# MougyTestspace/hclib

Hardware: AMD Instinct MI355X
Metric: UTS nodes/sec (tasks/sec) at 1/2/4/8 MI355X vs host-CPU HClib; forasync HBM GB/s (higher is better)
Workload: dtype u32; 1 GPU; test/uts T3L (-t 0 -b 2000 -q 0.200014 -m 5 -r 7) searched whole on 1 GPU (no split); nodes=111345631, bit_exact=True, parallelism=shard1 (hash-partitioned frontier, RCCL all-reduce of counts)

## Files before the change

hclib_amd/__init__.py:

```python
from __future__ import annotations

import ctypes as C
import os
from typing import Optional, Tuple

PKG = os.path.dirname(os.path.abspath(__file__))
LIB_PATH = os.environ.get("HCLIB_AMD_LIB") or os.path.join(PKG, "lib", "libhclib_amd.so")

HCLIB_HIP_OK = 0
FORASYNC_MODE_FLAT = 0
FORASYNC_MODE_RECURSIVE = 1
BODY_TRIAD_F32 = 1
BODY_IOTA_CHECK = 2
BODY_VISIT_COUNT = 3


class HclibError(RuntimeError):
    pass


class LoopDomain(C.Structure):

    _fields_ = [("low", C.c_int), ("high", C.c_int), ("stride", C.c_int), ("tile", C.c_int)]

# ... 48 lines not shown

class SwEdges(C.Structure):

    _fields_ = [("bottoms", C.c_void_p), ("rights", C.c_void_p), ("corners", C.c_void_p),
                ("path", C.c_int), ("form", C.c_int)]


SW_EDGE_BOTTOMS, SW_EDGE_RIGHTS, SW_EDGE_CORNERS = 1, 2, 4
SW_PATHS = {1: "queue", 2: "rows1", 3: "band-rows", 4: "dag-wave", 5: "dag-wg", 6: "dag-pk"}


class CholeskyResult(C.Structure):

    _fields_ = [("tasks", C.c_uint64), ("puts", C.c_uint64), ("releases", C.c_uint64),
                ("potrf", C.c_uint64), ("trsm", C.c_uint64), ("syrk", C.c_uint64), ("gemm", C.c_uint64),
                ("kernel_ms", C.c_double), ("gflops", C.c_double), ("fail_col", C.c_int)]


class SortResult(C.Structure):

    _fields_ = [("tasks", C.c_uint64), ("sort_leaf", C.c_uint64), ("sort_split", C.c_uint64),
                ("merge_leaf", C.c_uint64), ("merge_split", C.c_uint64), ("merge_empty", C.c_uint64),
                ("finishes", C.c_uint64), ("check_ins", C.c_uint64),
                ("kernel_ms", C.c_double), ("keys_per_s", C.c_double)]


class SparseLUResult(C.Structure):

    _fields_ = [("blocks_in", C.c_uint64), ("blocks_out", C.c_uint64),
                ("lu0", C.c_uint64), ("fwd", C.c_uint64), ("bdiv", C.c_uint64), ("bmod", C.c_uint64),
                ("tasks", C.c_uint64), ("puts", C.c_uint64), ("releases", C.c_uint64),
                ("kernel_ms", C.c_double), ("gflops", C.c_double), ("wgs_per_cu", C.c_int)]


class NQueensResult(C.Structure):

    _fields_ = [("solutions", C.c_uint64), ("tasks", C.c_uint64), ("items", C.c_uint64), ("scopes", C.c_uint64),
                ("joins", C.c_uint64), ("chunks_pushed", C.c_uint64), ("chunks_stolen", C.c_uint64),
                ("kernel_ms", C.c_double), ("busy_frac", C.c_double)]


class StrassenResult(C.Structure):

    _fields_ = [("tasks", C.c_uint64), ("splits", C.c_uint64), ("base", C.c_uint64), ("tiles", C.c_uint64),
                ("pre_bands", C.c_uint64), ("combine_bands", C.c_uint64), ("finishes", C.c_uint64),
                ("check_ins", C.c_uint64), ("workspace_bytes", C.c_uint64),
                ("kernel_ms", C.c_double), ("gflops", C.c_double)]


class FftResult(C.Structure):

    _fields_ = [("tasks", C.c_uint64), ("leaves", C.c_uint64), ("calls", C.c_uint64), ("unsh_bands", C.c_uint64),
                ("twid_bands", C.c_uint64), ("finishes", C.c_uint64), ("check_ins", C.c_uint64),
                ("bytes_moved", C.c_uint64), ("nfactors", C.c_int32), ("factors", C.c_int32 * 40),
                ("cutoff", C.c_int32), ("band", C.c_int32), ("kernel_ms", C.c_double), ("gbytes_per_s", C.c_double)]


class JacobiResult(C.Structure):

    _fields_ = [("tasks", C.c_uint64), ("puts", C.c_uint64), ("releases", C.c_uint64), ("supersteps", C.c_uint64),
                ("bytes_moved", C.c_uint64), ("block", C.c_int), ("fuse", C.c_int), ("wgs_per_cu", C.c_int),
                ("kernel_ms", C.c_double), ("gbytes_per_s", C.c_double), ("gcells_per_s", C.c_double)]


class BfsResult(C.Structure):

    _fields_ = [("levels", C.c_uint64), ("reached", C.c_uint64), ("relaxed", C.c_uint64), ("items", C.c_uint64),
                ("chunks_pushed", C.c_uint64), ("chunks_stolen", C.c_uint64),
                ("kernel_ms", C.c_double), ("busy_frac", C.c_double)]


class HealthParams(C.Structure):

    _fields_ = [(k, C.c_int) for k in ("level", "cities", "population_ratio", "sim_time", "assess_time",
                                       "convalescence_time")] + [("seed", C.c_int32)] + \
               [(k, C.c_float) for k in ("get_sick_p", "convalescence_p", "realloc_p")]


class HealthResult(C.Structure):

    _fields_ = [(k, C.c_int64) for k in ("population", "hospitals", "personnel", "hosps_visited", "in_village",
                                         "waiting", "assess", "inside", "total_time")] + \
               [(k, C.c_uint64) for k in ("tasks", "finishes", "check_ins", "leaf_calls", "inner_calls", "posts")] + \
               [("kernel_ms", C.c_double), ("rounds_per_s", C.c_double)]


class HealthState(C.Structure):

    _fields_ = [(k, C.c_void_p) for k in ("seed", "time", "time_left", "hosps_visited", "village", "lists")]


FLOORPLAN_MAX_CELLS, FLOORPLAN_MAX_SHAPES = 20, 8


class FloorplanInput(C.Structure):

    _fields_ = [("n", C.c_int32), ("solution", C.c_int32), ("shapes", C.c_int32 * (FLOORPLAN_MAX_CELLS + 1)),
                ("shape", C.c_int32 * 2 * FLOORPLAN_MAX_SHAPES * (FLOORPLAN_MAX_CELLS + 1)),
                ("left", C.c_int32 * (FLOORPLAN_MAX_CELLS + 1)), ("above", C.c_int32 * (FLOORPLAN_MAX_CELLS + 1)),
                ("next", C.c_int32 * (FLOORPLAN_MAX_CELLS + 1))]


class FloorplanPlacement(C.Structure):

    _fields_ = [("shape", C.c_int32), ("top", C.c_int32), ("lhs", C.c_int32)]


class FloorplanResult(C.Structure):

    _fields_ = [("min_area", C.c_int32), ("footprint", C.c_int32 * 2),
                ("placements", FloorplanPlacement * FLOORPLAN_MAX_CELLS)] + \
               [(k, C.c_uint64) for k in ("tasks", "items", "laid", "complete", "improvements", "chunks_pushed",
                                          "chunks_stolen")] + [("kernel_ms", C.c_double), ("busy_frac", C.c_double)]


class AlignmentInput(C.Structure):

    _fields_ = [("nseqs", C.c_int32), ("total", C.c_int32), ("length", C.POINTER(C.c_int32)),
                ("offset", C.POINTER(C.c_int32)), ("codes", C.POINTER(C.c_uint8)), ("names", C.c_void_p)]


class AlignmentMatrix(C.Structure):

    _fields_ = [("avscore", C.c_int32), ("score", C.c_int32 * 32 * 32)]


class AlignmentPair(C.Structure):

    _fields_ = [(k, C.c_int32) for k in ("si", "sj", "g", "gh", "maxscore", "se1", "se2", "sb1", "sb2", "matches",
                                         "diff_calls", "type2", "ties")]


class AlignmentResult(C.Structure):

    _fields_ = [("scores", C.c_void_p)] + \
               [(k, C.c_uint64) for k in ("pairs", "tasks", "created", "promises", "pair_tasks", "spawn_tasks",
                                          "leaf_tasks", "matches", "diff_calls", "type2", "ties", "cells")] + \
               [("cutoff", C.c_int32), ("kernel_ms", C.c_double), ("cells_per_s", C.c_double)]


class AtomicViewStruct(C.Structure):

    _fields_ = [("slots", C.c_void_p), ("nslots", C.c_uint32), ("stride", C.c_uint32),
                ("dtype", C.c_int), ("op", C.c_int)]


EXPORTS_HIP = [
    "hclib_hip_init", "hclib_hip_finalize", "hclib_hip_device_memory_live", "hclib_hip_last_error",
    "hclib_hip_num_cus",
    "hclib_hip_version", "hclib_hip_forasync", "hclib_hip_forasync_triad_f32",
    "hclib_hip_num_workers", "hclib_hip_uts_search", "hclib_hip_uts_num_children_host",
    "hclib_hip_uts_bucket_check", "hclib_hip_sha1_calibrate",
    "hclib_hip_fib", "hclib_hip_sw", "hclib_hip_last_sched_counters", "hclib_hip_last_narrow_counters",
    "hclib_hip_last_phase_counters", "hclib_hip_last_shed_counters",
    "hclib_hip_sw_band_begin", "hclib_hip_sw_band_rows", "hclib_hip_sw_band_end",
    "hclib_hip_sw_edges", "hclib_hip_sw_band_bottoms",
    "hclib_hip_atomic_create", "hclib_hip_atomic_destroy", "hclib_hip_atomic_view",
    "hclib_hip_atomic_gather", "hclib_hip_atomic_gather_async", "hclib_hip_atomic_reset",
    "hclib_hip_forasync_reduce", "hclib_hip_cholesky", "hclib_hip_sort_i64", "hclib_hip_sort_bounds",
    "hclib_hip_sparselu_genmat", "hclib_hip_sparselu_plan", "hclib_hip_sparselu", "hclib_hip_sparselu_bmod_rate",
    "hclib_hip_nqueens", "hclib_hip_nqueens_bounds",
    "hclib_hip_strassen", "hclib_hip_strassen_bounds", "hclib_hip_strassen_last_ticks",
    "hclib_hip_health", "hclib_hip_health_bounds", "hclib_hip_health_last_ticks",
    "hclib_hip_floorplan", "hclib_hip_floorplan_read_input",
    "hclib_hip_alignment", "hclib_hip_alignment_read_input", "hclib_hip_alignment_free_input",
    "hclib_hip_alignment_read_matrix", "hclib_hip_alignment_bounds", "hclib_hip_alignment_last_ticks",
    "hclib_hip_fft", "hclib_hip_fft_factors", "hclib_hip_fft_twiddles", "hclib_hip_fft_bounds", "hclib_hip_fft_last_ticks",
    "hclib_hip_jacobi", "hclib_hip_jacobi_rhs", "hclib_hip_jacobi_bounds",
    "hclib_hip_bfs", "hclib_hip_bfs_bounds", "hclib_hip_bfs_read_input",
    "hclib_atomic_create", "hclib_atomic_init", "hclib_atomic_update", "hclib_atomic_gather",
]

_lib = None


def lib():
    global _lib
    if _lib is None:
        try:
            import torch
        except ImportError:
            pass
        if not os.path.exists(LIB_PATH):
            raise HclibError(f"{LIB_PATH} is missing: run `python -m hclib_amd.build`")
        L = C.CDLL(LIB_PATH)
        L.hclib_hip_version.restype = C.c_char_p
        L.hclib_hip_last_error.restype = C.c_char_p
        L.hclib_hip_finalize.restype = None
        L.hclib_hip_device_memory_live.argtypes = [C.POINTER(C.c_uint64)]
        L.hclib_hip_device_memory_live.restype = None
        L.hclib_hip_forasync_triad_f32.argtypes = [C.c_void_p, C.c_void_p, C.c_void_p, C.c_float,
                                                   C.c_int64, C.c_void_p]
        L.hclib_hip_forasync.argtypes = [C.c_int, C.c_void_p, C.c_int, C.POINTER(LoopDomain),
                                         C.c_int, C.c_void_p]
        L.hclib_hip_uts_search.argtypes = [C.POINTER(UtsParams), C.c_int, C.c_int, C.c_int,
                                           C.POINTER(UtsResult), C.c_void_p, C.c_int]
        L.hclib_hip_uts_num_children_host.argtypes = [C.POINTER(UtsParams), C.c_int,
                                                      C.POINTER(C.c_uint32)]
        L.hclib_hip_fib.argtypes = [C.c_int, C.POINTER(C.c_int64), C.POINTER(FibResult)]
        L.hclib_hip_sw.argtypes = [C.c_char_p, C.c_size_t, C.c_char_p, C.c_size_t, C.c_int,
                                   C.c_int, C.POINTER(C.c_int), C.POINTER(SwResult)]
        L.hclib_hip_sw_band_begin.argtypes = [C.c_char_p, C.c_size_t, C.c_char_p, C.c_size_t,
                                              C.c_int, C.c_int, C.c_int, C.c_int,
                                              C.POINTER(C.c_void_p)]
        L.hclib_hip_sw_band_rows.argtypes = [C.c_void_p, C.c_int, C.c_int, C.c_void_p, C.c_void_p,
                                             C.c_void_p]
        L.hclib_hip_sw_band_end.argtypes = [C.c_void_p, C.c_void_p, C.POINTER(C.c_int),
                                            C.POINTER(C.c_uint64)]
        L.hclib_hip_sw_edges.argtypes = [C.c_char_p, C.c_size_t, C.c_char_p, C.c_size_t, C.c_int,
                                         C.c_int, C.POINTER(C.c_int), C.POINTER(SwResult),
                                         C.POINTER(SwEdges), C.POINTER(C.c_uint32)]
        L.hclib_hip_sw_band_bottoms.argtypes = [C.c_void_p, C.c_void_p, C.c_void_p]
        L.hclib_hip_atomic_calibrate.argtypes = [C.c_int, C.c_int, C.POINTER(C.c_double),
                                                 C.POINTER(C.c_double)]
        L.hclib_hip_sha1_calibrate.argtypes = [C.c_int, C.c_int, C.c_int, C.POINTER(C.c_double),
                                               C.POINTER(C.c_double)]
        L.hclib_hip_uts_last_launch.argtypes = [C.POINTER(UtsLaunch)]
        L.hclib_hip_uts_bucket_check.argtypes = [C.POINTER(UtsParams), C.c_uint64, C.POINTER(C.c_uint64)]
        L.hclib_hip_global_bytes.restype = C.c_size_t
        L.hclib_hip_global_bytes.argtypes = [C.c_uint32]
        L.hclib_hip_global_init.argtypes = [C.c_void_p, C.c_uint32, C.c_int]
        L.hclib_hip_global_alloc.argtypes = [C.c_uint32, C.c_int, C.POINTER(C.c_void_p)]
        L.hclib_hip_global_free.argtypes = [C.c_void_p]
        L.hclib_hip_global_attach.argtypes = [C.c_void_p, C.c_uint32, C.c_int]
        L.hclib_hip_global_read.argtypes = [C.c_void_p, C.POINTER(C.c_uint64)]
        L.hclib_hip_ipc_export.argtypes = [C.c_void_p, C.c_void_p]
        L.hclib_hip_ipc_import.argtypes = [C.c_void_p, C.POINTER(C.c_void_p)]
        L.hclib_hip_ipc_close.argtypes = [C.c_void_p]
        L.hclib_hip_last_timeline.argtypes = [C.c_void_p, C.c_uint64, C.POINTER(C.c_uint32)]
        L.hclib_hip_atomic_create.argtypes = [C.c_int, C.c_int, C.c_void_p, C.POINTER(C.c_void_p)]
        L.hclib_hip_atomic_destroy.argtypes = [C.c_void_p]
        L.hclib_hip_atomic_view.argtypes = [C.c_void_p, C.POINTER(AtomicViewStruct)]
        L.hclib_hip_atomic_gather.argtypes = [C.c_void_p, C.c_void_p, C.c_void_p]
        L.hclib_hip_atomic_gather_async.argtypes = [C.c_void_p, C.c_void_p, C.c_void_p]
        L.hclib_hip_atomic_reset.argtypes = [C.c_void_p, C.c_void_p]
        L.hclib_hip_forasync_reduce.argtypes = [C.c_void_p, C.c_void_p, C.c_int, C.POINTER(LoopDomain),
                                                C.c_int, C.c_void_p]
        L.hclib_hip_cholesky.argtypes = [C.c_void_p, C.c_int, C.c_int, C.c_int, C.c_void_p,
                                         C.POINTER(CholeskyResult)]
        L.hclib_hip_sort_i64.argtypes = [C.c_void_p, C.c_int64, C.c_int, C.c_int, C.POINTER(SortResult)]
        L.hclib_hip_sort_bounds.argtypes = [C.c_int64, C.c_int, C.c_int, C.POINTER(C.c_uint64)]
        L.hclib_hip_sort_last_ticks.argtypes = [C.POINTER(C.c_uint64)]
        L.hclib_hip_sort_last_ticks.restype = None
        L.hclib_hip_sparselu_genmat.argtypes = [C.c_int, C.c_int, C.c_void_p, C.c_void_p]
        L.hclib_hip_sparselu_plan.argtypes = [C.c_void_p, C.c_int, C.c_void_p, C.POINTER(C.c_uint64), C.c_void_p,
                                              C.c_void_p, C.c_void_p]
        L.hclib_hip_sparselu.argtypes = [C.c_void_p, C.c_void_p, C.c_int, C.c_int, C.c_void_p, C.c_void_p,
                                         C.POINTER(SparseLUResult)]
        L.hclib_hip_sparselu_bmod_rate.argtypes = [C.c_int, C.c_int, C.c_int, C.POINTER(C.c_double),
                                                   C.POINTER(C.c_double)]
        L.hclib_hip_nqueens.argtypes = [C.c_int, C.c_int, C.c_int, C.POINTER(NQueensResult), C.POINTER(C.c_uint64)]
        L.hclib_hip_nqueens_bounds.argtypes = [C.c_int, C.c_int, C.c_int, C.POINTER(C.c_uint64)]
        L.hclib_hip_floorplan.argtypes = [C.POINTER(FloorplanInput), C.c_int, C.POINTER(FloorplanResult), C.c_void_p,
                                          C.POINTER(C.c_uint64)]
        L.hclib_hip_floorplan_read_input.argtypes = [C.c_char_p, C.POINTER(FloorplanInput)]
        L.hclib_hip_strassen.argtypes = [C.c_void_p, C.c_void_p, C.c_void_p, C.c_int, C.c_int, C.c_int,
                                         C.POINTER(StrassenResult)]
        L.hclib_hip_strassen_bounds.argtypes = [C.c_int, C.c_int, C.c_int, C.POINTER(C.c_uint64)]
        L.hclib_hip_strassen_last_ticks.argtypes = [C.POINTER(C.c_uint64)]
        L.hclib_hip_strassen_last_ticks.restype = None
        L.hclib_hip_health.argtypes = [C.POINTER(HealthParams), C.POINTER(HealthResult), C.POINTER(HealthState)]
        L.hclib_hip_health_bounds.argtypes = [C.POINTER(HealthParams), C.POINTER(C.c_uint64)]
        L.hclib_hip_health_last_ticks.argtypes = [C.POINTER(C.c_uint64)]
        L.hclib_hip_health_last_ticks.restype = None
        L.hclib_hip_alignment.argtypes = [C.POINTER(AlignmentInput), C.POINTER(AlignmentMatrix), C.c_int,
                                          C.POINTER(AlignmentResult), C.c_void_p]
        L.hclib_hip_alignment_read_input.argtypes = [C.c_char_p, C.POINTER(AlignmentInput)]
        L.hclib_hip_alignment_free_input.argtypes = [C.POINTER(AlignmentInput)]
        L.hclib_hip_alignment_free_input.restype = None
        L.hclib_hip_alignment_read_matrix.argtypes = [C.c_char_p, C.POINTER(AlignmentMatrix)]
        L.hclib_hip_alignment_bounds.argtypes = [C.POINTER(AlignmentInput), C.c_int, C.POINTER(C.c_uint64)]
        L.hclib_hip_alignment_last_ticks.argtypes = [C.POINTER(C.c_uint64)]
        L.hclib_hip_alignment_last_ticks.restype = None
        L.hclib_hip_fft.argtypes = [C.c_void_p, C.c_void_p, C.c_int, C.c_void_p, C.c_int, C.c_int, C.POINTER(FftResult)]
        L.hclib_hip_fft_factors.argtypes = [C.c_int, C.POINTER(C.c_int)]
        L.hclib_hip_fft_twiddles.argtypes = [C.c_int, C.c_void_p]
        L.hclib_hip_fft_bounds.argtypes = [C.c_int, C.c_int, C.c_int, C.POINTER(C.c_uint64)]
        L.hclib_hip_fft_last_ticks.argtypes = [C.POINTER(C.c_uint64)]
        L.hclib_hip_fft_last_ticks.restype = None
        L.hclib_hip_jacobi.argtypes = [C.c_void_p, C.c_void_p, C.c_int, C.c_int, C.c_double, C.c_double, C.c_int, C.c_int,
                                       C.c_int, C.c_void_p, C.POINTER(JacobiResult)]
        L.hclib_hip_jacobi_rhs.argtypes = [C.c_int, C.c_int, C.c_void_p, C.c_void_p]
        L.hclib_hip_jacobi_bounds.argtypes = [C.c_int, C.c_int, C.c_int, C.c_int, C.c_int, C.POINTER(C.c_uint64)]
        L.hclib_hip_bfs.argtypes = [C.c_void_p, C.c_void_p, C.c_int, C.c_void_p, C.c_int, C.c_int, C.c_int, C.c_void_p,
                                    C.POINTER(BfsResult), C.c_void_p, C.c_void_p]
        L.hclib_hip_bfs_bounds.argtypes = [C.c_void_p, C.c_void_p, C.c_int, C.c_void_p, C.c_int, C.c_int, C.c_int,
                                           C.POINTER(C.c_uint64)]
        L.hclib_hip_bfs_read_input.argtypes = [C.c_char_p, C.c_void_p, C.c_void_p, C.c_void_p, C.POINTER(C.c_int64)]
        _lib = L
    return _lib


def _check(rc: int, what: str):
    if rc != HCLIB_HIP_OK:
        msg = lib().hclib_hip_last_error().decode(errors="replace")
        raise HclibError(f"{what} failed ({rc}): {msg}")


def version() -> str:
    return lib().hclib_hip_version().decode()


def init(device: int = 0) -> None:
    _check(lib().hclib_hip_init(device), "hclib_hip_init")


def finalize() -> None:
# ... 728 lines not shown
              inp.next[c]) for c in range(1, inp.n + 1)]
    return cells, inp.solution


def floorplan(cells_or_path, prune: bool = True, hist: bool = False) -> dict:
    cells = floorplan_read_input(cells_or_path)[0] if isinstance(cells_or_path, (str, bytes, os.PathLike)) \
        else cells_or_path
    inp = _floorplan_input(cells)
    r = FloorplanResult()
    board = (C.c_uint8 * 4096)()
    h = (C.c_uint64 * (FLOORPLAN_MAX_CELLS + 1))() if hist else None
    _check(lib().hclib_hip_floorplan(C.byref(inp), 0 if prune else FLOORPLAN_NOPRUNE, C.byref(r), board, h),
           "hclib_hip_floorplan")
    out = {k: getattr(r, k) for k, _ in FloorplanResult._fields_ if k not in ("footprint", "placements")}
    out["footprint"] = list(r.footprint)
    out["placements"] = [[p.shape, p.top, p.lhs] for p in r.placements[:inp.n]] if r.min_area < 4096 else None
    out["board"] = bytes(board)
    if hist:
        out["hist"] = list(h)[:inp.n + 1]
    return out


ALIGNMENT_CODES = "ABCDEFGHIKLMNPQRSTUVWXYZ-"
ALIGNMENT_MAX_LEN = 4999
ALIGNMENT_DEFAULT_CUTOFF = 16384
ALIGNMENT_BOUNDS = ("pairs", "tasks", "spawns", "diff_calls", "arena_bytes", "row_bytes")
ALIGNMENT_TICKS = ("root", "pair", "spawn", "leaf")


def alignment_read_input(path):
    inp = AlignmentInput()
    _check(lib().hclib_hip_alignment_read_input(os.fsencode(path), C.byref(inp)), "hclib_hip_alignment_read_input")
    try:
        names = C.string_at(inp.names, inp.nseqs * 31)
        return [(names[31 * i:31 * i + 31].split(b"\0")[0].decode("latin-1"),
                 [inp.codes[inp.offset[i] + k] for k in range(inp.length[i])]) for i in range(inp.nseqs)]
    finally:
        lib().hclib_hip_alignment_free_input(C.byref(inp))


def alignment_read_matrix(path):
    m = AlignmentMatrix()
    _check(lib().hclib_hip_alignment_read_matrix(os.fsencode(path), C.byref(m)), "hclib_hip_alignment_read_matrix")
    return m.avscore, [list(row) for row in m.score]


def _alignment_input(seqs):
    if isinstance(seqs, (str, bytes, os.PathLike)):
        seqs = alignment_read_input(seqs)
    codes = [list(q[1]) if isinstance(q, tuple) else list(q) for q in seqs]
    if any(not 0 <= c <= 255 for q in codes for c in q):
        raise ValueError("alignment: residue codes are 0..31")
    n, total = len(codes), sum(len(q) for q in codes)
    length = (C.c_int32 * max(n, 1))(*[len(q) for q in codes])
    offset = (C.c_int32 * max(n, 1))()
    flat = (C.c_uint8 * max(total, 1))()
    at = 0
    for i, q in enumerate(codes):
        offset[i] = at
        flat[at:at + len(q)] = q
        at += len(q)
    inp = AlignmentInput(nseqs=n, total=total, length=length, offset=offset, codes=flat, names=None)
    return inp, (length, offset, flat)


def _alignment_matrix(matrix) -> AlignmentMatrix:
    if isinstance(matrix, AlignmentMatrix):
        return matrix
    if isinstance(matrix, (str, bytes, os.PathLike)):
        matrix = alignment_read_matrix(matrix)
    avscore, rows = matrix
    if len(rows) != 32 or any(len(r) != 32 for r in rows):
        raise ValueError("alignment: the matrix has 32 x 32 scores")
    m = AlignmentMatrix(avscore=avscore)
    for i, row in enumerate(rows):
        for j, v in enumerate(row):
            m.score[i][j] = v
    return m


def alignment_bounds(seqs, cutoff: int = 0) -> dict:
    inp, keep = _alignment_input(seqs)
    out = (C.c_uint64 * 6)()
    _check(lib().hclib_hip_alignment_bounds(C.byref(inp), cutoff, out), "hclib_hip_alignment_bounds")
    return dict(zip(ALIGNMENT_BOUNDS, out))


def alignment(seqs, matrix, cutoff: int = 0, pairs: bool = False) -> dict:
    inp, keep = _alignment_input(seqs)
    m = _alignment_matrix(matrix)
    ns = inp.nseqs
    scores = (C.c_int32 * max(ns * ns, 1))()
    r = AlignmentResult(scores=C.addressof(scores))
    npairs = alignment_bounds([list(keep[2][keep[1][i]:keep[1][i] + keep[0][i]]) for i in range(ns)], cutoff)["pairs"] \
        if pairs else 0
    recs = (AlignmentPair * max(npairs, 1))() if pairs else None
    _check(lib().hclib_hip_alignment(C.byref(inp), C.byref(m), cutoff, C.byref(r), recs), "hclib_hip_alignment")
    out = {k: getattr(r, k) for k, _ in AlignmentResult._fields_ if k != "scores"}
    out["scores"] = [list(scores[i * ns:(i + 1) * ns]) for i in range(ns)]
    if pairs:
        out["pair_records"] = [{k: getattr(q, k) for k, _ in AlignmentPair._fields_} for q in recs[:npairs]]
    return out


def alignment_last_ticks() -> dict:
    out = (C.c_uint64 * 4)()
    lib().hclib_hip_alignment_last_ticks(out)
    return dict(zip(ALIGNMENT_TICKS, out))


ATOMIC_SCATTER_RET64 = 0
ATOMIC_HOT_WORD = 1
ATOMIC_COALESCED32 = 2


def atomic_calibrate(mode: int, iters: int = 256):
    r, ms = C.c_double(), C.c_double()
    _check(lib().hclib_hip_atomic_calibrate(mode, iters, C.byref(r), C.byref(ms)),
           "hclib_hip_atomic_calibrate")
    return r.value, ms.value


def sha1_calibrate(chains: int = 1, waves_per_cu: int = 8, iters: int = 2000):
    r, ms = C.c_double(), C.c_double()
    _check(lib().hclib_hip_sha1_calibrate(chains, waves_per_cu, iters, C.byref(r), C.byref(ms)),
           "hclib_hip_sha1_calibrate")
    return r.value, ms.value


def last_phase_counters():
    out = (C.c_uint64 * 8)()
    lib().hclib_hip_last_phase_counters(out)
    return list(out)


def last_sched_counters():
    out = (C.c_uint64 * 16)()
    lib().hclib_hip_last_sched_counters(out)
    return list(out)


def last_narrow_counters():
    out = (C.c_uint64 * 4)()
    lib().hclib_hip_last_narrow_counters(out)
    return list(out)


def last_shed_counters():
    out = (C.c_uint64 * 8)()
    lib().hclib_hip_last_shed_counters(out)
    return dict(zip(("exits", "placed", "blocks", "items", "fallbacks"), out))


TIMELINE_EVENTS = {1: "start", 2: "busy", 3: "idle", 4: "spill", 5: "term", 6: "end"}


def last_timeline():
    per = C.c_uint32()
    nw = lib().hclib_hip_last_timeline(None, 0, C.byref(per))
    if nw <= 0 or per.value == 0:
        return []
    import numpy as np
    buf = np.zeros(nw * per.value, dtype=np.uint64)
    lib().hclib_hip_last_timeline(buf.ctypes.data, buf.size, C.byref(per))
    buf = buf.reshape(nw, per.value)
    out = []
    for w in range(nw):
        row = buf[w][buf[w] != 0]
        out.append([(int(v >> 24), int((v >> 20) & 0xF), int(v & 0xFFFFF)) for v in row])
    return out
```

hclib_amd/csrc/hx_module.h:

```cpp
#pragma once

#include <hip/hip_runtime.h>
#include <stdint.h>

#include <string>
#include <vector>

#include "../../include/hclib_hip.h"
#include "../../include/hclib_hip/hx_sched.h"

namespace hx {

enum ArenaId {
    kArenaGlobals,
    kArenaWaveStats,
    kArenaWaveCtr,
    kArenaTimeline,
    kArenaDeques,
    kArenaSeed,
    kArenaDag,
    kArenaDagTrace,
    kArenaDyn,
    kArenaCholesky,
    kArenaSparselu,
    kArenaSort,
    kArenaStrassen,
    kArenaHealth,
    kArenaAlignment,
    kArenaFft,
    kArenaJacobi,
    kArenaUtsTables,
    kArenaCount
};
struct Arena {
    void *mem = nullptr;
    size_t bytes = 0;
};

struct Module {
    bool inited = false;
    int device = -1;
    int num_cus = 0;
    std::string arch;
    hipStream_t stream = nullptr;
    hipEvent_t ev0 = nullptr, ev1 = nullptr;
    Arena arenas[kArenaCount];
    bool uts_tables_cached = false;
    SchedGlobals *globals = nullptr;
    unsigned long long last_counters[16] = {};
    unsigned long long last_narrow[4] = {};
    unsigned long long last_shed[8] = {};
    unsigned long long last_phase[8] = {};
    WaveStat *wave_stats = nullptr;
    uint32_t wave_stats_cap = 0;
    std::vector<WaveStat> last_waves;
    unsigned long long *wave_ctr = nullptr;
    uint32_t rec_workers = 0;
    GlobalView gview = {nullptr, nullptr, nullptr, 0, 0};
    unsigned long long *timeline = nullptr;
    uint32_t timeline_cap = 0;
    std::vector<unsigned long long> last_timeline;
};

Module &mod();
void set_error(const char *fmt, ...);
int ensure_device();
int hip_check(hipError_t e, const char *what);
int check_resident(const void *kern, int blocks, int threads, size_t lds, const char *what);
int upload_async(void *dst, const void *src, size_t bytes, hipStream_t stream);

int arena_reserve(ArenaId id, size_t bytes, const char *who, void **ptr);

class DevBuf {
  public:
    DevBuf() = default;
    DevBuf(const DevBuf &) = delete;
    DevBuf &operator=(const DevBuf &) = delete;
    ~DevBuf();
    int alloc(size_t bytes, const char *who);
    char *p = nullptr;

  private:
    size_t bytes_ = 0;
};

int make_pool(uint32_t nq, uint32_t cap, uint32_t chunk, uint32_t words, PoolView *out);
struct SeedCfg {
    uint32_t target, max_levels, words, min_levels;
    uint32_t solo_cap = 0;
};
int reset_sched(const PoolView &pool, uint32_t outstanding_init, bool global = false, uint32_t workers = 0,
                const SeedCfg *seed = nullptr);
int finish_sched(SchedGlobals *host_copy, const char *who);

int env_int(const char *name, int dflt);

}

#define HX_TRY(expr)                         \
    do {                                     \
        int _rc = (expr);                    \
        if (_rc != HCLIB_HIP_OK) return _rc; \
    } while (0)
#define HX_HIP(call) HX_TRY(::hx::hip_check((call), #call))
```

hclib_amd/csrc/hx_uts_plan.h:

```cpp
#pragma once

#include <stdarg.h>
#include <stdio.h>

#include "hx_uts_host.h"

namespace hx {

enum UtsMode : int {
    kUtsRulesGlobal = 0,
    kUtsRulesLds = 1,
    kUtsBin = 2,
    kUtsGeoFixed = 3,
};

constexpr int kUtsSeedMaxLevels = 24;

struct UtsKnobs {
    static constexpr int kUnset = -0x7fffffff;
    int grid = 0;
    int waves_per_cu = kUnset;
    int wpg = 4;
    int uts_ring = kUnset;
    int uts_geo_fixed = 1;
    int uts_seed = 1;
    int uts_trace = 0;
    int uts_dual = 1;
    int deques = 128, deque_cap = 4096, chunk = 64;
    int spill_hi = 512;
    int spill_lo = kUnset;
    int seed_per_wave = kUnset;
    bool seed_per_wave_set = false;
    int seed_levels = 20, seed_solo = 128;
    int hunger = kUnset;
    int spin_limit_ms = 20000, stamps = 0, carry = 2, backoff = 16, defer = 1, spills_per_batch = 0;
    int narrow_shed = 1, narrow_shed_sibs = 3;
};

struct UtsPlan {
    int status = HCLIB_HIP_OK;
    bool bin = false, geo_fixed = false;
    int geo_depth = 0;
    int lds_tables = 0;
    uint32_t bin_thr = 0;
    int mode = 0;
    int feat = 0;
    bool global = false;
    int ring = 512, wpg = 1, grid = 0, waves_per_cu = 0;
    uint32_t nq = 0, deque_cap = 0, chunk = 0;
    uint32_t spill_hi = 0, spill_lo = 0, spin_limit = 0, nwaves = 0, stamps = 0, hunger = 0, backoff = 0, carry = 0,
             defer = 0, dual = 0, spills = 0, hunger_init_full = 0, narrow_shed = 0;
    uint32_t seed_target = 0, seed_max_levels = 0, seed_min_levels = 0, seed_solo_cap = 0;
    hclib_hip_uts_launch_t launch = {-1, 0, 0, 0, 0, 0, 0, 0, 0};
};

namespace uts_detail {
__attribute__((format(printf, 2, 3))) inline int refuse(std::string &err, const char *fmt, ...) {
    char buf[512];
    va_list ap;
    va_start(ap, fmt);
    vsnprintf(buf, sizeof(buf), fmt, ap);
    va_end(ap);
    err = buf;
    return HCLIB_HIP_EINVAL;
}
}

inline UtsPlan uts_plan(const hclib_hip_uts_params_t &p, const UtsTables &T, int num_cus, int shard, int nshards,
                        int split_depth, int max_levels, bool global_attached, const UtsKnobs &kn, std::string &err) {
    using uts_detail::refuse;
    constexpr int U = UtsKnobs::kUnset;
    (void)shard;
    UtsPlan P;
    const int trace_kind = max_levels > 0 ? kn.uts_trace : 0;
    const bool trace = trace_kind != 0;

    P.lds_tables = (T.rules.size() <= kUtsLdsRules && T.thr.size() <= kUtsLdsThr) ? 1 : 0;
    {
        const int nr = (int)T.rules.size();
        int d = 1;
        while (d < nr && T.rules[d].x == 2 && T.rules[d].z == 0) ++d;
        bool rest_zero = d > 1 && T.stationary;
        for (int e = d; e < nr && rest_zero; ++e) rest_zero = T.rules[e].x == 0 && T.rules[e].y == 0;
        if (rest_zero && T.thr.size() >= 128) P.geo_depth = d;
    }
    const bool bin = p.type == 0 && T.rules.size() == 2 && T.rules[1].x == 1 && T.stationary;
    const bool geo_fixed = !bin && P.geo_depth > 0 && kn.uts_geo_fixed;
    P.bin = bin;
    P.geo_fixed = geo_fixed;
    if (bin) P.bin_thr = (uint32_t)T.rules[1].y;
    const int mode = bin ? kUtsBin : geo_fixed ? kUtsGeoFixed : (P.lds_tables ? kUtsRulesLds : kUtsRulesGlobal);
    P.mode = mode;
    const double est = uts_expected_nodes(p);

    const bool trace_refused = trace && (mode != kUtsBin || nshards > 1);

    P.nq = (uint32_t)kn.deques;
    P.deque_cap = (uint32_t)kn.deque_cap;
    P.chunk = (uint32_t)kn.chunk;

    const bool global = nshards > 1 && global_attached && max_levels == 0;
    P.global = global;
    const bool seed_on = geo_fixed && !global && kn.uts_seed;
    bool bin_seed = bin && nshards > 1 && !global && max_levels == 0 && split_depth >= 1 &&
                    split_depth + 1 < kUtsSeedMaxLevels && kn.uts_seed;
    int wpc_default = bin && !global ? 4 : 2, ring_default = 512;
    if (!bin) {
        if (seed_on) {
            wpc_default = 8;
            ring_default = 512;
        } else {
            wpc_default = est >= 3e7 ? 8 : (geo_fixed ? 2 : 4);
            ring_default = est >= 3e7 ? 512 : 256;
        }
    }
    const int grid = kn.grid > 0 ? kn.grid : num_cus * (kn.waves_per_cu != U ? kn.waves_per_cu : wpc_default);
    P.grid = grid;
    P.waves_per_cu = grid / (num_cus > 0 ? num_cus : 1);
    if (bin_seed) {
        const double cap = 8.0 * 1 + 65536.0;
        const double qm = p.non_leaf_prob * bin_rule_m(p) > 0 ? p.non_leaf_prob * bin_rule_m(p) : 0.0;
        double n = T.root_nc > 0 ? (double)T.root_nc : 0.0, widest = n;
        for (int d = 2; d <= split_depth; ++d) {
            n *= qm;
            if (n > widest) widest = n;
        }
        const double n_mine = n * qm / nshards;
        if (!(widest <= 0.5 * cap && n_mine <= 0.5 * cap && n_mine <= (double)grid * (1024 / 4))) bin_seed = false;
    }
    P.spill_hi = (uint32_t)kn.spill_hi;
    const int ring_used = geo_fixed && !(nshards > 1 || max_levels > 0) ? (kn.uts_ring != U ? kn.uts_ring : ring_default)
                                                                       : 512;
    if (ring_used != 256 && ring_used != 512 && ring_used != 1024) {
        P.status = refuse(err,
                          "hclib_hip_uts_search: HCLIB_HIP_UTS_RING=%d is not a ring the search is built for (256, 512 "
                          "or 1024 items per wave)", ring_used);
        return P;
    }
    int spill_lo_default = bin ? 66 : (geo_fixed && ring_used < 512) ? 128 : 224;
    const int per_wave = kn.seed_per_wave != U ? kn.seed_per_wave : (est >= 3e7 ? 32 : 16);
    bool seed_fits = seed_on && ring_used >= 512;
    if (seed_fits) {
        if (kn.seed_per_wave_set) {
            const double b = geo_bi(p, 1) > kUtsMaxChildren ? (double)kUtsMaxChildren : geo_bi(p, 1);
            if (per_wave < 1) {
                P.status = refuse(err,
                                  "hclib_hip_uts_search: HCLIB_HIP_SEED_PER_WAVE=%d is not a slot count (1 or more; "
                                  "HCLIB_HIP_UTS_SEED=0 turns the seeding off)", per_wave);
                return P;
            }
            if (b * per_wave > ring_used / 2) {
                P.status = refuse(err,
                                  "hclib_hip_uts_search: HCLIB_HIP_SEED_PER_WAVE=%d cannot fit the ring: a wave's share "
                                  "of the seeded level reaches %.0f x %d items, the seeding hands over at most %d of a "
                                  "%d-item ring", per_wave, b, per_wave, ring_used / 2, ring_used);
                return P;
            }
        }
        const double target = (double)grid * per_wave, cap = 8.0 * target + 65536.0;
        double n = T.root_nc > 0 ? (double)T.root_nc : 0.0;
        for (int d = 1; d < 64 && n > 0.0 && n < target; ++d) {
            const double b = geo_bi(p, d) > kUtsMaxChildren ? (double)kUtsMaxChildren : geo_bi(p, d);
            n *= b > 0.0 ? b : 0.0;
        }
        seed_fits = n <= 0.5 * cap && n <= (double)grid * (ring_used / 4);
    }
    const bool seeded = seed_fits;
    if (seeded) spill_lo_default = est >= 3e7 ? 448 : 336;
    {
        const int ring_launch = bin ? 1024 : ring_used, lo = kn.spill_lo != U ? kn.spill_lo : spill_lo_default;
        if (lo < 1 || lo > ring_launch) {
            P.status = refuse(err,
                              "hclib_hip_uts_search: HCLIB_HIP_SPILL_LO=%d does not fit the %d-item ring of this launch "
                              "(1..%d)", lo, ring_launch, ring_launch);
            return P;
        }
        P.spill_lo = (uint32_t)lo;
    }
    P.spin_limit = (uint32_t)kn.spin_limit_ms;
    P.nwaves = (uint32_t)grid;
    P.stamps = (uint32_t)kn.stamps;
    const bool small_fixed = geo_fixed && est < 3e7;
    const bool large_fixed = geo_fixed && ring_used >= 512 && !small_fixed;
    P.hunger = (uint32_t)(kn.hunger != U ? kn.hunger : large_fixed ? 128 : bin ? 64 : 32);
    P.carry = (uint32_t)kn.carry;
    P.backoff = (uint32_t)kn.backoff;
    P.defer = (uint32_t)kn.defer;
    P.dual = (uint32_t)kn.uts_dual;
    P.spills = (uint32_t)kn.spills_per_batch;
    {
        const int rule = kn.narrow_shed, sibs = kn.narrow_shed_sibs;
        if (rule < 0 || rule > 3 || sibs < 0 || sibs > 3) {
            P.status = refuse(err,
                              "hclib_hip_uts_search: HCLIB_HIP_NARROW_SHED=%d / HCLIB_HIP_NARROW_SHED_SIBS=%d: the keep "
                              "rule is 0 (off), 1, 2 or 3, the sibling inboxes per exit 0..3", rule, sibs);
            return P;
        }
        P.narrow_shed = (uint32_t)rule | (uint32_t)sibs << 8;
    }
    if (trace_refused) {
        P.status = refuse(err, "hclib_hip_uts_search: the depth trace is for unsharded BIN trees");
        return P;
    }
    if (seeded) {
        P.seed_target = (uint32_t)(grid * per_wave);
        P.seed_max_levels = (uint32_t)kn.seed_levels;
        P.seed_solo_cap = (uint32_t)kn.seed_solo;
        if (nshards > 1) {
            double n_split = 1.0, n_next = 1.0;
            for (int d = 0; d <= split_depth && d < 64; ++d) {
                if (d < split_depth) n_split *= geo_bi(p, d) > 0 ? geo_bi(p, d) : 0.0;
                n_next *= geo_bi(p, d) > 0 ? geo_bi(p, d) : 0.0;
            }
            const double cap = 8.0 * P.seed_target + 65536.0;
            const bool fits = split_depth + 1 < kUtsSeedMaxLevels && split_depth < (int)P.seed_max_levels &&
                              n_split <= 0.5 * cap && n_next / nshards <= (double)grid * (512 / 8);
            P.seed_min_levels = fits ? (uint32_t)split_depth : 0u;
        }
    } else if (bin_seed) {
        P.seed_target = 1;
        P.seed_max_levels = (uint32_t)split_depth;
        P.seed_min_levels = (uint32_t)split_depth;
    }

    const bool seed_past_split = P.seed_target && nshards > 1 && P.seed_min_levels == (uint32_t)split_depth;
    const bool filter = max_levels > 0 || (nshards > 1 && (global || !seed_past_split));
    P.feat = trace ? (trace_kind == 2 ? 3 : 2) : (filter ? 1 : 0);
    P.ring = mode == kUtsBin ? 1024 : 512;
    if (mode == kUtsGeoFixed && !filter && !global) P.ring = ring_used;
    if (mode == kUtsBin && !global && (!trace || trace_kind == 2)) {
        P.wpg = kn.wpg;
        if (P.wpg != 2 && P.wpg != 4) P.wpg = 1;
        if (grid % P.wpg) P.wpg = 1;
    }
    P.launch = hclib_hip_uts_launch_t{mode, trace ? 1 + trace_kind : P.feat, P.wpg, grid, P.ring, P.seed_target ? 1 : 0, (int)P.seed_target,
                                      (int)P.spill_lo, P.waves_per_cu};
    return P;
}

}
```

hclib_amd/csrc/module.hip:

```cpp
#include <stdarg.h>
#include <stdio.h>
#include <stdlib.h>
#include <string.h>

#include "hx_client.h"

namespace hx {

static Module g_mod;
static thread_local char g_err[512] = "";

Module &mod() { return g_mod; }

void set_error(const char *fmt, ...) {
    va_list ap;
    va_start(ap, fmt);
    vsnprintf(g_err, sizeof(g_err), fmt, ap);
    va_end(ap);
}

static uint64_t g_live[2] = {0, 0};
static bool dev_acquire(void **p, size_t bytes) {
    if (hipMalloc(p, bytes) != hipSuccess) {
        (void)hipGetLastError();
// ... 82 lines not shown
int make_pool(uint32_t nq, uint32_t cap, uint32_t chunk, uint32_t words, PoolView *out) {
    if (nq < 8 || nq % 8 || cap < 2 || (cap & (cap - 1)) || chunk < 1 || chunk > 64) {
        set_error("chunk deques: need 8k deques, power-of-two capacity, 1..64 items per chunk");
        return HCLIB_HIP_EINVAL;
    }
    for (uint32_t c = chunk; c * 2 <= 64; c *= 2) cap *= 2;
    const size_t hdr = sizeof(QueueHdr) * nq;
    const size_t slots = (size_t)nq * cap;
    const size_t need = hdr + slots * 4 * 2 + slots * chunk * words * 4 + 4096;
    char *p = nullptr;
    HX_TRY(arena_reserve(kArenaDeques, need, "chunk deques", (void **)&p));
    out->hdr = (QueueHdr *)p;
    p += hdr;
    out->seq = (uint32_t *)p;
    out->cnt = out->seq + 1;
    p += slots * 8;
    p = (char *)(((uintptr_t)p + 255) & ~(uintptr_t)255);
    out->data = (uint32_t *)p;
    out->nq = nq;
    out->cap = cap;
    out->chunk = chunk;
    return HCLIB_HIP_OK;
}

struct Staged {
    void *host;
    hipEvent_t done;
};
std::vector<Staged> &staged() {
    static std::vector<Staged> v;
    return v;
}
void reap_staged() {
    std::vector<Staged> &v = staged();
    for (size_t i = 0; i < v.size();) {
        if (hipEventQuery(v[i].done) == hipSuccess) {
            (void)hipHostFree(v[i].host);
            (void)hipEventDestroy(v[i].done);
            v[i] = v.back();
            v.pop_back();
        } else {
            ++i;
        }
    }
}
int upload_async(void *dst, const void *src, size_t bytes, hipStream_t st) {
    reap_staged();
    void *pin = nullptr;
    HX_HIP(hipHostMalloc(&pin, bytes, hipHostMallocDefault));
    memcpy(pin, src, bytes);
    hipEvent_t ev;
    if (hipEventCreateWithFlags(&ev, hipEventDisableTiming) != hipSuccess) {
        (void)hipHostFree(pin);
        set_error("upload: hipEventCreate failed");
        return HCLIB_HIP_EHIP;
    }
    if (hipMemcpyAsync(dst, pin, bytes, hipMemcpyHostToDevice, st) != hipSuccess ||
        hipEventRecord(ev, st) != hipSuccess) {
        (void)hipStreamSynchronize(st);
        (void)hipHostFree(pin);
        (void)hipEventDestroy(ev);
        set_error("upload: host-to-device copy failed");
        return HCLIB_HIP_EHIP;
    }
    staged().push_back(Staged{pin, ev});
    return HCLIB_HIP_OK;
}

int reset_sched(const PoolView &pool, uint32_t outstanding_init, bool global, uint32_t workers,
                const SeedCfg *seed) {
    Module &m = g_mod;
    HX_HIP(hipMemsetAsync(pool.hdr, 0, sizeof(QueueHdr) * pool.nq, m.stream));
    const uint32_t total = pool.nq * pool.cap;
    hipLaunchKernelGGL(k_reset_pool, dim3((total + 255) / 256), dim3(256), 0, m.stream, pool.seq,
                       pool.cap, total);
    HX_HIP(hipGetLastError());
    SchedGlobals init;
    memset(&init, 0, sizeof(init));
    init.outstanding = outstanding_init;
    init.wave_stats = m.wave_stats;
    init.wave_stats_cap = m.wave_stats_cap;
    m.rec_workers = workers < m.wave_stats_cap ? workers : m.wave_stats_cap;
    init.wave_ctr = m.rec_workers ? m.wave_ctr : nullptr;
    init.wave_ctr_cap = m.rec_workers;
    if (seed && seed->target && workers) {
        const uint32_t cap = 8u * seed->target + 65536u;
        const size_t ctl = (size_t)kSeedCtlLines * 256;
        const size_t need = ctl + 2ull * cap * seed->words * 4;
        char *seed_mem = nullptr;
        HX_TRY(arena_reserve(kArenaSeed, need, "seeding", (void **)&seed_mem));
        HX_HIP(hipMemsetAsync(seed_mem, 0, ctl, m.stream));
        init.seed.ctl = (uint32_t *)seed_mem;
        init.seed.buf = (uint32_t *)(seed_mem + ctl);
        init.seed.cap = cap;
        init.seed.target = seed->target;
        init.seed.max_levels = seed->max_levels;
        init.seed.min_levels = seed->min_levels;
        init.seed.solo_cap = seed->solo_cap;
        init.outstanding = workers;
    }
    if (global) init.gview = m.gview;
    const int tl_cap = env_int("HCLIB_HIP_TIMELINE", 0);
    if (tl_cap > 0) {
        HX_TRY(arena_reserve(kArenaTimeline, (size_t)m.wave_stats_cap * tl_cap * 8, "worker timelines",
                             (void **)&m.timeline));
        m.timeline_cap = (uint32_t)tl_cap;
        HX_HIP(hipMemsetAsync(m.timeline, 0, (size_t)m.wave_stats_cap * tl_cap * 8, m.stream));
        init.timeline = m.timeline;
        init.timeline_cap = m.timeline_cap;
    }
    static SchedGlobals *stage = nullptr;
    if (!stage && hipHostMalloc((void **)&stage, sizeof(SchedGlobals), hipHostMallocDefault) != hipSuccess)
        return upload_async(m.globals, &init, sizeof(init), m.stream);
    *stage = init;
    HX_HIP(hipMemcpyAsync(m.globals, stage, sizeof(init), hipMemcpyHostToDevice, m.stream));
    return HCLIB_HIP_OK;
}

static const char *err_name(uint32_t e) {
    switch (e) {
    case kErrQueueFull: return "chunk deque full and LDS ring near capacity";
    case kErrStackOverflow: return "LDS ring overflow";
    case kErrSpinTimeout: return "idle spin timed out (no termination)";
    case kErrDepthTable: return "tree deeper than the device depth-rule table";
    case kErrArena: return "device arena exhausted";
    case kErrBadTask: return "malformed task";
    default: return "unknown device error";
    }
}

int finish_sched(SchedGlobals *host_copy, const char *who) {
    Module &m = g_mod;
    HX_HIP(hipMemcpyAsync(host_copy, m.globals, sizeof(SchedGlobals), hipMemcpyDeviceToHost,
                          m.stream));
    const uint32_t nw_cap = m.wave_stats_cap;
    static std::vector<unsigned long long> rec;
    const uint32_t nrec = m.rec_workers;
    for (int i = 0; i < 8; ++i) m.last_phase[i] = 0;
    m.rec_workers = 0;
    if (nrec) {
        rec.resize((size_t)nrec * kWaveCtrWords);
        HX_HIP(hipMemcpyAsync(rec.data(), m.wave_ctr, rec.size() * 8, hipMemcpyDeviceToHost, m.stream));
    }
    HX_HIP(hipStreamSynchronize(m.stream));
    for (uint32_t w = 0; w < nrec; ++w) {
        const unsigned long long *r = &rec[(size_t)w * kWaveCtrWords];
        for (int i = 0; i < 16; ++i)
            if (i >= 8 || i < 4) host_copy->counters[i] += r[i];
        for (int i = 4; i < 8; ++i) host_copy->counters[i] += r[24 + i - 4];
        for (int i = 0; i < 4; ++i)
            if (r[16 + i] > host_copy->maxes[i]) host_copy->maxes[i] = r[16 + i];
        for (int i = 0; i < 3; ++i) host_copy->narrow[i] += r[20 + i];
        for (int i = 0; i < kShedCounts; ++i) host_copy->shed[i] += r[32 + i];
        m.last_phase[0] += r[23];
        for (int i = 0; i < 4; ++i) m.last_phase[1 + i] += r[28 + i];
        m.last_phase[5] += r[24];
        m.last_phase[6] += r[27];
    }
    memcpy(m.last_counters, host_copy->counters, sizeof(m.last_counters));
    memcpy(m.last_narrow, host_copy->narrow, sizeof(m.last_narrow));
    memcpy(m.last_shed, host_copy->shed, sizeof(m.last_shed));
    uint64_t nw = host_copy->counters[kCtrWaves];
    if (nw > nw_cap) nw = nw_cap;
    m.last_waves.resize(nw);
    if (nw) HX_HIP(hipMemcpy(m.last_waves.data(), m.wave_stats, nw * sizeof(WaveStat), hipMemcpyDeviceToHost));
    if (host_copy->timeline) {
        m.last_timeline.resize((size_t)nw * m.timeline_cap);
        if (nw)
            HX_HIP(hipMemcpy(m.last_timeline.data(), m.timeline, (size_t)nw * m.timeline_cap * 8,
                             hipMemcpyDeviceToHost));
    } else {
        m.last_timeline.clear();
    }
    if (host_copy->err) {
        set_error("%s: device error %u (%s)", who, host_copy->err, err_name(host_copy->err));
        return HCLIB_HIP_EDEVICE;
    }
    return HCLIB_HIP_OK;
}

}

using namespace hx;

extern "C" {

const char *hclib_hip_version(void) { return "hclib-mi355x 0.1 (gfx950 megakernel scheduler)"; }

const char *hclib_hip_last_error(void) { return g_err; }

int hclib_hip_init(int device) {
    Module &m = g_mod;
    if (m.inited) return HCLIB_HIP_OK;
    int n = 0;
    if (hipGetDeviceCount(&n) != hipSuccess || n <= 0) {
        set_error("hclib_hip_init: no HIP device visible");
        return HCLIB_HIP_ENODEV;
    }
    if (device < 0 || device >= n) {
        set_error("hclib_hip_init: device %d out of range (%d devices)", device, n);
        return HCLIB_HIP_EINVAL;
    }
    HX_HIP(hipSetDevice(device));
    hipDeviceProp_t prop;
    HX_HIP(hipGetDeviceProperties(&prop, device));
    m.arch = prop.gcnArchName;
    if (m.arch.rfind("gfx950", 0) != 0) {
        set_error("hclib_hip_init: device %d is %s, this module is built for gfx950 only", device,
                  prop.gcnArchName);
        return HCLIB_HIP_ENODEV;
    }
    m.device = device;
    m.num_cus = prop.multiProcessorCount;
    HX_HIP(hipStreamCreateWithFlags(&m.stream, hipStreamNonBlocking));
    HX_HIP(hipEventCreate(&m.ev0));
    HX_HIP(hipEventCreate(&m.ev1));
    const char *who = "hclib_hip_init";
    HX_TRY(arena_reserve(kArenaGlobals, sizeof(SchedGlobals), who, (void **)&m.globals));
    m.wave_stats_cap = (uint32_t)m.num_cus * 32;
    HX_TRY(arena_reserve(kArenaWaveStats, sizeof(WaveStat) * m.wave_stats_cap, who, (void **)&m.wave_stats));
    HX_TRY(arena_reserve(kArenaWaveCtr, 8ull * kWaveCtrWords * m.wave_stats_cap, who, (void **)&m.wave_ctr));
    m.inited = true;
    return HCLIB_HIP_OK;
}

void hclib_hip_finalize(void) {
    Module &m = g_mod;
    if (!m.inited) return;
    (void)hipStreamSynchronize(m.stream);
    for (Arena &a : m.arenas) dev_release(a.mem, a.bytes);
    (void)hipEventDestroy(m.ev0);
    (void)hipEventDestroy(m.ev1);
    (void)hipStreamDestroy(m.stream);
    m = Module();
}

void hclib_hip_device_memory_live(uint64_t out[2]) {
    out[0] = g_live[0];
    out[1] = g_live[1];
}

int hclib_hip_num_cus(void) { return g_mod.inited ? g_mod.num_cus : 0; }

int hclib_hip_device(void) { return g_mod.inited ? g_mod.device : -1; }

void *hclib_hip_stream(void) { return g_mod.inited ? (void *)g_mod.stream : nullptr; }

void hclib_hip_last_sched_counters(uint64_t out[16]) {
    for (int i = 0; i < 16; ++i) out[i] = g_mod.last_counters[i];
}

extern "C" void hclib_hip_last_phase_counters(uint64_t out[8]) {
    for (int i = 0; i < 8; ++i) out[i] = g_mod.last_phase[i];
}

void hclib_hip_last_narrow_counters(uint64_t out[4]) {
    for (int i = 0; i < 4; ++i) out[i] = g_mod.last_narrow[i];
}

void hclib_hip_last_shed_counters(uint64_t out[8]) {
    for (int i = 0; i < 8; ++i) out[i] = g_mod.last_shed[i];
}

int hclib_hip_last_wave_stats(hclib_hip_wave_stats_t *out, int max) {
    static_assert(sizeof(hclib_hip_wave_stats_t) == sizeof(WaveStat), "layout");
    const int n = (int)g_mod.last_waves.size();
    for (int i = 0; out && i < n && i < max; ++i) memcpy(&out[i], &g_mod.last_waves[(size_t)i], sizeof(WaveStat));
    return n;
}

int hclib_hip_last_timeline(uint64_t *out, uint64_t max_words, uint32_t *events_per_worker) {
    Module &m = g_mod;
    if (events_per_worker) *events_per_worker = m.last_timeline.empty() ? 0u : m.timeline_cap;
    const uint64_t n = m.last_timeline.size();
    for (uint64_t i = 0; out && i < n && i < max_words; ++i) out[i] = m.last_timeline[i];
    return m.timeline_cap ? (int)(n / m.timeline_cap) : 0;
}

int hclib_hip_sched_begin(uint32_t entry_words, uint32_t chunk, int waves_per_cu,
                          hclib_hip_sched_launch_t *out) {
    if (!out || entry_words < 4 || entry_words > 64 || waves_per_cu < 1 || waves_per_cu > 8) {
        set_error("hclib_hip_sched_begin: invalid arguments");
        return HCLIB_HIP_EINVAL;
    }
    HX_TRY(ensure_device());
    Module &m = g_mod;
    PoolView pool;
    HX_TRY(sched_pool(64, chunk, entry_words, &pool));
    HX_TRY(reset_sched(pool, 1, false, (uint32_t)(m.num_cus * waves_per_cu)));
    HX_HIP(hipEventRecord(m.ev0, m.stream));
    out->hdr = pool.hdr;
    out->seq = pool.seq;
    out->cnt = pool.cnt;
    out->data = pool.data;
    out->nq = pool.nq;
    out->cap = pool.cap;
    out->chunk = pool.chunk;
    out->globals = m.globals;
    out->stream = m.stream;
    out->grid = m.num_cus * waves_per_cu;
    out->num_cus = m.num_cus;
    return HCLIB_HIP_OK;
}

int hclib_hip_sched_end(const char *who, uint64_t counters[16], uint64_t maxes[4], double *kernel_ms) {
    Module &m = g_mod;
    if (!m.inited) {
        set_error("hclib_hip_sched_end: no device");
        return HCLIB_HIP_ENODEV;
    }
    SchedGlobals gl;
    memset(&gl, 0, sizeof(gl));
    float ms = 0;
    const int rc = end_sched(who ? who : "hclib_hip_sched_end", &gl, &ms);
    if (kernel_ms) *kernel_ms = ms;
    for (int i = 0; counters && i < 16; ++i) counters[i] = gl.counters[i];
    for (int i = 0; maxes && i < 4; ++i) maxes[i] = gl.maxes[i];
    return rc;
}

int hclib_hip_num_workers(void) {
    if (!g_mod.inited) return 0;
    return g_mod.num_cus * env_int("HCLIB_HIP_WAVES_PER_CU", 4);
}

}

static size_t global_layout(uint32_t cap, size_t *ctl_off, size_t *data_off) {
    const size_t words = 64 * 8;
    const size_t hdr = (sizeof(GlobalHdr) + 255) & ~(size_t)255;
    const size_t ctl = ((size_t)cap * 8 + 255) & ~(size_t)255;
    *ctl_off = hdr;
    *data_off = hdr + ctl;
    return hdr + ctl + (size_t)cap * words * 4;
}

extern "C" size_t hclib_hip_global_bytes(uint32_t cap) {
    size_t a, b;
    if (cap < 2 || (cap & (cap - 1))) return 0;
    return global_layout(cap, &a, &b);
}

__global__ void k_reset_global(uint32_t *ctl, uint32_t cap) {
    const uint32_t i = blockIdx.x * blockDim.x + threadIdx.x;
    if (i < cap) {
        ctl[2 * i] = i;
        ctl[2 * i + 1] = 0;
    }
}

extern "C" int hclib_hip_global_init(void *region, uint32_t cap, int nranks) {
    if (!region || cap < 2 || (cap & (cap - 1)) || nranks < 1 || nranks > kGlobalMaxRanks) {
        set_error("hclib_hip_global_init: invalid arguments");
        return HCLIB_HIP_EINVAL;
    }
    HX_TRY(ensure_device());
    Module &m = g_mod;
    size_t co, dof;
    global_layout(cap, &co, &dof);
    HX_HIP(hipMemsetAsync(region, 0, co, m.stream));
    hipLaunchKernelGGL(k_reset_global, dim3((cap + 255) / 256), dim3(256), 0, m.stream,
                       (uint32_t *)((char *)region + co), cap);
    HX_HIP(hipGetLastError());
    const uint32_t active = (uint32_t)nranks;
    uint32_t held[kGlobalMaxRanks];
    for (int r = 0; r < kGlobalMaxRanks; ++r) held[r] = r < nranks ? 1u : 0u;
    HX_HIP(hipMemcpyAsync(region, &active, 4, hipMemcpyHostToDevice, m.stream));
    HX_HIP(hipMemcpyAsync((char *)region + offsetof(GlobalHdr, held), held, sizeof(held), hipMemcpyHostToDevice,
                          m.stream));
    HX_HIP(hipStreamSynchronize(m.stream));
    return HCLIB_HIP_OK;
}

extern "C" int hclib_hip_global_attach(void *region, uint32_t cap, int rank) {
    HX_TRY(ensure_device());
    Module &m = g_mod;
    if (!region) {
        m.gview = GlobalView{nullptr, nullptr, nullptr, 0, 0};
        return HCLIB_HIP_OK;
    }
    if (cap < 2 || (cap & (cap - 1)) || rank < 0 || rank >= kGlobalMaxRanks) {
        set_error("hclib_hip_global_attach: invalid arguments");
        return HCLIB_HIP_EINVAL;
    }
    size_t co, dof;
    global_layout(cap, &co, &dof);
    m.gview.hdr = (GlobalHdr *)region;
    m.gview.ctl = (uint32_t *)((char *)region + co);
    m.gview.data = (uint32_t *)((char *)region + dof);
    m.gview.cap = cap;
    m.gview.rank = (uint32_t)rank;
    return HCLIB_HIP_OK;
}

extern "C" int hclib_hip_global_read(const void *region, uint64_t out[3 + 2 * kGlobalMaxRanks]) {
    if (!region || !out) {
        set_error("hclib_hip_global_read: invalid arguments");
        return HCLIB_HIP_EINVAL;
    }
    HX_TRY(ensure_device());
    GlobalHdr h;
    HX_HIP(hipMemcpy(&h, region, sizeof(h), hipMemcpyDeviceToHost));
    out[0] = h.active;
    out[1] = h.idle;
    out[2] = h.tail - h.head;
    for (int i = 0; i < 2 * kGlobalMaxRanks; ++i) out[3 + i] = h.moved[i];
    return HCLIB_HIP_OK;
}

extern "C" int hclib_hip_global_alloc(uint32_t cap, int kind, void **region_out) {
    size_t co, dof;
    if (!region_out || cap < 2 || (cap & (cap - 1)) || kind < 0 || kind > 2) {
        set_error("hclib_hip_global_alloc: invalid arguments");
        return HCLIB_HIP_EINVAL;
// ... 50 lines not shown
```

hclib_amd/csrc/uts.hip:

```cpp
#include <string.h>

#include <type_traits>
#include <vector>

#include "hx_client.h"
#include "uts_sha1.h"
#include "hx_uts_plan.h"

namespace hx {


static_assert(sizeof(UtsRule) == sizeof(int4) && offsetof(UtsRule, x) == offsetof(int4, x) &&
                  offsetof(UtsRule, y) == offsetof(int4, y) && offsetof(UtsRule, z) == offsetof(int4, z) &&
                  offsetof(UtsRule, w) == offsetof(int4, w),
              "UtsRule is uploaded as int4");
static_assert(kUtsSeedMaxLevels == kSeedMaxLevels, "the plan's level bound is the seeding's");
struct UtsCtx {
    uint32_t root[5];
    int root_nc;
    int nrules;
    int stationary;
    int gran;
    int m;
    int shard, nshards, split;
// ... 74 lines not shown
    using Ctx = UtsCtx;
    static constexpr bool kFixedChildren = MODE == kUtsBin;
    __device__ static uint32_t fixed_children(const Ctx &c) { return c.m > 0 ? (uint32_t)c.m : 0u; }
    struct Acc {
        uint32_t nodes = 0, leaves = 0;
        uint32_t maxd = 0;
        uint32_t trace_seen = 0;
        uint32_t mode = 0;
        uint32_t wid = 0;
        __device__ void totals(unsigned long long (&c)[8], unsigned long long (&m)[4]) {
            c[0] = wave_sum((unsigned long long)nodes);
            c[1] = wave_sum((unsigned long long)leaves);
            m[0] = (unsigned long long)wave_max(maxd);
        }
    };

    __device__ static bool movable(const Ctx &c, const uint32_t *tmpl) {
        return c.nshards <= 1 || (int)tmpl[5] >= c.split;
    }

    __device__ static int roots(const Ctx &c, Acc &acc, uint32_t *tmpl) {
        if (lane_id() == 0 && c.shard == 0) {
            acc.nodes += 1;
            if (c.root_nc <= 0) acc.leaves += 1;
            if (c.hist && c.hist_levels > 0) atomicAdd(&c.hist[0], 1ull);
        }
        for (int k = 0; k < 5; ++k) tmpl[k] = c.root[k];
        tmpl[5] = FEAT == 3 ? 0x80000000u : 0u;
        return c.root_nc;
    }

    template <int F = FEAT>
    __device__ static __forceinline__ int finish(const Ctx &c, Acc &acc, const uint32_t *t, const uint32_t *ch,
                                                 uint32_t *child, uint32_t *err, bool valid) {
        const int h1 = (int)(F == 3 ? t[5] & 0x7fffffffu : t[5]) + 1;
        bool counted = valid;
        if (F && c.nshards > 1) {
            if (h1 == c.split && (ch[0] % (uint32_t)c.nshards) != (uint32_t)c.shard) return 0;
            if (h1 < c.split && c.shard != 0) counted = false;
        }
        int nc = uts_nc<MODE>(c, valid ? h1 : 1, ch[4] & 0x7fffffffu, err);
        acc.nodes += counted ? 1u : 0u;
        acc.leaves += (counted && nc <= 0) ? 1u : 0u;
        acc.maxd = (counted && (uint32_t)h1 > acc.maxd) ? (uint32_t)h1 : acc.maxd;
        if (F == 1 && counted && c.hist && h1 < c.hist_levels) atomicAdd(&c.hist[h1], 1ull);
        if (F == 2 && c.hist) {
            const uint32_t dm = wave_max(counted ? (uint32_t)h1 : 0u);
            if (dm > acc.trace_seen) {
                acc.trace_seen = dm;
                if (lane_id() == 0 && (int)dm < c.hist_levels)
                    __hip_atomic_fetch_min(&c.hist[dm],
                                           ((__builtin_amdgcn_s_memrealtime() & 0x3fffffffffffull) << 17) |
                                               ((unsigned long long)(acc.wid & 0xffffu) << 1) | acc.mode,
                                           __ATOMIC_RELAXED, HX_AGENT);
            }
        }
        if (!valid) nc = 0;
        child[0] = ch[0];
        child[1] = ch[1];
        child[2] = ch[2];
        child[3] = ch[3];
        child[4] = ch[4];
        child[5] = (uint32_t)h1;
        return nc;
    }

    __device__ static __forceinline__ uint32_t chain_next(const Ctx &c, const uint32_t *t, bool valid) {
        uint32_t kc = 0xffffffffu;
        if (FEAT == 3 && valid && (t[5] >> 31)) kc = c.chain[(t[5] & 0x7fffffffu) + 1u];
        return kc;
    }
    __device__ static __forceinline__ void chain_stamp(const Ctx &c, const Acc &acc, uint32_t *child, bool on,
                                                       bool valid, uint32_t dual) {
        if constexpr (FEAT == 3) {
            const uint32_t fill = (uint32_t)__builtin_popcountll(__ballot(valid));
            if (on) {
                const uint32_t d = child[5];
                child[5] = d | 0x80000000u;
                c.hist[4 * d] = __builtin_amdgcn_s_memrealtime();
                c.hist[4 * d + 1] = (unsigned long long)((acc.wid & 0xffffu) | (acc.mode << 16) | (dual << 17) |
                                                         (fill << 20));
            }
        }
    }

    __device__ static void trace_item(const Ctx &c, const uint32_t *w, bool valid, uint32_t ev, bool via_inbox) {
        if constexpr (FEAT == 3) {
            if (valid && (w[5] >> 31)) {
                const uint32_t d = (w[5] & 0x7fffffffu) + 1u;
                const uint32_t kc = c.chain[d];
                if (kc >= w[kWords - 2] && kc < w[kWords - 1])
                    c.hist[4 * d + ev] = __builtin_amdgcn_s_memrealtime() | (via_inbox ? 1ull << 63 : 0ull);
            }
        }
    }

    __device__ static int process(const Ctx &c, Acc &acc, const uint32_t *t, uint32_t k,
                                  uint32_t *child, uint32_t *err, bool valid) {
        uint32_t ch[5];
        const uint32_t kc = chain_next(c, t, valid);
        rng_spawn_dev(t, k, ch);
        for (int g = 1; g < c.gran; ++g) rng_spawn_dev(t, k, ch);
        const int nc = finish(c, acc, t, ch, child, err, valid);
        chain_stamp(c, acc, child, k == kc, valid, 0u);
        return nc;
    }

    static constexpr bool kBulkCount = FEAT == 0;
    __device__ static __forceinline__ bool process_bulk(const Ctx &c, Acc &acc, const uint32_t *t, uint32_t k,
                                                        uint32_t *child, uint32_t *err, bool valid) {
        static_assert(MODE == kUtsBin, "the fixed-size narrow loop runs BIN trees");
        uint32_t ch[5];
        rng_spawn_dev(t, k, ch);
        for (int g = 1; g < c.gran; ++g) rng_spawn_dev(t, k, ch);
        const int h1 = (int)t[5] + 1;
        acc.maxd = (valid && (uint32_t)h1 > acc.maxd) ? (uint32_t)h1 : acc.maxd;
        for (int i = 0; i < 5; ++i) child[i] = ch[i];
        child[5] = (uint32_t)h1;
        return valid && (ch[4] & 0x7fffffffu) < c.bin_thr;
    }
    __device__ static void count_bulk(Acc &acc, uint32_t nodes, uint32_t leaves) {
        if (lane_id() == 0) {
            acc.nodes += nodes;
            acc.leaves += leaves;
        }
    }

    __device__ static int seed_process(const Ctx &c, Acc &acc, const uint32_t *t, uint32_t k, uint32_t *child,
                                       uint32_t *err, bool valid) {
        uint32_t ch[5];
        rng_spawn_dev(t, k, ch);
        for (int g = 1; g < c.gran; ++g) rng_spawn_dev(t, k, ch);
        return finish<FEAT == 0 ? 1 : FEAT>(c, acc, t, ch, child, err, valid);
    }

    __device__ static void process2(const Ctx &c, Acc &acc, const uint32_t *tA, uint32_t kA, uint32_t *childA,
                                    int &ncA, const uint32_t *tB, uint32_t kB, uint32_t *childB, int &ncB,
                                    uint32_t *err, bool validB) {
        uint32_t chA[5], chB[5];
        const uint32_t kcA = chain_next(c, tA, true), kcB = chain_next(c, tB, validB);
        const uint32_t *pp[2] = {tA, tB};
        const uint32_t ii[2] = {kA, kB};
        uint32_t *oo[2] = {chA, chB};
        rng_spawn_n<2>(pp, ii, oo);
        for (int g = 1; g < c.gran; ++g) rng_spawn_n<2>(pp, ii, oo);
        ncA = finish(c, acc, tA, chA, childA, err, true);
        ncB = finish(c, acc, tB, chB, childB, err, validB);
        chain_stamp(c, acc, childA, kA == kcA, true, 1u);
        chain_stamp(c, acc, childB, kB == kcB, validB, 1u);
    }
};

template <int MODE, int FEAT, int CAP = (MODE == kUtsBin ? 1024 : 512), bool GLOBAL = false, int WPG = 1>
__global__ __launch_bounds__(64 * WPG) void k_uts_search(UtsCtx ctx, PoolView pool, SchedGlobals *g,
                                                         SchedConfig cfg) {
    constexpr int kUtsCap = CAP;
    using K = UtsKind<MODE, FEAT, CAP>;
    __shared__ WaveStack<K, kUtsCap> st[WPG];
    __shared__ Inbox<K> ib[WPG];
    const uint32_t wave = WPG > 1 ? threadIdx.x / 64 : 0;
    const uint32_t worker = blockIdx.x * WPG + wave;
    if (WPG > 1) {
        if (threadIdx.x < WPG) {
            ib[threadIdx.x].state = 0;
            ib[threadIdx.x].idle = 0;
        }
    }
    if (MODE == kUtsGeoFixed) {
        for (int i = threadIdx.x; i < 128; i += 64 * WPG) s_thr[i] = ctx.thr[i];
        for (int i = threadIdx.x; i < kUtsBuckets / 4; i += 64 * WPG) s_thr[128 + i] = ctx.nb[i];
    }
    if (MODE == kUtsRulesLds) {
        for (int i = threadIdx.x; i < ctx.nrules; i += 64 * WPG) s_rules[i] = ctx.rules[i];
        for (int i = threadIdx.x; i < ctx.nthr; i += 64 * WPG) s_thr[i] = ctx.thr[i];
    }
    __syncthreads();
    run_worker<K, kUtsCap, GLOBAL, WPG>(ctx, pool, g, cfg, st[wave], worker == 0, ib, wave, worker);
}

static int uts_tables(const hclib_hip_uts_params_t &p, UtsTables &T) {
    std::string err;
    const int rc = build_tables(p, T, err);
    if (rc != HCLIB_HIP_OK) set_error("%s", err.c_str());
    return rc;
}

}

using namespace hx;

extern "C" int hclib_hip_uts_num_children_host(const hclib_hip_uts_params_t *params, int height,
                                               const uint32_t st[5]) {
    static hclib_hip_uts_params_t last_p;
    static UtsTables T;
    static bool have = false;
    if (!have || memcmp(&last_p, params, sizeof(last_p)) != 0) {
        have = false;
        if (uts_tables(*params, T) != HCLIB_HIP_OK) return -1;
        last_p = *params;
        have = true;
    }
    if (height == 0) return T.root_nc;
    return host_nc(*params, T, height, st[4] & 0x7fffffffu);
}

extern "C" int hclib_hip_uts_bucket_check(const hclib_hip_uts_params_t *params, uint64_t nrandom,
                                          uint64_t *checked) {
    if (!params) {
        set_error("hclib_hip_uts_bucket_check: NULL params");
        return HCLIB_HIP_EINVAL;
    }
    UtsTables T;
    if (uts_tables(*params, T) != HCLIB_HIP_OK) return HCLIB_HIP_EINVAL;
    if (T.thr.size() < 128) {
        if (checked) *checked = 0;
        return 0;
    }
    const uint32_t *t0 = T.thr.data();
    uint8_t nb[kUtsBuckets];
    build_buckets(t0, nb);
    uint64_t n = 0;
    int bad = 0;
    auto one = [&](int64_t v) {
        if (v < 0 || v > 0x7fffffffll) return;
        const uint32_t r = (uint32_t)v;
        int exact = 0;
        for (int k = 1; k <= 100; ++k) exact += t0[k] <= r;
        bad += bucket_nc(t0, nb, r) != exact;
        ++n;
    };
    for (int k = 1; k <= 100; ++k)
        if (t0[k] != 0x80000000u)
            for (int d = -3; d <= 3; ++d) one((int64_t)t0[k] + d);
    for (int b = 0; b <= kUtsBuckets; ++b)
        for (int d = -1; d <= 1; ++d) one(((int64_t)b << kUtsBucketShift) + d);
    uint64_t x = 0x9e3779b97f4a7c15ull;
    for (uint64_t i = 0; i < nrandom; ++i) {
        x += 0x9e3779b97f4a7c15ull;
        uint64_t z = x;
        z = (z ^ (z >> 30)) * 0xbf58476d1ce4e5b9ull;
        z = (z ^ (z >> 27)) * 0x94d049bb133111ebull;
        one((int64_t)((z ^ (z >> 31)) & 0x7fffffffull));
    }
    if (checked) *checked = n;
    return bad;
}

static thread_local hclib_hip_uts_launch_t g_last_launch{-1, 0, 0, 0, 0, 0, 0, 0, 0};

extern "C" int hclib_hip_uts_last_launch(hclib_hip_uts_launch_t *out) {
    if (!out) {
        set_error("hclib_hip_uts_last_launch: null output");
        return HCLIB_HIP_EINVAL;
    }
    *out = g_last_launch;
    return g_last_launch.mode < 0 ? HCLIB_HIP_EINVAL : HCLIB_HIP_OK;
}

static UtsKnobs uts_knobs() {
    UtsKnobs k;
    k.grid = env_int("HCLIB_HIP_GRID", k.grid);
    k.waves_per_cu = env_int("HCLIB_HIP_WAVES_PER_CU", k.waves_per_cu);
    k.wpg = env_int("HCLIB_HIP_WPG", k.wpg);
    k.uts_ring = env_int("HCLIB_HIP_UTS_RING", k.uts_ring);
    k.uts_geo_fixed = env_int("HCLIB_HIP_UTS_GEO_FIXED", k.uts_geo_fixed);
    k.uts_seed = env_int("HCLIB_HIP_UTS_SEED", k.uts_seed);
    k.uts_trace = env_int("HCLIB_HIP_UTS_TRACE", k.uts_trace);
    k.uts_dual = env_int("HCLIB_HIP_UTS_DUAL", k.uts_dual);
    k.deques = env_int("HCLIB_HIP_DEQUES", k.deques);
    k.deque_cap = env_int("HCLIB_HIP_DEQUE_CAP", k.deque_cap);
    k.chunk = env_int("HCLIB_HIP_CHUNK", k.chunk);
    k.spill_hi = env_int("HCLIB_HIP_SPILL_HI", k.spill_hi);
    k.spill_lo = env_int("HCLIB_HIP_SPILL_LO", k.spill_lo);
    k.seed_per_wave = env_int("HCLIB_HIP_SEED_PER_WAVE", k.seed_per_wave);
    k.seed_per_wave_set = getenv("HCLIB_HIP_SEED_PER_WAVE") != nullptr;
    k.seed_levels = env_int("HCLIB_HIP_SEED_LEVELS", k.seed_levels);
    k.seed_solo = env_int("HCLIB_HIP_SEED_SOLO", k.seed_solo);
    k.hunger = env_int("HCLIB_HIP_HUNGER", k.hunger);
    k.spin_limit_ms = env_int("HCLIB_HIP_SPIN_LIMIT_MS", k.spin_limit_ms);
    k.stamps = env_int("HCLIB_HIP_STAMPS", k.stamps);
    k.carry = env_int("HCLIB_HIP_CARRY", k.carry);
    k.backoff = env_int("HCLIB_HIP_BACKOFF", k.backoff);
    k.defer = env_int("HCLIB_HIP_DEFER", k.defer);
    k.spills_per_batch = env_int("HCLIB_HIP_SPILLS_PER_BATCH", k.spills_per_batch);
    k.narrow_shed = env_int("HCLIB_HIP_NARROW_SHED", k.narrow_shed);
    k.narrow_shed_sibs = env_int("HCLIB_HIP_NARROW_SHED_SIBS", k.narrow_shed_sibs);
    return k;
}

typedef void (*uts_kernel_t)(UtsCtx, PoolView, SchedGlobals *, SchedConfig);
static uts_kernel_t uts_kernel(int mode, int feat, int cap, bool global, int wpg) {
#define HX_UTS_KERNEL(MODE, FEAT, CAP, GLOBAL, WPG) {MODE, FEAT, CAP, GLOBAL, WPG, k_uts_search<MODE, FEAT, CAP, GLOBAL, WPG>}
    static const struct {
        int mode, feat, cap;
        bool global;
        int wpg;
        uts_kernel_t kern;
    } kernels[] = {
        HX_UTS_KERNEL(kUtsRulesGlobal, 0, 512, false, 1), HX_UTS_KERNEL(kUtsRulesGlobal, 1, 512, false, 1),
        HX_UTS_KERNEL(kUtsRulesLds, 0, 512, false, 1), HX_UTS_KERNEL(kUtsRulesLds, 1, 512, false, 1),
        HX_UTS_KERNEL(kUtsBin, 0, 1024, false, 1), HX_UTS_KERNEL(kUtsBin, 1, 1024, false, 1),
        HX_UTS_KERNEL(kUtsGeoFixed, 0, 512, false, 1), HX_UTS_KERNEL(kUtsGeoFixed, 1, 512, false, 1),
        HX_UTS_KERNEL(kUtsBin, 3, 1024, false, 1), HX_UTS_KERNEL(kUtsBin, 2, 1024, false, 1),
        HX_UTS_KERNEL(kUtsRulesGlobal, 1, 512, true, 1), HX_UTS_KERNEL(kUtsRulesLds, 1, 512, true, 1),
        HX_UTS_KERNEL(kUtsBin, 1, 1024, true, 1), HX_UTS_KERNEL(kUtsGeoFixed, 1, 512, true, 1),
        HX_UTS_KERNEL(kUtsGeoFixed, 0, 256, false, 1), HX_UTS_KERNEL(kUtsGeoFixed, 0, 1024, false, 1),
        HX_UTS_KERNEL(kUtsBin, 3, 1024, false, 2), HX_UTS_KERNEL(kUtsBin, 3, 1024, false, 4),
        HX_UTS_KERNEL(kUtsBin, 1, 1024, false, 2), HX_UTS_KERNEL(kUtsBin, 0, 1024, false, 2),
        HX_UTS_KERNEL(kUtsBin, 1, 1024, false, 4), HX_UTS_KERNEL(kUtsBin, 0, 1024, false, 4),
    };
#undef HX_UTS_KERNEL
    for (const auto &k : kernels)
        if (k.mode == mode && k.feat == feat && k.cap == cap && k.global == global && k.wpg == wpg) return k.kern;
    return nullptr;
}

extern "C" int hclib_hip_uts_search(const hclib_hip_uts_params_t *params, int shard, int nshards,
                                    int split_depth, hclib_hip_uts_result_t *result,
                                    uint64_t *level_hist, int max_levels) {
    const char *who = "hclib_hip_uts_search";
    const UtsKnobs knobs = uts_knobs();
    if (!params || !result || nshards < 1 || shard < 0 || shard >= nshards || max_levels < 0 ||
        max_levels > (knobs.uts_trace == 2 ? 4 * 65536 : 65536) || (nshards > 1 && split_depth < 1)) {
        set_error("hclib_hip_uts_search: invalid arguments");
        return HCLIB_HIP_EINVAL;
    }
    HX_TRY(ensure_device());
    Module &m = mod();
    static struct {
        hclib_hip_uts_params_t p;
        UtsTables T;
    } tab;
    const auto pad = [](size_t b) { return (b + 255) & ~(size_t)255; };
    if (!m.uts_tables_cached || memcmp(&tab.p, params, sizeof(tab.p)) != 0) {
        m.uts_tables_cached = false;
        HX_TRY(uts_tables(*params, tab.T));
        const size_t rb = tab.T.rules.size() * sizeof(int4), tb = tab.T.thr.size() * 4;
        char *dp = nullptr;
        HX_TRY(arena_reserve(kArenaUtsTables, pad(rb) + pad(tb) + kUtsBuckets + 256, who, (void **)&dp));
        HX_HIP(hipMemcpy(dp, tab.T.rules.data(), rb, hipMemcpyHostToDevice));
        HX_HIP(hipMemcpy(dp + pad(rb), tab.T.thr.data(), tb, hipMemcpyHostToDevice));
        uint8_t nb[kUtsBuckets] = {0};
        if (tab.T.thr.size() >= 128) build_buckets(tab.T.thr.data(), nb);
        HX_HIP(hipMemcpy(dp + pad(rb) + pad(tb), nb, kUtsBuckets, hipMemcpyHostToDevice));
        tab.p = *params;
        m.uts_tables_cached = true;
    }
    const UtsTables &T = tab.T;
    char *d_tab = (char *)m.arenas[kArenaUtsTables].mem;

    std::string why;
    const UtsPlan plan = uts_plan(*params, T, m.num_cus, shard, nshards, split_depth, max_levels,
                                  m.gview.hdr != nullptr, knobs, why);
    if (plan.status != HCLIB_HIP_OK) {
        set_error("%s", why.c_str());
        return plan.status;
    }
    const uts_kernel_t kern = uts_kernel(plan.mode, plan.feat, plan.ring, plan.global, plan.wpg);
    if (!kern) {
        set_error("%s: no kernel for mode %d, feat %d, ring %d, global %d, %d waves per workgroup", who, plan.mode,
                  plan.feat, plan.ring, (int)plan.global, plan.wpg);
        return HCLIB_HIP_EINVAL;
    }

    const size_t hb = (size_t)max_levels * 8;
    DevBuf hist_buf, chain_buf;
    if (max_levels) HX_TRY(hist_buf.alloc(hb, who));
    unsigned long long *d_hist = (unsigned long long *)hist_buf.p;
    if (max_levels) HX_HIP(hipMemsetAsync(d_hist, plan.feat >= 2 ? 0xff : 0, hb, m.stream));
    uint32_t *d_chain = nullptr;
    if (plan.feat == 3) {
        std::vector<uint32_t> chain;
        const char *path = getenv("HCLIB_HIP_UTS_CHAIN");
        if (FILE *f = path ? fopen(path, "rb") : nullptr) {
            uint32_t w;
            while (fread(&w, 4, 1, f) == 1) chain.push_back(w);
            fclose(f);
        }
        if (chain.empty() || chain[0] + 1 != chain.size() || (size_t)max_levels < 4 * chain.size()) {
            set_error("hclib_hip_uts_search: chain trace needs HCLIB_HIP_UTS_CHAIN and max_levels >= 4 (D + 1)");
            return HCLIB_HIP_EINVAL;
        }
        HX_TRY(chain_buf.alloc(chain.size() * 4, who));
        d_chain = (uint32_t *)chain_buf.p;
        HX_HIP(hipMemcpy(d_chain, chain.data(), chain.size() * 4, hipMemcpyHostToDevice));
    }

    UtsCtx ctx;
    memcpy(ctx.root, T.root, sizeof(ctx.root));
    ctx.root_nc = T.root_nc;
    ctx.nrules = (int)T.rules.size();
    ctx.stationary = T.stationary;
    ctx.gran = params->compute_gran < 1 ? 1 : params->compute_gran;
    ctx.m = bin_rule_m(*params);
    ctx.shard = shard;
    ctx.nshards = nshards;
    ctx.split = split_depth;
    ctx.hist_levels = max_levels;
    ctx.lds_tables = plan.lds_tables;
    ctx.bin_thr = plan.bin_thr;
    ctx.nthr = (int)T.thr.size();
    ctx.geo_depth = plan.geo_depth;
    ctx.rules = (const int4 *)d_tab;
    ctx.thr = (const uint32_t *)(d_tab + pad(T.rules.size() * sizeof(int4)));
    ctx.nb = (const uint32_t *)((const char *)ctx.thr + pad(T.thr.size() * 4));
    ctx.hist = max_levels ? d_hist : nullptr;
    ctx.chain = d_chain;

    PoolView pool;
    HX_TRY(make_pool(plan.nq, plan.deque_cap, plan.chunk, UtsKind<kUtsBin, 0>::kWords, &pool));
    SchedConfig cfg;
    cfg.spill_hi = plan.spill_hi;
    cfg.spill_lo = plan.spill_lo;
    cfg.spin_limit = plan.spin_limit;
    cfg.nwaves = plan.nwaves;
    cfg.stamps = plan.stamps;
    cfg.hunger = plan.hunger;
    cfg.backoff = plan.backoff;
    cfg.carry = plan.carry;
    cfg.defer = plan.defer;
    cfg.dual = plan.dual;
    cfg.spills = plan.spills;
    cfg.hunger_init_full = plan.hunger_init_full;
    cfg.narrow_shed = plan.narrow_shed;
    SeedCfg seed{plan.seed_target, plan.seed_max_levels, (uint32_t)UtsKind<kUtsBin, 0>::kWords, plan.seed_min_levels};
    seed.solo_cap = plan.seed_solo_cap;
    HX_TRY(reset_sched(pool, 1, plan.global, (uint32_t)plan.grid, seed.target ? &seed : nullptr));
    g_last_launch = plan.launch;
    SchedGlobals gl;
    float ms = 0;
    const int rc = launch_sched((const void *)kern, plan.grid / plan.wpg, 64 * plan.wpg, who, [&] {
        hipLaunchKernelGGL(kern, dim3(plan.grid / plan.wpg), dim3(64 * plan.wpg), 0, m.stream, ctx, pool, m.globals, cfg);
    }, &gl, &ms);
    if (rc != HCLIB_HIP_OK) return rc;
    if (max_levels) {
        std::vector<unsigned long long> h(max_levels);
        HX_HIP(hipMemcpy(h.data(), d_hist, hb, hipMemcpyDeviceToHost));
        for (int i = 0; i < max_levels; ++i) level_hist[i] = h[i];
    }
    result->nodes = gl.counters[0];
    result->leaves = gl.counters[1];
    result->max_depth = gl.maxes[0];
    result->batches = gl.counters[kCtrBatches];
    result->chunks_pushed = gl.counters[kCtrPushed];
    result->chunks_stolen = gl.counters[kCtrStolen];
    result->kernel_ms = ms;
    result->busy_frac = busy_frac(gl);
    const double busy = (double)gl.counters[kCtrBusyCycles];
    const double mhz = gl.counters[kCtrRealTicks]
                           ? 100.0 * (double)gl.counters[kCtrClockTicks] / (double)gl.counters[kCtrRealTicks]
                           : 2400.0;
    result->us_per_batch = gl.counters[kCtrBatches] ? busy / gl.counters[kCtrBatches] / mhz : 0.0;
    return HCLIB_HIP_OK;
}
```

include/hclib_hip.h:

```cpp
#ifndef HCLIB_HIP_H_
#define HCLIB_HIP_H_

#include <stddef.h>
#include <stdint.h>

#ifdef __cplusplus
extern "C" {
#endif

#define HCLIB_HIP_OK 0
#define HCLIB_HIP_ENODEV (-1)
#define HCLIB_HIP_EINVAL (-2)
#define HCLIB_HIP_ENOMEM (-3)
#define HCLIB_HIP_EDEVICE (-4)
#define HCLIB_HIP_EHIP (-5)

int hclib_hip_init(int device);
void hclib_hip_finalize(void);
void hclib_hip_device_memory_live(uint64_t out[2]);
const char *hclib_hip_last_error(void);
int hclib_hip_num_cus(void);
int hclib_hip_device(void);
void *hclib_hip_stream(void);
const char *hclib_hip_version(void);
void hclib_hip_last_sched_counters(uint64_t out[16]);

typedef struct {
    uint64_t executed;
    uint64_t spawned;
    uint64_t batches;
    uint64_t chunks_pushed;
    uint64_t chunks_stolen;
    uint64_t items_stolen;
    uint64_t xcd;
    uint64_t reserved;
    uint64_t stolen_from[8];
} hclib_hip_wave_stats_t;
int hclib_hip_last_wave_stats(hclib_hip_wave_stats_t *out, int max);
void hclib_hip_last_narrow_counters(uint64_t out[4]);
void hclib_hip_last_shed_counters(uint64_t out[8]);
void hclib_hip_last_phase_counters(uint64_t out[8]);
int hclib_hip_last_timeline(uint64_t *out, uint64_t max_words, uint32_t *events_per_worker);

#define HCLIB_HIP_ATOMIC_SCATTER_RET64 0
#define HCLIB_HIP_ATOMIC_HOT_WORD 1
#define HCLIB_HIP_ATOMIC_COALESCED32 2
int hclib_hip_atomic_calibrate(int mode, int iters, double *mops_per_s, double *kernel_ms);
int hclib_hip_sparselu_bmod_rate(int B, int wgs_per_cu, int reps, double *ms, double *gflops);
int hclib_hip_sha1_calibrate(int chains, int waves_per_cu, int iters, double *sha1_per_s, double *kernel_ms);

typedef struct {
    void *hdr;
    uint32_t *seq;
    uint32_t *cnt;
    uint32_t *data;
    uint32_t nq, cap, chunk;
    void *globals;
    void *stream;
    int grid;
    int num_cus;
} hclib_hip_sched_launch_t;

int hclib_hip_sched_begin(uint32_t entry_words, uint32_t chunk, int waves_per_cu,
                          hclib_hip_sched_launch_t *out);
int hclib_hip_sched_end(const char *who, uint64_t counters[16], uint64_t maxes[4],
                        double *kernel_ms);

typedef struct {
    int low;
    int high;
    int stride;
    int tile;
} hclib_hip_loop_domain_t;

#define HCLIB_HIP_FORASYNC_FLAT 0
#define HCLIB_HIP_FORASYNC_RECURSIVE 1

#define HCLIB_HIP_BODY_TRIAD_F32 1
#define HCLIB_HIP_BODY_IOTA_CHECK 2
#define HCLIB_HIP_BODY_VISIT_COUNT 3

typedef struct {
    float *a;
    const float *b;
    const float *c;
    float s;
} hclib_hip_triad_args_t;

typedef struct {
    int *ran;
    int *errors;
} hclib_hip_iota_args_t;

typedef struct {
    int *counts;
    int base[3];
    int extent[3];
} hclib_hip_visit_args_t;

int hclib_hip_forasync(int body, const void *args, int dim, hclib_hip_loop_domain_t *domain,
                       int mode, void *stream);

int hclib_hip_forasync_triad_f32(float *a, const float *b, const float *c, float s, int64_t n,
                                 void *stream);

int hclib_hip_num_workers(void);

typedef struct {
    int first, count, stride, pad;
} hclib_hip_run_t;
typedef struct {
    const hclib_hip_run_t *runs[3];
    const int64_t *prefix[3];
    int nruns[3];
    int ndim;
    int64_t total;
    void *mem;
} hclib_hip_sweep_plan_t;
int hclib_hip_forasync_plan(int dim, hclib_hip_loop_domain_t *domain, int mode, void *stream,
                            hclib_hip_sweep_plan_t *plan);
int hclib_hip_forasync_plan_release(hclib_hip_sweep_plan_t *plan, void *stream);

#define HCLIB_HIP_ATOMIC_I32 0
#define HCLIB_HIP_ATOMIC_U32 1
#define HCLIB_HIP_ATOMIC_I64 2
#define HCLIB_HIP_ATOMIC_U64 3
#define HCLIB_HIP_ATOMIC_F32 4
#define HCLIB_HIP_ATOMIC_F64 5
#define HCLIB_HIP_ATOMIC_SUM 0
#define HCLIB_HIP_ATOMIC_MAX 1
#define HCLIB_HIP_ATOMIC_OR 2
#define HCLIB_HIP_ATOMIC_STRIDE 128

typedef struct hclib_hip_atomic hclib_hip_atomic_t;
typedef struct {
    void *slots;
    uint32_t nslots;
    uint32_t stride;
    int dtype, op;
} hclib_hip_atomic_view_t;

int hclib_hip_atomic_create(int dtype, int op, const void *default_value, hclib_hip_atomic_t **out);
int hclib_hip_atomic_destroy(hclib_hip_atomic_t *atomic);
int hclib_hip_atomic_view(const hclib_hip_atomic_t *atomic, hclib_hip_atomic_view_t *view);
int hclib_hip_atomic_gather(hclib_hip_atomic_t *atomic, void *stream, void *host_out);
int hclib_hip_atomic_gather_async(hclib_hip_atomic_t *atomic, void *stream, void *device_out);
int hclib_hip_atomic_reset(hclib_hip_atomic_t *atomic, void *stream);

int hclib_hip_forasync_reduce(hclib_hip_atomic_t *atomic, const void *x, int dim, hclib_hip_loop_domain_t *domain,
                              int mode, void *stream);

typedef struct {
    int type;
    int shape_fn;
    int gen_mx;
    int root_id;
    int non_leaf_bf;
    int compute_gran;
    double b_0;
    double non_leaf_prob;
    double shift_depth;
} hclib_hip_uts_params_t;

typedef struct {
    uint64_t nodes;
    uint64_t leaves;
    uint64_t max_depth;
    uint64_t chunks_pushed;
    uint64_t chunks_stolen;
    uint64_t batches;
    double kernel_ms;
    double busy_frac;
    double us_per_batch;
} hclib_hip_uts_result_t;

int hclib_hip_uts_search(const hclib_hip_uts_params_t *params, int shard, int nshards,
                         int split_depth, hclib_hip_uts_result_t *result, uint64_t *level_hist,
                         int max_levels);

typedef struct {
    int mode, feat, workers_per_group, grid, ring, seeded, seed_target, spill_lo, waves_per_cu;
} hclib_hip_uts_launch_t;
int hclib_hip_uts_last_launch(hclib_hip_uts_launch_t *out);

size_t hclib_hip_global_bytes(uint32_t cap);
int hclib_hip_global_alloc(uint32_t cap, int kind, void **region_out);
int hclib_hip_global_free(void *region);
int hclib_hip_global_init(void *region, uint32_t cap, int nranks);
int hclib_hip_global_attach(void *region, uint32_t cap, int rank);
int hclib_hip_global_read(const void *region, uint64_t out[35]);
int hclib_hip_ipc_export(void *dev_ptr, void *handle_out);
int hclib_hip_ipc_import(const void *handle, void **dev_ptr_out);
int hclib_hip_ipc_close(void *dev_ptr);
// ... 282 lines not shown
```

include/hclib_hip/hx_sched.h:

```cpp
#pragma once

#include <type_traits>

#include "hx_common.h"

namespace hx {

constexpr int kWaveSize = 64;

struct alignas(256) QueueHdr {
    uint32_t head;
    uint32_t done;
    uint32_t pad0[30];
    uint32_t tail;
    uint32_t pad1[31];
};

struct WaveStat {
    unsigned long long executed, spawned, batches, chunks_pushed, chunks_stolen, items_stolen;
    unsigned long long xcd;
    unsigned long long reserved;
    unsigned long long stolen_from[8];
};
static_assert(sizeof(WaveStat) == 128, "WaveStat is 16 words");

struct alignas(256) GlobalHdr {
    uint32_t active;
    uint32_t pad0[63];
    uint32_t idle;
    uint32_t pad1[63];
    uint32_t head;
    uint32_t pad2[63];
    uint32_t tail;
    uint32_t pad3[63];
    uint32_t err;
    uint32_t pad4[63];
    unsigned long long moved[32];
    uint32_t held[16];
};
constexpr int kGlobalMaxRanks = 16;

struct GlobalView {
    GlobalHdr *hdr;
    uint32_t *ctl;
    uint32_t *data;
    uint32_t cap;
    uint32_t rank;
};

struct alignas(256) SchedGlobals {
    uint32_t outstanding;
    uint32_t pad0[63];
    uint32_t hint;
    uint32_t pad1[63];
    uint32_t hints[8 * 64];
    uint32_t err;
    uint32_t pad2[63];
    unsigned long long counters[16];
    unsigned long long maxes[4];
    WaveStat *wave_stats;
    uint32_t wave_stats_cap;
    unsigned long long narrow[4];
    GlobalView gview;
    unsigned long long *timeline;
    uint32_t timeline_cap;
    unsigned long long *wave_ctr;
    uint32_t wave_ctr_cap;
    struct Seed {
        uint32_t *buf;
        uint32_t *ctl;
        uint32_t cap;
        uint32_t target;
        uint32_t max_levels;
        uint32_t min_levels;
        uint32_t solo_cap;
    } seed;
    unsigned long long shed[8];
};
constexpr int kSeedMaxLevels = 24;
constexpr int kSeedGoLines = 64;
constexpr int kSeedCtlLines = 2 * kSeedMaxLevels + 2 + kSeedGoLines;
constexpr int kWaveCtrWords = 40;
enum : int {
    kShedExits = 0,
    kShedPlaced = 1,
    kShedBlocks = 2,
    kShedItems = 3,
    kShedFallbacks = 4,
    kShedCounts = 5,
};

#ifndef HX_TIMELINE
#define HX_TIMELINE 0
#endif
enum : uint32_t {
    kTlStart = 1,
    kTlBusy = 2,
    kTlIdle = 3,
    kTlSpill = 4,
    kTlTerm = 5,
    kTlEnd = 6,
    kTlProbe = 7,
    kTlSeed = 8,
};
struct Timeline {
    unsigned long long *p;
    uint32_t n, cap;
    __device__ __forceinline__ void init(SchedGlobals *g, uint32_t worker) {
#if HX_TIMELINE
        cap = g->timeline_cap;
        p = g->timeline ? g->timeline + (size_t)worker * cap : nullptr;
        n = 0;
#endif
    }
    __device__ __forceinline__ void log(uint32_t type, uint32_t value) {
#if HX_TIMELINE
        if (p && n < cap && lane_id() == 0)
            p[n] = ((unsigned long long)__builtin_amdgcn_s_memrealtime() << 24) | ((unsigned long long)type << 20) |
                   (value & 0xfffffu);
        ++n;
#endif
    }
};

#ifndef HX_STAMPS
#define HX_STAMPS 0
#endif

enum : int {
    kCtrPushCycles = 4,
    kCtrClockTicks = 5,
    kCtrRealTicks = 6,
    kCtrFormCycles = 7,
    kCtrProcCycles = 8,
    kCtrBusyCycles = 9,
    kCtrIdleCycles = 10,
    kCtrSpillCycles = 11,
    kCtrWaves = 12,
    kCtrBatches = 13,
    kCtrPushed = 14,
    kCtrStolen = 15,
};

struct PoolView {
    QueueHdr *hdr;
    uint32_t *seq;
    uint32_t *cnt;
    uint32_t *data;
    uint32_t nq;
    uint32_t cap;
    uint32_t chunk;
};

struct SchedConfig {
    uint32_t spill_hi;
    uint32_t spill_lo;
    uint32_t spin_limit;
    uint32_t nwaves;
    uint32_t stamps;
    uint32_t hunger;
    uint32_t backoff = 16;
    uint32_t carry = 2;
    uint32_t defer = 1;
    uint32_t dual = 1;
    uint32_t spills = 0;
    uint32_t hunger_init_full = 0;
    uint32_t narrow_shed = 0;
};


constexpr uint32_t kResidualSplitMin = 2;

template <class K, class = void>
struct KindHasSeedProcess {
    static constexpr bool value = false;
};
template <class K>
struct KindHasSeedProcess<K, decltype((void)&K::seed_process)> {
    static constexpr bool value = true;
};
template <class K>
__device__ __forceinline__ int kind_seed_process(const typename K::Ctx &c, typename K::Acc &acc, const uint32_t *t,
                                                 uint32_t k, uint32_t *child, uint32_t *err, bool valid) {
    if constexpr (KindHasSeedProcess<K>::value) return K::seed_process(c, acc, t, k, child, err, valid);
    else return K::process(c, acc, t, k, child, err, valid);
}

template <class K, class = void>
struct KindPieces {
    static constexpr int value = 8;
};
template <class K>
struct KindPieces<K, decltype((void)K::kPieces)> {
    static constexpr int value = K::kPieces;
};
template <class K>
constexpr int pieces_of() { return KindPieces<K>::value; }
template <class K, class = void>
struct KindHasDual {
    static constexpr bool value = false;
};
template <class K>
struct KindHasDual<K, decltype((void)&K::process2)> {
    static constexpr bool value = K::kPure;
};
template <class K>
constexpr int group_max_of() { return KindPieces<K>::value + 2; }
template <class K, class = void>
struct KindFixedChildren {
    static constexpr bool value = false;
};
template <class K, class = void>
struct KindBulkCount {
    static constexpr bool value = false;
};
template <class K>
struct KindBulkCount<K, decltype((void)K::kBulkCount)> {
    static constexpr bool value = K::kBulkCount;
};
template <class K>
struct KindFixedChildren<K, decltype((void)K::kFixedChildren)> {
    static constexpr bool value = K::kFixedChildren;
};
constexpr uint32_t kMaxChildren = 1u << 24;

template <bool ON>
struct ShedSlots {};
template <>
struct ShedSlots<true> {
    unsigned long long shed_g;
    uint32_t shed_ib;
    uint32_t shed_wave;
    uint32_t shed_cfg;
    uint32_t shed_cnt[kShedCounts];
};

template <class Kind, int CAP>
struct WaveStack : ShedSlots<(CAP >= 1024)> {
    static constexpr int TW = Kind::kTmplWords;
    static_assert(TW == 2 || TW == 6, "templates are 2 or 6 words");
    static_assert((CAP & (CAP - 1)) == 0, "CAP must be a power of two");
    uint2 d[CAP];
    uint4 t0[TW == 6 ? CAP : 1];
    uint2 t1[CAP];
    uint32_t mark[64];
    uint32_t stolen_from[8];
    unsigned long long cyc[6];
    static constexpr bool kCarryLds = CAP >= 1024;
    uint4 cscr[kCarryLds ? 128 : 1];
};

template <class WS>
__device__ __forceinline__ void lds_sum(WS &st, int i, unsigned long long v) {
    if (lane_id() == 0) __hip_atomic_fetch_add(&st.cyc[i], v, __ATOMIC_RELAXED, __HIP_MEMORY_SCOPE_WAVEFRONT);
}

template <class Kind, int CAP>
__device__ __forceinline__ void load_tmpl(const WaveStack<Kind, CAP> &st, uint32_t slot, uint32_t *t) {
    if constexpr (Kind::kTmplWords == 6) {
        const uint4 a = st.t0[slot];
        const uint2 b = st.t1[slot];
        t[0] = a.x;
        t[1] = a.y;
        t[2] = a.z;
        t[3] = a.w;
        t[4] = b.x;
        t[5] = b.y;
    } else {
        const uint2 b = st.t1[slot];
        t[0] = b.x;
        t[1] = b.y;
    }
}
template <class Kind, int CAP>
__device__ __forceinline__ void store_tmpl(WaveStack<Kind, CAP> &st, uint32_t slot, const uint32_t *t) {
    if constexpr (Kind::kTmplWords == 6) {
        st.t0[slot] = make_uint4(t[0], t[1], t[2], t[3]);
        st.t1[slot] = make_uint2(t[4], t[5]);
    } else {
        st.t1[slot] = make_uint2(t[0], t[1]);
    }
}

__device__ __forceinline__ int wave_scan_add(int x) {
    x += __builtin_amdgcn_update_dpp(0, x, 0x111, 0xf, 0xf, false);
    x += __builtin_amdgcn_update_dpp(0, x, 0x112, 0xf, 0xf, false);
    x += __builtin_amdgcn_update_dpp(0, x, 0x114, 0xf, 0xf, false);
    x += __builtin_amdgcn_update_dpp(0, x, 0x118, 0xf, 0xf, false);
    x += __builtin_amdgcn_update_dpp(0, x, 0x142, 0xa, 0xf, false);
    x += __builtin_amdgcn_update_dpp(0, x, 0x143, 0xc, 0xf, false);
    return x;
}
__device__ __forceinline__ int imax(int a, int b) { return a > b ? a : b; }
__device__ __forceinline__ int wave_scan_max(int x) {
    x = imax(x, __builtin_amdgcn_update_dpp(-1, x, 0x111, 0xf, 0xf, false));
    x = imax(x, __builtin_amdgcn_update_dpp(-1, x, 0x112, 0xf, 0xf, false));
    x = imax(x, __builtin_amdgcn_update_dpp(-1, x, 0x114, 0xf, 0xf, false));
    x = imax(x, __builtin_amdgcn_update_dpp(-1, x, 0x118, 0xf, 0xf, false));
    x = imax(x, __builtin_amdgcn_update_dpp(-1, x, 0x142, 0xa, 0xf, false));
    x = imax(x, __builtin_amdgcn_update_dpp(-1, x, 0x143, 0xc, 0xf, false));
    return x;
}
__device__ __forceinline__ int lane63(int x) { return __builtin_amdgcn_readlane(x, 63); }

#ifndef HX_STRICT_HANDOFF
#define HX_STRICT_HANDOFF 0
#endif
__device__ __forceinline__ void handoff_publish() {
#if HX_STRICT_HANDOFF
    release_agent();
#else
    vm_drain();
#endif
}
__device__ __forceinline__ void handoff_consume() {
#if HX_STRICT_HANDOFF
    acquire_agent();
#else
    __builtin_amdgcn_fence(__ATOMIC_ACQUIRE, "wavefront");
#endif
}
__device__ __forceinline__ uint32_t lane0(uint32_t x) { return __builtin_amdgcn_readfirstlane(x); }

__device__ __forceinline__ uint32_t *slot_ctl(const PoolView &pool, uint32_t slot) { return pool.seq + 2u * slot; }

struct PendingChunk {
    uint32_t slot, pos, q;
    bool live;
};

template <int TW>
__device__ __forceinline__ void after_body(const uint32_t *child) {
    (void)child;
}

template <class Kind, int CAP>
__device__ __forceinline__ void publish_pending(const PoolView &pool, SchedGlobals *g, PendingChunk &pc) {
    if (!pc.live) return;
    handoff_publish();
    if (lane_id() == 0) {
        st_sc1_u32(slot_ctl(pool, pc.slot), pc.pos + 1);
        st_sc1_u32(&g->hints[64u * ((pc.q / (pool.nq / 8u)) & 7u)], pc.q);
    }
    pc.live = false;
}

template <class K, class = void>
struct kind_has_export : std::false_type {};
template <class K>
struct kind_has_export<K, decltype((void)&K::export_item)> : std::true_type {};
template <class Kind>
__device__ __forceinline__ void kind_export(const typename Kind::Ctx &ctx, uint32_t *w, bool valid, uint32_t *err) {
    if constexpr (kind_has_export<Kind>::value) Kind::export_item(ctx, w, valid, err);
}

template <class K, class = void>
struct kind_has_trace_item : std::false_type {};
template <class K>
struct kind_has_trace_item<K, decltype((void)&K::trace_item)> : std::true_type {};
template <class Kind>
__device__ __forceinline__ void kind_trace_item(const typename Kind::Ctx &ctx, const uint32_t *w, bool valid,
                                                uint32_t ev, bool via_inbox) {
    if constexpr (kind_has_trace_item<Kind>::value) Kind::trace_item(ctx, w, valid, ev, via_inbox);
}

template <class K, class = void>
struct kind_has_seed : std::false_type {};
template <class K>
struct kind_has_seed<K, decltype((void)&K::seeding)> : std::true_type {};

template <class K, class = void>
struct kind_has_drain : std::false_type {};
template <class K>
struct kind_has_drain<K, decltype((void)&K::drain)> : std::true_type {};
template <class K, class = void>
struct kind_has_renew : std::false_type {};
template <class K>
struct kind_has_renew<K, decltype((void)&K::renew)> : std::true_type {};
template <class Kind>
__device__ __forceinline__ void kind_drain(const typename Kind::Ctx &ctx, typename Kind::Acc &acc, uint32_t *err) {
    if constexpr (kind_has_drain<Kind>::value) Kind::drain(ctx, acc, err);
}

template <class Kind, int CAP>
__device__ bool enqueue_chunk(const typename Kind::Ctx &ctx, const PoolView &pool, SchedGlobals *g, uint32_t q,
                              WaveStack<Kind, CAP> &st, uint32_t bot, uint32_t n, uint32_t &occ, PendingChunk &pc,
                              bool defer, bool relief = false) {
    constexpr int W = Kind::kWords;
    const int lane = lane_id();
    QueueHdr *h = &pool.hdr[q];
    const bool valid = (uint32_t)lane < n;
    uint32_t w[W];
    {
        const uint32_t p = bot + (valid ? (uint32_t)lane : 0u);
        const uint2 dd = st.d[p & (CAP - 1)];
        load_tmpl<Kind, CAP>(st, (p - (dd.y >> 24)) & (CAP - 1), w);
        w[W - 2] = dd.x;
        w[W - 1] = dd.y & (kMaxChildren - 1);
    }
    uint32_t pos = 0, seen = 0;
    int ok = 0;
    const bool fast = occ < pool.cap / 4;
    if (lane == 0) {
        if (fast) {
            add_agent(&g->outstanding, 1u);
            pos = add_agent(&h->tail, 1u);
            seen = pos - ld_agent(&h->head);
            ok = 1;
        } else {
            const uint32_t hd = ld_agent(&h->head), tl = ld_agent(&h->tail);
            seen = tl - hd;
            if ((int)(tl - hd) < (int)(relief ? pool.cap - 1 : pool.cap / 2) && cas_agent(&h->tail, tl, tl + 1u)) {
                add_agent(&g->outstanding, 1u);
                pos = tl;
                ok = 1;
            }
        }
    }
    occ = lane0(seen);
    if (!lane0((uint32_t)ok)) return false;
    pos = lane0(pos);
    const uint32_t slot = q * pool.cap + (pos & (pool.cap - 1));
    if (lane == 0) {
        const unsigned long long t0 = __builtin_amdgcn_s_memrealtime();
        while (ld_agent(slot_ctl(pool, slot)) != pos) {
            if (__builtin_amdgcn_s_memrealtime() - t0 > 100000000ull) {
                dev_error(&g->err, kErrQueueFull);
                break;
            }
            __builtin_amdgcn_s_sleep(1);
        }
    }
    uint32_t *dst = pool.data + (size_t)slot * pool.chunk * W;
    {
        kind_export<Kind>(ctx, w, valid, &g->err);
        kind_trace_item<Kind>(ctx, w, valid, 2u, false);
        if (valid) {
            if constexpr (W % 4 == 0) {
#pragma unroll
                for (int i = 0; i < W; i += 4)
                    st_sc1_x4(&dst[(uint32_t)lane * W + i], make_uint4(w[i], w[i + 1], w[i + 2], w[i + 3]));
            } else {
#pragma unroll
                for (int i = 0; i < W; ++i) st_agent(&dst[(uint32_t)lane * W + i], w[i]);
            }
        }
    }
    if (lane == 0) st_sc1_u32(slot_ctl(pool, slot) + 1, n);
    if (defer) {
        pc.slot = slot;
        pc.pos = pos;
        pc.q = q;
        pc.live = true;
        return true;
    }
    handoff_publish();
    if (lane == 0) {
        st_sc1_u32(slot_ctl(pool, slot), pos + 1);
        st_sc1_u32(&g->hints[64u * ((q / (pool.nq / 8u)) & 7u)], q);
    }
    vm_drain();
    return true;
}

struct ProbeStats {
    uint32_t probes = 0, empty = 0, lost = 0, wait_us = 0;
};

template <class Kind, int CAP>
__device__ uint32_t dequeue_chunk(const typename Kind::Ctx &ctx, const PoolView &pool, uint32_t q, WaveStack<Kind, CAP> &st,
                                  SchedGlobals *g, uint32_t &done, ProbeStats &ps) {
    constexpr int W = Kind::kWords;
    const int lane = lane_id();
    QueueHdr *h = &pool.hdr[q];
    uint32_t pos = 0, fin = 0;
    int ok = 0, nonempty = 0;
    unsigned long long sc0 = 0;
    if (lane == 0) {
        const unsigned long long hd2 = ld_agent((const unsigned long long *)&h->head);
        const uint32_t hd = (uint32_t)hd2, tl = ld_agent(&h->tail);
        fin = (uint32_t)(hd2 >> 32);
        nonempty = (int)(tl - hd) > 0;
        if (nonempty) {
            sc0 = ld_agent((const unsigned long long *)slot_ctl(pool, q * pool.cap + (hd & (pool.cap - 1))));
            if (cas_agent(&h->head, hd, hd + 1)) {
                pos = hd;
                ok = 1;
            }
        }
    }
    done = lane0(fin);
    if (HX_TIMELINE) {
        ps.probes++;
        if (!lane0((uint32_t)nonempty)) ps.empty++;
        else if (!lane0((uint32_t)ok)) ps.lost++;
    }
    if (!lane0((uint32_t)ok)) return 0;
    pos = lane0(pos);
    const uint32_t slot = q * pool.cap + (pos & (pool.cap - 1));
    uint32_t cnt = 0;
    uint32_t waited = 0;
    if (lane == 0) {
        const unsigned long long t0 = __builtin_amdgcn_s_memrealtime();
        for (bool first = true;; first = false) {
            const unsigned long long sc = first ? sc0 : ld_agent((const unsigned long long *)slot_ctl(pool, slot));
            if ((uint32_t)sc == pos + 1) {
                cnt = (uint32_t)(sc >> 32);
                break;
            }
            if (__builtin_amdgcn_s_memrealtime() - t0 > 100000000ull) {
                dev_error(&g->err, kErrSpinTimeout);
                break;
            }
            __builtin_amdgcn_s_sleep(1);
        }
        if (HX_TIMELINE) waited = (uint32_t)((__builtin_amdgcn_s_memrealtime() - t0) / 100u);
    }
    if (HX_TIMELINE) ps.wait_us += lane0(waited);
    handoff_consume();
    const uint32_t n = lane0(cnt);
    const uint32_t *src = pool.data + (size_t)slot * pool.chunk * W;
    if ((uint32_t)lane < n) {
        uint32_t w[W];
        if constexpr (W == 8) {
            uint4 a, b;
            ld_sc1_x4x2(&src[(uint32_t)lane * W], a, b);
            w[0] = a.x, w[1] = a.y, w[2] = a.z, w[3] = a.w, w[4] = b.x, w[5] = b.y, w[6] = b.z, w[7] = b.w;
        } else {
#pragma unroll
            for (int i = 0; i < W; ++i) w[i] = ld_agent(&src[(uint32_t)lane * W + i]);
        }
        store_tmpl<Kind, CAP>(st, (uint32_t)lane, w);
        st.d[lane] = make_uint2(w[W - 2], w[W - 1]);
        kind_trace_item<Kind>(ctx, w, true, 3u, false);
    }
    vm_drain();
    if (lane == 0) st_sc1_u32(slot_ctl(pool, slot), pos + pool.cap);
    return n;
}

template <class Kind, int CAP>
__device__ bool global_enqueue(const typename Kind::Ctx &ctx, const GlobalView &gv, uint32_t words_per_chunk,
                               WaveStack<Kind, CAP> &st, uint32_t bot, uint32_t n, uint32_t *err) {
    constexpr int W = Kind::kWords;
    const int lane = lane_id();
    GlobalHdr *h = gv.hdr;
    uint32_t w[W];
    bool mv = true;
    if ((uint32_t)lane < n) {
        const uint32_t p = bot + (uint32_t)lane;
        const uint2 dd = st.d[p & (CAP - 1)];
        load_tmpl<Kind, CAP>(st, (p - (dd.y >> 24)) & (CAP - 1), w);
        w[W - 2] = dd.x;
        w[W - 1] = dd.y & (kMaxChildren - 1);
        mv = Kind::movable(ctx, w);
    }
    if (__ballot(!mv) != 0) return false;
    uint32_t pos = 0;
    int ok = 0;
    if (lane == 0) {
        const uint32_t hd = ld_sys(&h->head), tl = ld_sys(&h->tail);
        if ((int)(tl - hd) < (int)(gv.cap / 2)) {
            add_sys(&h->active, 1u);
            pos = add_sys(&h->tail, 1u);
            ok = 1;
        }
    }
    if (!lane0((uint32_t)ok)) return false;
    kind_export<Kind>(ctx, w, (uint32_t)lane < n, err);
    pos = lane0(pos);
    const uint32_t slot = pos & (gv.cap - 1);
    uint32_t *ctl = gv.ctl + 2u * slot;
    uint32_t timed_out = 0;
    if (lane == 0) {
        const unsigned long long t0 = __builtin_amdgcn_s_memrealtime();
        while (ld_sys(ctl) != pos) {
            if (__builtin_amdgcn_s_memrealtime() - t0 > 100000000ull) {
                dev_error(err, kErrQueueFull);
                dev_error_sys(&h->err, kErrQueueFull);
                timed_out = 1;
                break;
            }
            __builtin_amdgcn_s_sleep(2);
        }
    }
    if (lane0(timed_out)) return false;
    uint32_t *dst = gv.data + (size_t)slot * words_per_chunk;
    if ((uint32_t)lane < n) {
#pragma unroll
// ... 266 lines not shown
    NarrowState<Kind::kTmplWords> ns, uint32_t mu, uint32_t r_fix, uint32_t ck_fix) {
    constexpr int TW = Kind::kTmplWords;
    const typename Kind::Ctx ctx = ctx_ref;
    typename Kind::Acc acc = acc_ref;
    acc_set_mode(acc, 1u);
    const uint32_t lane = (uint32_t)lane_id();
    constexpr bool kBulk = KindBulkCount<Kind>::value;
    uint32_t carry = lane0(ns.carry), batches = 0, s_exec = 0, s_nsp = 0, t2;
    const uint32_t k = ck_fix;
    uint32_t ch2[TW];
    bool sp;
    unsigned long long sp2;
    while (true) {
    do {
        const bool h = lane < carry;
        if constexpr (kBulk) sp = Kind::process_bulk(ctx, acc, ns.ctmpl, k, ch2, err, h);
        else sp = Kind::process(ctx, acc, ns.ctmpl, k, ch2, err, h) > 0;
        ++batches;
        s_exec += carry;
        sp2 = __builtin_amdgcn_ballot_w64(sp);
        const uint32_t nsp = (uint32_t)__builtin_popcountll(sp2);
        s_nsp += nsp;
        t2 = mu * nsp;
        carry_lds_slot<TW>(st.cscr, sp2, sp, ch2, ns.ctmpl, r_fix);
        carry = t2;
    } while (t2 - 1u < (uint32_t)kWaveSize);
    if (t2 == 0) break;
    const uint32_t nsp = (uint32_t)__builtin_popcountll(sp2);
    uint32_t kept = 0, to_ring = 0;
    if constexpr (WPG > 1) kept = narrow_shed<Kind, CAP, WPG>(ctx, st, mu, nsp, r_fix, ck_fix, to_ring);
    carry = mu * kept;
    if (kept != 0 && to_ring == nsp) continue;
    const uint32_t rk2 = (uint32_t)__builtin_amdgcn_mbcnt_hi(
        (uint32_t)(sp2 >> 32), __builtin_amdgcn_mbcnt_lo((uint32_t)sp2, 0u));
    push_uniform<Kind, CAP>(st, ns.top, mu * (rk2 - to_ring), mu * (nsp - to_ring), mu, sp && rk2 >= to_ring, ch2);
    ns.top += mu * (nsp - to_ring);
    break;
    }
    ns.ck = ck_fix;
    if constexpr (kBulk) Kind::count_bulk(acc, s_exec, s_exec - s_nsp);
    if (lane == 0) {
        ns.n_exec += s_exec;
        ns.n_spawn += mu * s_nsp;
    }
    ns.carry = carry;
    ns.batches = batches;
    acc_set_mode(acc, 0u);
    acc_ref = acc;
    return ns;
}

template <class Kind, int CAP, int WPG = 1>
__device__ __forceinline__ NarrowState<Kind::kTmplWords> narrow_loop(
    const typename Kind::Ctx &ctx_ref, typename Kind::Acc &acc_ref, uint32_t *err, WaveStack<Kind, CAP> &st,
    NarrowState<Kind::kTmplWords> ns) {
    constexpr int TW = Kind::kTmplWords;
    constexpr int kPieces = pieces_of<Kind>();
    const typename Kind::Ctx ctx = ctx_ref;
    typename Kind::Acc acc = acc_ref;
    acc_set_mode(acc, 1u);
    const uint32_t lane = (uint32_t)lane_id();
    uint32_t carry = lane0(ns.carry), batches = 0;
    uint32_t mu_fix = 0, rcp_fix = 0;
    if constexpr (KindFixedChildren<Kind>::value) {
        mu_fix = lane0(Kind::fixed_children(ctx));
        if (mu_fix > (uint32_t)kPieces) mu_fix = 0;
        rcp_fix = mu_fix ? rcp16(mu_fix) : 0u;
    }
    const bool hoist = mu_fix != 0;
    const uint32_t r_fix = hoist ? __umul24(lane, rcp_fix) >> 16 : 0u;
    const uint32_t ck_fix = hoist ? lane - __umul24(r_fix, mu_fix) : 0u;
    if constexpr (KindFixedChildren<Kind>::value && Kind::kPure && Kind::kBoundedChildren &&
                  WaveStack<Kind, CAP>::kCarryLds) {
        if (hoist) return narrow_loop_fixed<Kind, CAP, WPG>(ctx_ref, acc_ref, err, st, ns, mu_fix, r_fix, ck_fix);
    }
    while (true) {
        const bool h = lane < carry;
        uint32_t ch2[TW];
        int c2 = 0;
        if constexpr (Kind::kPure) {
            c2 = Kind::process(ctx, acc, ns.ctmpl, ns.ck, ch2, err, h);
        } else {
            if (h) c2 = Kind::process(ctx, acc, ns.ctmpl, ns.ck, ch2, err, true);
        }
        ++batches;
        uint32_t u2 = c2 > 0 ? (uint32_t)c2 : 0u;
        if (!Kind::kBoundedChildren && u2 >= kMaxChildren) {
            dev_error(err, kErrBadTask);
            u2 = 0;
        }
        ns.n_exec += h ? 1u : 0u;
        ns.n_spawn += h ? u2 : 0u;
        const uint32_t n2 = u2 > (uint32_t)kPieces ? (uint32_t)kPieces : u2;
        const unsigned long long sp2 = __ballot(n2 != 0);
        if (!sp2) {
            carry = 0;
            break;
        }
        uint32_t mu2;
        bool uni2;
        if (KindFixedChildren<Kind>::value && mu_fix) {
            mu2 = mu_fix;
            uni2 = true;
        } else {
            mu2 = (uint32_t)__builtin_amdgcn_readlane((int)n2, __builtin_ctzll(sp2));
            uni2 = __ballot(u2 > (uint32_t)kPieces || (n2 != 0 && n2 != mu2)) == 0;
        }
        if (uni2) {
            const uint32_t t2 = mu2 * (uint32_t)__builtin_popcountll(sp2);
            if (t2 <= (uint32_t)kWaveSize) {
                if constexpr (WaveStack<Kind, CAP>::kCarryLds) {
                    if (hoist) {
                        carry_lds_slot<TW>(st.cscr, sp2, ((sp2 >> lane) & 1ull) != 0, ch2, ns.ctmpl, r_fix);
                        ns.ck = ck_fix;
                    } else {
                        carry_lds<TW>(st.cscr, sp2, mu2, ch2, ns.ctmpl, ns.ck, rcp_fix);
                    }
                }
                else carry_permute<TW>(sp2, mu2, n2, ch2, ns.ctmpl, ns.ck, rcp_fix);
                carry = t2;
                continue;
            }
            const uint32_t rk2 = (uint32_t)__builtin_amdgcn_mbcnt_hi(
                (uint32_t)(sp2 >> 32), __builtin_amdgcn_mbcnt_lo((uint32_t)sp2, 0u));
            push_uniform<Kind, CAP>(st, ns.top, mu2 * rk2, t2, mu2, n2 != 0, ch2);
            ns.top += t2;
        } else {
            const int P2 = wave_scan_add((int)n2);
            const uint32_t t2 = (uint32_t)lane63(P2);
            push_outputs<Kind, CAP>(st, ns.top, (uint32_t)(P2 - (int)n2), t2, 0u, u2, n2, ns.ctmpl, ch2, ns.ck,
                                    ns.ck + 1, ns.tag);
            ns.tag += 16;
            ns.top += t2;
        }
        carry = 0;
        break;
    }
    ns.carry = carry;
    ns.batches = batches;
    acc_set_mode(acc, 0u);
    acc_ref = acc;
    return ns;
}

template <class Kind>
struct Inbox {
    uint32_t state;
    uint32_t n;
    uint32_t idle;
    uint32_t pad;
    uint32_t w[64 * Kind::kWords];
};

template <class Kind>
__device__ __forceinline__ uint32_t inbox_claim(Inbox<Kind> &ib) {
    uint32_t ok = 0;
    if (lane_id() == 0) ok = lds_cas(&ib.state, 0u, 2u) ? 1u : 0u;
    return ok;
}

template <class Kind>
__device__ __forceinline__ void inbox_fill(const typename Kind::Ctx &ctx, Inbox<Kind> &ib, uint32_t *w, bool valid,
                                           uint32_t n, SchedGlobals *g) {
    constexpr int W = Kind::kWords;
    kind_export<Kind>(ctx, w, valid, &g->err);
    kind_trace_item<Kind>(ctx, w, valid, 2u, true);
    if (valid) {
        hx_lds_u32 *dst = (hx_lds_u32 *)&ib.w[(uint32_t)lane_id() * W];
#pragma unroll
        for (int i = 0; i < W; ++i) dst[i] = w[i];
    }
    asm volatile("" ::: "memory");
    if (lane_id() == 0) {
        add_agent(&g->outstanding, 1u);
        lds_store(&ib.n, n);
        lds_store(&ib.idle, 0u);
        lds_store(&ib.state, 1u);
    }
}

template <class Kind, int CAP>
__device__ bool inbox_put(const typename Kind::Ctx &ctx, Inbox<Kind> &ib, WaveStack<Kind, CAP> &st, uint32_t bot,
                          uint32_t n, SchedGlobals *g) {
    constexpr int W = Kind::kWords;
    const int lane = lane_id();
    const bool valid = (uint32_t)lane < n;
    const uint32_t p = bot + (valid ? (uint32_t)lane : 0u);
    const uint2 dd = st.d[p & (CAP - 1)];
    const uint32_t ok = inbox_claim<Kind>(ib);
    uint32_t w[W];
    load_tmpl<Kind, CAP>(st, (p - (dd.y >> 24)) & (CAP - 1), w);
    if (!lane0(ok)) return false;
    w[W - 2] = dd.x;
    w[W - 1] = dd.y & (kMaxChildren - 1);
    inbox_fill<Kind>(ctx, ib, w, valid, n, g);
    return true;
}

template <class Kind, int CAP, int WPG>
__device__ __forceinline__ uint32_t narrow_shed(const typename Kind::Ctx &ctx, WaveStack<Kind, CAP> &st, uint32_t mu,
                                                uint32_t nsp, uint32_t r_fix, uint32_t ck_fix, uint32_t &to_ring) {
    constexpr int TW = Kind::kTmplWords, W = Kind::kWords;
    const uint32_t lane = (uint32_t)lane_id();
    to_ring = 0;
    const uint32_t cfg = lane0(lds_load(&st.shed_cfg));
    const uint32_t rule = cfg & 0xffu, max_blocks = (cfg >> 8) & 0xffu;
    if (rule == 0) return 0;
    const uint32_t fit = (64u * rcp16(mu)) >> 16;
    uint32_t keep = rule == 2 ? fit : (rule == 3 ? nsp / 4 : nsp / 2);
    keep = keep > fit ? fit : (keep == 0 ? 1u : keep);
    const uint32_t wave = lane0(lds_load(&st.shed_wave));
    typedef __attribute__((address_space(3))) Inbox<Kind> lds_inbox;
    Inbox<Kind> *ib = (Inbox<Kind> *)(lds_inbox *)(uintptr_t)lane0(lds_load(&st.shed_ib));
    const unsigned long long gp = st.shed_g;
    SchedGlobals *g = (SchedGlobals *)(((unsigned long long)lane0((uint32_t)(gp >> 32)) << 32) | lane0((uint32_t)gp));
    uint32_t sid[WPG], sst[WPG];
#pragma unroll
    for (uint32_t a = 1; a < (uint32_t)WPG; ++a) {
        sid[a] = lds_load(&ib[(wave + a) % (uint32_t)WPG].idle);
        sst[a] = lds_load(&ib[(wave + a) % (uint32_t)WPG].state);
    }
    const uint32_t nshed = nsp - keep;
    uint32_t placed = 0, blocks = 0;
#pragma unroll
    for (uint32_t a = 1; a < (uint32_t)WPG; ++a) {
        if (placed < nshed && blocks < max_blocks && lane0(sid[a]) == 1u && lane0(sst[a]) == 0u) {
            Inbox<Kind> &to = ib[(wave + a) % (uint32_t)WPG];
            const uint32_t bs = nshed - placed < fit ? nshed - placed : fit, n = bs * mu;
            const bool valid = lane < n;
            const uint32_t ok = inbox_claim<Kind>(to);
            uint32_t w[W];
            carry_lds_read<TW>(st.cscr, keep + placed + (valid ? r_fix : 0u), w);
            if (lane0(ok)) {
                w[W - 2] = ck_fix;
                w[W - 1] = ck_fix + 1u;
                inbox_fill<Kind>(ctx, to, w, valid, n, g);
                placed += bs;
                ++blocks;
            }
        }
    }
    to_ring = keep + placed;
    if (lane == 0) {
        st.shed_cnt[kShedExits] += 1u;
        st.shed_cnt[placed == nshed ? kShedPlaced : kShedFallbacks] += 1u;
        st.shed_cnt[kShedBlocks] += blocks;
        st.shed_cnt[kShedItems] += placed * mu;
    }
    return keep;
}

template <class Kind, int CAP>
__device__ uint32_t inbox_take(const typename Kind::Ctx &ctx, Inbox<Kind> &ib, WaveStack<Kind, CAP> &st) {
    constexpr int W = Kind::kWords;
    const int lane = lane_id();
    if (lane0(lds_load(&ib.state)) != 1u) return 0;
    const uint32_t n = lane0(lds_load(&ib.n));
    if ((uint32_t)lane < n) {
        uint32_t w[W];
#pragma unroll
        for (int i = 0; i < W; ++i) w[i] = ib.w[(uint32_t)lane * W + i];
        store_tmpl<Kind, CAP>(st, (uint32_t)lane, w);
        st.d[lane] = make_uint2(w[W - 2], w[W - 1]);
        kind_trace_item<Kind>(ctx, w, true, 3u, true);
    }
    if (lane == 0) lds_store(&ib.state, 0u);
    return n;
}

template <bool GLOBAL>
__device__ __forceinline__ void wave_goes_idle(SchedGlobals *g, const GlobalView &gv, const PoolView &pool) {
    if (lane_id() != 0) return;
    if constexpr (GLOBAL) {
        const uint32_t prev = __hip_atomic_fetch_add(&g->outstanding, (uint32_t)-1, __ATOMIC_RELEASE, HX_AGENT);
        if (prev == 1u) {
            add_sys(&gv.hdr->idle, 1u);
            __hip_atomic_store(&gv.hdr->held[gv.rank], 0u, __ATOMIC_RELEASE, __HIP_MEMORY_SCOPE_SYSTEM);
            add_sys(&gv.hdr->active, (uint32_t)-1);
        }
    } else {
        const uint32_t prev = __hip_atomic_fetch_add(&g->outstanding, (uint32_t)-1, __ATOMIC_RELEASE, HX_AGENT);
        if (prev == 1u) {
            for (uint32_t q = 0; q < pool.nq; ++q) st_agent(&pool.hdr[q].done, 1u);
        }
    }
}

#ifndef HX_SEED_FENCES
#define HX_SEED_FENCES 0
#endif
template <class Kind, int CAP>
__device__ uint32_t seed_levels(const typename Kind::Ctx &ctx, typename Kind::Acc &acc, SchedGlobals *g,
                                WaveStack<Kind, CAP> &st, uint32_t gid, uint32_t nw, uint32_t spin_limit_ms,
                                uint32_t &n_exec, uint32_t &n_spawn, uint32_t &nbatch, Timeline &tl) {
    static_assert(Kind::kPure, "breadth-first seeding runs slots branch-free");
    constexpr int TW = Kind::kTmplWords, W = Kind::kWords;
    static_assert(TW == 6 && W == 8, "seeding moves 32-byte slots {6-word template, k, k + 1}");
    const int lane = lane_id();
    const auto &sd = g->seed;
    uint32_t *ctl = sd.ctl;
    auto line = [&](int i) { return ctl + 64 * i; };
    uint32_t *go = line(2 * kSeedMaxLevels + 2 + (int)(gid % kSeedGoLines));
    uint32_t *err = &g->err;
    const unsigned long long t0 = __builtin_amdgcn_s_memrealtime();
    auto wait_ge = [&](uint32_t *p, uint32_t want) -> bool {
        uint32_t v = 0;
        for (uint32_t n = 0;; ++n) {
            if (lane == 0) v = ld_agent(p);
            if (lane0(v) >= want) return true;
            if ((n & 63) == 63) {
                if (__builtin_amdgcn_s_memrealtime() - t0 > 100000ull * spin_limit_ms) {
                    if (lane == 0) dev_error(err, kErrSpinTimeout);
                    return false;
                }
                uint32_t e = 0;
                if (lane == 0) e = ld_agent(err);
                if (lane0(e)) return false;
            }
            __builtin_amdgcn_s_sleep(1);
        }
    };
    constexpr uint32_t kSoloCap = (uint32_t)(CAP - 64) / 2;
    constexpr uint32_t kScr = 2 * kSoloCap;
    static_assert(kSoloCap >= 64, "the solo levels need ring room");
    uint32_t mtag = 1u << 20;
    auto run_slots = [&](const uint32_t (&tmpl)[TW], uint32_t k, bool valid, uint32_t *dst, uint32_t lds_out,
                         auto &&alloc) -> bool {
        uint32_t child[TW];
        const int nc = kind_seed_process<Kind>(ctx, acc, tmpl, k, child, err, valid);
        ++nbatch;
        const uint32_t u = valid && nc > 0 ? (uint32_t)nc : 0u;
        n_exec += valid ? 1u : 0u;
        n_spawn += u;
        const int S = wave_scan_add((int)u);
        const uint32_t tot = (uint32_t)lane63(S), excl = (uint32_t)S - u;
        const uint32_t base = alloc(tot);
        st.t0[kScr + lane] = make_uint4(child[0], child[1], child[2], child[3]);
        st.t1[kScr + lane] = make_uint2(child[4], child[5]);
        st.d[kScr + lane] = make_uint2(excl, u);
        asm volatile("" ::: "memory");
        if (base + tot > sd.cap) {
            if (lane == 0) dev_error(err, kErrStackOverflow);
            return false;
        }
        int owner = 0;
        for (uint32_t r0 = 0; r0 < tot; r0 += 64) {
            ++mtag;
            if (u && excl >= r0 && excl < r0 + 64u) st.mark[excl - r0] = (mtag << 6) | (uint32_t)lane;
            const uint32_t mk = st.mark[lane];
            const int sc = wave_scan_max((mk >> 6) == mtag ? (int)(mk & 63u) : -1);
            const int prev = owner;
            owner = (int)lane63(sc >= 0 ? sc : prev);
            const uint32_t o = r0 + (uint32_t)lane;
            if (o < tot) {
                const int lo = sc >= 0 ? sc : prev;
                const uint32_t j = o - st.d[kScr + lo].x;
                const uint4 t0 = st.t0[kScr + lo];
                const uint2 t1 = st.t1[kScr + lo];
                uint32_t *q = dst + (size_t)(base + o) * W;
                st_sc1_x4(q, t0);
                st_sc1_x4(q + 4, make_uint4(t1.x, t1.y, j, j + 1));
                if (lds_out != ~0u && base + o < kSoloCap) {
                    st.t0[lds_out + base + o] = t0;
                    st.t1[lds_out + base + o] = t1;
                    st.d[lds_out + base + o] = make_uint2(j, j + 1);
                }
            }
        }
        asm volatile("" ::: "memory");
        return true;
    };
    auto buf = [&](int d) { return sd.buf + (size_t)(d & 1) * sd.cap * W; };
    auto stop = [&](uint32_t E, int d) {
        return E == 0 || d >= (int)sd.max_levels || d + 1 >= kSeedMaxLevels ||
               (E >= sd.target && d >= (int)sd.min_levels);
    };
    uint32_t E = 0;
    int d = 0;
    if (gid == 0) {
        uint32_t tmpl[TW];
        const int rn = Kind::roots(ctx, acc, tmpl);
        E = rn > 0 ? ((uint32_t)rn < sd.cap ? (uint32_t)rn : sd.cap) : 0u;
        for (uint32_t e = (uint32_t)lane; e < E; e += 64) {
            uint32_t *q = buf(0) + (size_t)e * W;
            st_sc1_x4(q, make_uint4(tmpl[0], tmpl[1], tmpl[2], tmpl[3]));
            st_sc1_x4(q + 4, make_uint4(tmpl[4], tmpl[5], e, e + 1));
            if (e < kSoloCap) {
                st.t0[e] = make_uint4(tmpl[0], tmpl[1], tmpl[2], tmpl[3]);
                st.t1[e] = make_uint2(tmpl[4], tmpl[5]);
                st.d[e] = make_uint2(e, e + 1);
            }
        }
        asm volatile("" ::: "memory");
        uint32_t in = 0, out = kSoloCap;
        bool ok = true;
        const uint32_t solo = sd.solo_cap && sd.solo_cap < kSoloCap ? sd.solo_cap : kSoloCap;
        while (ok && !stop(E, d) && E <= solo) {
            uint32_t cnt = 0;
            auto alloc = [&](uint32_t tot) {
                const uint32_t b0 = cnt;
                cnt += tot;
                return b0;
            };
            for (uint32_t b = 0; b * 64 < E && ok; ++b) {
                const uint32_t e = b * 64 + (uint32_t)lane;
                const bool valid = e < E;
                const uint32_t src = in + (valid ? e : 0u);
                const uint4 a = st.t0[src];
                const uint2 c = st.t1[src];
                const uint32_t t[TW] = {a.x, a.y, a.z, a.w, c.x, c.y};
                ok = run_slots(t, st.d[src].x, valid, buf(d + 1), out, alloc);
            }
            E = cnt;
            ++d;
            const uint32_t x = in;
            in = out;
            out = x;
            tl.log(kTlSeed, (uint32_t)d);
        }
        vm_drain();
        if (HX_SEED_FENCES) release_agent();
        for (uint32_t i = (uint32_t)lane; i < (uint32_t)kSeedGoLines; i += 64) {
            unsigned long long *gl = (unsigned long long *)(line(2 * kSeedMaxLevels + 2 + (int)i) + kSeedMaxLevels);
            st_agent(gl, (unsigned long long)(E + 1) | ((unsigned long long)(uint32_t)d << 32));
        }
        vm_drain();
        if (!ok) return 0;
    }
    if (!wait_ge(go + kSeedMaxLevels, 1u)) return 0;
    if (HX_SEED_FENCES) acquire_agent();
    if (lane == 0) {
        const unsigned long long r = ld_agent((const unsigned long long *)(go + kSeedMaxLevels));
        E = (uint32_t)r - 1u;
        d = (int)(r >> 32);
    }
    E = lane0(E);
    d = (int)lane0((uint32_t)d);
    for (; !stop(E, d); ++d) {
        const uint32_t nblk = (E + 63) / 64;
        unsigned long long *word = (unsigned long long *)line(2 * d + 1);
        auto alloc = [&](uint32_t tot) {
            unsigned long long b0 = 0;
            if (lane == 0 && tot) b0 = add_agent(word, (unsigned long long)tot);
            return (uint32_t)lane0((uint32_t)b0);
        };
        bool ok = true;
        for (uint32_t b = gid; b < nblk && ok; b += nw) {
            const uint32_t e = b * 64 + (uint32_t)lane;
            const bool valid = e < E;
            uint4 s0, s1;
            ld_sc1_x4x2(buf(d) + (size_t)(valid ? e : 0u) * W, s0, s1);
            const uint32_t t[TW] = {s0.x, s0.y, s0.z, s0.w, s1.x, s1.y};
            ok = run_slots(t, s1.z, valid, buf(d + 1), ~0u, alloc);
        }
        if (!ok) return 0;
        const uint32_t P = nblk < nw ? nblk : nw;
        if (gid < P) {
            vm_drain();
            unsigned long long prev = 0;
            if (lane == 0) prev = __hip_atomic_fetch_add(word, 1ull << 32, __ATOMIC_ACQ_REL, HX_AGENT);
            const uint32_t done = lane0((uint32_t)(prev >> 32)) + 1u;
            const uint32_t e1 = lane0((uint32_t)prev) + 1u;
            if (done == P) {
                if (HX_SEED_FENCES) release_agent();
                for (uint32_t i = (uint32_t)lane; i < (uint32_t)kSeedGoLines; i += 64)
                    st_agent(line(2 * kSeedMaxLevels + 2 + (int)i) + d, e1);
            }
        }
        if (!wait_ge(go + d, 1u)) return 0;
        if (HX_SEED_FENCES) acquire_agent();
        uint32_t e2 = 0;
        if (lane == 0) e2 = ld_agent(go + d);
        E = lane0(e2) - 1u;
        tl.log(kTlSeed, (uint32_t)d + 1u);
    }
    if (E > sd.cap) E = sd.cap;
    const uint32_t lo = (uint32_t)(((unsigned long long)E * gid) / nw),
                   hi = (uint32_t)(((unsigned long long)E * (gid + 1)) / nw);
    const uint32_t n = hi - lo;
    constexpr uint32_t kMax = CAP / 2;
    if (n > kMax) {
        if (lane == 0) dev_error(err, kErrStackOverflow);
        return 0;
    }
    const uint32_t *src = buf(d);
    for (uint32_t i0 = 0; i0 < n; i0 += 64) {
        const uint32_t i = i0 + (uint32_t)lane;
        uint4 a, c;
        ld_sc1_x4x2(src + (size_t)(lo + (i < n ? i : 0u)) * W, a, c);
        if (i < n) {
            const uint32_t w[W] = {a.x, a.y, a.z, a.w, c.x, c.y, c.z, c.w};
            store_tmpl<Kind, CAP>(st, i, w);
            st.d[i] = make_uint2(w[W - 2], w[W - 1]);
        }
    }
    return n;
}

template <class Kind, int CAP>
__device__ __forceinline__ uint32_t push_root(WaveStack<Kind, CAP> &st, uint32_t *err, const uint32_t *tmpl, int n,
                                              int lane, uint32_t tag) {
    constexpr int kPieces = pieces_of<Kind>();
    uint32_t ucnt = lane == 0 && n > 0 ? (uint32_t)n : 0u;
    if (ucnt >= kMaxChildren) {
        dev_error(err, kErrBadTask);
        ucnt = 0;
    }
    const uint32_t nch = ucnt > (uint32_t)kPieces ? (uint32_t)kPieces : ucnt;
    const uint32_t tout = lane0(nch);
    push_outputs<Kind, CAP>(st, 0, 0, tout, 0, ucnt, nch, tmpl, tmpl, 0, 0, tag);
    return tout;
}

template <class Kind, int CAP, bool GLOBAL = false, int WPG = 1>
__device__ void run_worker(const typename Kind::Ctx &ctx, const PoolView &pool, SchedGlobals *g,
                           const SchedConfig &cfg, WaveStack<Kind, CAP> &st, bool seed_roots,
                           Inbox<Kind> *ib = nullptr, uint32_t wave = 0, uint32_t worker = 0xffffffffu) {
    constexpr int TW = Kind::kTmplWords;
    constexpr uint32_t M = CAP - 1;
    constexpr int kPieces = pieces_of<Kind>();
    constexpr int kGroupMax = group_max_of<Kind>();
    constexpr uint32_t kRoom = CAP - kGroupMax;
    static_assert(CAP >= kWaveSize * kGroupMax + kGroupMax, "ring must hold one batch's pushes");
    const int lane = lane_id();
    const uint32_t gid = worker != 0xffffffffu ? worker : blockIdx.x;
    GlobalView gv;
    if constexpr (GLOBAL) gv = g->gview;
    uint32_t gidle_pf = 0, gidle = 0;
    const uint32_t qpx = pool.nq / 8;
    const uint32_t xcc = xcc_id() & 7u;
    const uint32_t home = xcc * qpx + (gid / 8) % qpx;
    uint32_t rng = 0x9e3779b9u ^ (gid * 0x85ebca6bu + 1u);

    typename Kind::Acc acc;
    acc_set_wid(acc, gid);
    Timeline tl;
    tl.init(g, gid);
    tl.log(kTlStart, 0);
    ProbeStats pstat;
    uint32_t bot = 0, top = 0;
    bool active = false;
    uint32_t spins = 0;
    unsigned long long idle_since = 0;
    uint32_t nbatch = 0, npush = 0, nsteal = 0;
    unsigned long long cyc_form = 0, cyc_proc = 0, cyc_push = 0;
    unsigned long long ph_sum[6] = {0, 0, 0, 0, 0, 0}, ph_n = 0, ph_a = 0, ph_b = 0, ph_c = 0, ph_d = 0, ph_m = 0,
                       ph_p = 0;
    bool ph_single = false;
    uint32_t tag = 1;
    for (int i = lane; i < kWaveSize; i += kWaveSize) st.mark[i] = 0;
    if (lane < 8) st.stolen_from[lane] = 0;
    constexpr bool kShed = WPG > 1 && WaveStack<Kind, CAP>::kCarryLds;
    if constexpr (kShed) {
        if (lane == 0) {
            st.shed_g = (unsigned long long)(uintptr_t)g;
            st.shed_ib = (uint32_t)(uintptr_t)(__attribute__((address_space(3))) Inbox<Kind> *)ib;
            st.shed_wave = wave;
            st.shed_cfg = cfg.narrow_shed;
        }
        if (lane < kShedCounts) st.shed_cnt[lane] = 0;
    }
    uint32_t n_exec = 0, n_spawn = 0;
    uint32_t items_stolen = 0;
    uint32_t n_narrow = 0, n_narrow_in = 0;
    uint32_t carry = 0, ck = 0;
    uint32_t ctmpl[TW];
    PendingChunk pend;
    pend.live = false;
    uint32_t occ = 0;
#pragma unroll
    for (int i = 0; i < TW; ++i) ctmpl[i] = 0;

    bool seeded = false;
    if constexpr (Kind::kPure && Kind::kTmplWords == 6 && Kind::kWords == 8 && CAP >= 128) {
        if (g->seed.buf) {
            seeded = true;
            top = seed_levels<Kind, CAP>(ctx, acc, g, st, gid, cfg.nwaves, cfg.spin_limit, n_exec, n_spawn, nbatch, tl);
            st.mark[lane] = 0;
            active = true;
            tl.log(kTlBusy, top);
            if (top == 0) {
                active = false;
                wave_goes_idle<GLOBAL>(g, gv, pool);
            }
        }
    }
    if constexpr (kind_has_seed<Kind>::value) {
        if (!seeded && Kind::seeding(ctx)) {
            seeded = true;
            top = lane0(Kind::seed(ctx, acc, st, gid, cfg.nwaves, cfg.spin_limit, &g->err));
            active = true;
            tl.log(kTlBusy, top);
            if (top == 0) {
                active = false;
                wave_goes_idle<GLOBAL>(g, gv, pool);
            }
        }
    }
    if (seed_roots && !seeded) {
        uint32_t tmpl[TW];
        const int n = Kind::roots(ctx, acc, tmpl);
        const uint32_t tout = push_root<Kind, CAP>(st, &g->err, tmpl, n, lane, tag);
        tag += 16;
        top = tout;
        active = true;
        tl.log(kTlBusy, tout);
        if (top == 0) {
            active = false;
            wave_goes_idle<GLOBAL>(g, gv, pool);
        }
    }

    unsigned long long t_mark = __builtin_amdgcn_s_memtime();
    if (lane < 6) st.cyc[lane] = 0;
    if (lane == 0) {
        st.cyc[4] = t_mark;
        st.cyc[5] = __builtin_amdgcn_s_memrealtime();
    }
    unsigned long long t_batch = t_mark;
    bool busy_phase = true;
    uint32_t outst_pf = seeded && cfg.hunger_init_full ? cfg.nwaves : 0u;
    uint32_t outst_cur = 0, hunger_in = 0;
    vm_drain();
    while (true) {
        top = lane0(top);
        bot = lane0(bot);
        carry = lane0(carry);
        const uint32_t size = top - bot;
        if (size == 0 && carry == 0) {
            publish_pending<Kind, CAP>(pool, g, pend);
            if (busy_phase) {
                const unsigned long long now = __builtin_amdgcn_s_memtime();
                lds_sum(st, 0, now - t_mark);
                t_mark = now;
                busy_phase = false;
            }
            if (active) {
                kind_drain<Kind>(ctx, acc, &g->err);
                if constexpr (kind_has_renew<Kind>::value) {
                    uint32_t tmpl[TW];
                    const int rn = Kind::renew(ctx, acc, tmpl);
                    if (rn > 0) {
                        bot = 0;
                        top = push_root<Kind, CAP>(st, &g->err, tmpl, rn, lane, tag);
                        tag += 16;
                        if (top) {
                            tl.log(kTlBusy, top);
                            const unsigned long long now = __builtin_amdgcn_s_memtime();
                            lds_sum(st, 1, now - t_mark);
                            t_mark = now;
                            t_batch = now;
                            busy_phase = true;
                            continue;
                        }
                    }
                }
                active = false;
                wave_goes_idle<GLOBAL>(g, gv, pool);
                tl.log(kTlIdle, 0);
                if constexpr (WPG > 1) {
                    if (lane == 0) lds_store(&ib[wave].idle, 1u);
                }
            }
            uint32_t n = 0, src = 0;
            uint32_t q = home;
            if constexpr (WPG > 1) {
                n = inbox_take<Kind, CAP>(ctx, ib[wave], st);
                if (n) src = 3;
            }
            uint32_t fin = 0;
            if (n == 0) {
                const uint32_t phase = spins % 3;
                if (phase == 1) {
                    uint32_t hq = 0;
                    if (lane == 0) hq = ld_agent(&g->hints[64u * ((xcc + spins / 3u) & 7u)]);
                    q = lane0(hq) % pool.nq;
                } else if (phase == 2) {
                    uint32_t r = lane0(xorshift(rng));
                    q = ((r & 3) != 0) ? xcc * qpx + (r >> 2) % qpx : (r >> 2) % pool.nq;
                }
                n = dequeue_chunk<Kind, CAP>(ctx, pool, q, st, g, fin, pstat);
                src = q == home ? 1 : 2;
            }
            if constexpr (!GLOBAL) {
                if (fin) {
                    tl.log(kTlTerm, 0);
                    break;
                }
            }
            if constexpr (WPG > 1) {
                if (n && lane == 0) lds_store(&ib[wave].idle, 0u);
            }
            if constexpr (GLOBAL) {
                if (n == 0 && (spins & 3) == 3) {
                    n = global_dequeue<Kind, CAP>(gv, pool.chunk * (uint32_t)Kind::kWords, st, &g->err);
                    if (n && lane == 0) {
                        const uint32_t prev = add_agent(&g->outstanding, 1u);
                        if (prev == 0u) {
                            const unsigned long long t0 = __builtin_amdgcn_s_memrealtime();
                            while (true) {
                                uint32_t z = 0u;
                                if (__hip_atomic_compare_exchange_strong(&gv.hdr->held[gv.rank], &z, 1u,
                                                                         __ATOMIC_ACQUIRE, __ATOMIC_RELAXED,
                                                                         __HIP_MEMORY_SCOPE_SYSTEM))
                                    break;
                                if (__builtin_amdgcn_s_memrealtime() - t0 > 100000000ull) {
                                    dev_error(&g->err, kErrSpinTimeout);
                                    dev_error_sys(&gv.hdr->err, kErrSpinTimeout);
                                    break;
                                }
                                __builtin_amdgcn_s_sleep(1);
// ... 162 lines not shown
                const int P = wave_scan_add(nout);
                tout = (uint32_t)lane63(P);
                const uint32_t excl = (uint32_t)(P - nout);
                if (!make_room(tout)) break;
                push_group<Kind, CAP>(st, top + excl, nresA, uA, nchA, tA, cA, kA, kendA);
                push_group<Kind, CAP>(st, top + excl + nresA + nchA, nresB, uB, nchB, tB, cB, kB, kendB);
                top += tout;
            }
        }
        if (!dual) {
        const uint32_t room = (uint32_t)kWaveSize - carry;
        const uint32_t take_ring = size < room ? size : room;
        const uint32_t take = carry + take_ring;
        const bool has = (uint32_t)lane < take;
        uint32_t tmpl[TW], child[TW];
        uint32_t k = 0, kend = 0;
        int cnt = 0;
        unsigned long long ts0 = 0;
        if (HX_STAMPS && cfg.stamps) ts0 = __builtin_amdgcn_s_memtime();
        if (HX_PHASES) {
            ph_b = __builtin_amdgcn_s_memtime();
            ph_single = true;
        }
        if ((uint32_t)lane < carry || take_ring == 0) {
#pragma unroll
            for (int i = 0; i < TW; ++i) tmpl[i] = ctmpl[i];
            k = ck;
            kend = ck + 1;
        } else if (Kind::kPure || has) {
            const uint32_t p = top - 1 - ((uint32_t)lane - carry);
            const uint2 dd = st.d[p & M];
            k = dd.x;
            kend = has ? dd.y & (kMaxChildren - 1) : k + 1;
            load_tmpl<Kind, CAP>(st, (p - (dd.y >> 24)) & M, tmpl);
        }
        carry = 0;
        if (HX_PHASES) {
            asm volatile("s_waitcnt lgkmcnt(0)" ::: "memory");
            ph_c = __builtin_amdgcn_s_memtime();
        }
        unsigned long long tsl = 0;
        if (HX_STAMPS && cfg.stamps) {
            asm volatile("s_waitcnt lgkmcnt(0)" ::: "memory");
            tsl = __builtin_amdgcn_s_memtime();
            cyc_form += tsl - t_batch;
            ts0 = tsl;
        }
        if constexpr (Kind::kPure) {
            cnt = Kind::process(ctx, acc, tmpl, k, child, &g->err, has);
        } else {
            if (has) cnt = Kind::process(ctx, acc, tmpl, k, child, &g->err, true);
        }
        after_body<TW>(child);
        if (HX_PHASES) {
#pragma unroll
            for (int i = 0; i < TW; ++i) asm volatile("" ::"v"(child[i]));
            ph_d = __builtin_amdgcn_s_memtime();
        }
        publish_pending<Kind, CAP>(pool, g, pend);
        if (HX_STAMPS && cfg.stamps) {
            const unsigned long long ts1 = __builtin_amdgcn_s_memtime();
            cyc_proc += ts1 - tsl;
        }
        top -= take_ring;
        const uint32_t rlen = has ? kend - k - 1u : 0u;
        const uint32_t nres = rlen == 0 ? 0u : (rlen < kResidualSplitMin ? 1u : 2u);
        uint32_t ucnt = cnt > 0 ? (uint32_t)cnt : 0u;
        n_exec += has ? 1u : 0u;
        n_spawn += has ? ucnt : 0u;
        if (!Kind::kBoundedChildren && ucnt >= kMaxChildren) {
            dev_error(&g->err, kErrBadTask);
            ucnt = 0;
        }
        const uint32_t nch = ucnt > (uint32_t)kPieces ? (uint32_t)kPieces : ucnt;
        const unsigned long long spawn = __ballot(nch != 0);
        const uint32_t mu = spawn ? (uint32_t)__builtin_amdgcn_readlane((int)nch, __builtin_ctzll(spawn)) : 0u;
        const bool uniform = __ballot(nres != 0 || ucnt > (uint32_t)kPieces || (nch != 0 && nch != mu)) == 0;
        uint32_t excl;
        int nout = 0;
        if (uniform) {
            excl = mu * (uint32_t)__builtin_amdgcn_mbcnt_hi((uint32_t)(spawn >> 32),
                                                            __builtin_amdgcn_mbcnt_lo((uint32_t)spawn, 0u));
            tout = mu * (uint32_t)__builtin_popcountll(spawn);
        } else {
            nout = (int)(nres + nch);
            const int P = wave_scan_add(nout);
            tout = (uint32_t)lane63(P);
            excl = (uint32_t)(P - nout);
        }
        {
            const uint32_t hungry0 = cfg.nwaves > outst ? cfg.nwaves - outst : 0;
            if (cfg.carry && uniform && tout > 0 && tout <= (uint32_t)kWaveSize &&
                !(hungry0 > 0 && (top - bot) + tout >= cfg.spill_lo)) {
                if constexpr (WaveStack<Kind, CAP>::kCarryLds) carry_lds<TW>(st.cscr, spawn, mu, child, ctmpl, ck);
                else carry_permute<TW>(spawn, mu, nch, child, ctmpl, ck);
                carry = tout;
                if (HX_STAMPS && cfg.stamps) cyc_push += __builtin_amdgcn_s_memtime() - ts0;
                if (HX_STAMPS && cfg.stamps) t_batch = __builtin_amdgcn_s_memtime();
                if (cfg.carry > 1 && top == bot && cfg.spill_lo > (uint32_t)kWaveSize && !(HX_STAMPS && cfg.stamps)) {
                    const unsigned long long tn0 = __builtin_amdgcn_s_memtime();
                    NarrowState<TW> ns;
#pragma unroll
                    for (int i = 0; i < TW; ++i) ns.ctmpl[i] = ctmpl[i];
                    ns.ck = ck;
                    ns.carry = carry;
                    ns.top = top;
                    ns.tag = tag;
                    ns.n_exec = n_exec;
                    ns.n_spawn = n_spawn;
                    ns.batches = 0;
                    ns = narrow_loop<Kind, CAP, WPG>(ctx, acc, &g->err, st, ns);
#pragma unroll
                    for (int i = 0; i < TW; ++i) ctmpl[i] = ns.ctmpl[i];
                    ck = ns.ck;
                    carry = lane0(ns.carry);
                    top = lane0(ns.top);
                    tag = lane0(ns.tag);
                    n_exec = ns.n_exec;
                    n_spawn = ns.n_spawn;
                    nbatch += lane0(ns.batches);
                    n_narrow += lane0(ns.batches);
                    lds_sum(st, 3, __builtin_amdgcn_s_memtime() - tn0);
                    ++n_narrow_in;
                }
                continue;
            }
        }
        if (HX_PHASES) ph_m = __builtin_amdgcn_s_memtime();
        if (!make_room(tout)) break;
        if (uniform) {
            push_uniform<Kind, CAP>(st, top, excl, tout, mu, nch != 0, child);
        } else {
            push_outputs<Kind, CAP>(st, top, excl, tout, nres, ucnt, nch, tmpl, child, k, kend, tag);
            tag += 16;
        }
        top += tout;
        if (HX_STAMPS && cfg.stamps) cyc_push += __builtin_amdgcn_s_memtime() - ts0;
        }
        if (HX_PHASES) ph_p = __builtin_amdgcn_s_memtime();
        uint32_t sz = top - bot;
        uint32_t hungry = cfg.nwaves > outst ? cfg.nwaves - outst : 0;
        const uint32_t lo = cfg.spill_lo;
        if (sz > cfg.spill_hi || (hungry > 0 && sz >= lo)) {
            const unsigned long long ts = __builtin_amdgcn_s_memtime();
            const uint32_t cmax = pool.chunk;
            uint32_t nsp = 0;
            while (sz > cfg.spill_hi || (hungry > 0 && sz >= lo)) {
                uint32_t n = (sz + 1) / 2;
                if (n > cmax) n = cmax;
                if (n == 0 || n == sz) break;
                bool ok = false;
                if constexpr (WPG > 1) {
                    uint32_t sid[WPG], sst[WPG];
#pragma unroll
                    for (uint32_t a = 1; a < (uint32_t)WPG; ++a) {
                        sid[a] = lds_load(&ib[(wave + a) % (uint32_t)WPG].idle);
                        sst[a] = lds_load(&ib[(wave + a) % (uint32_t)WPG].state);
                    }
#pragma unroll
                    for (uint32_t a = 1; a < (uint32_t)WPG; ++a)
                        if (!ok && lane0(sid[a]) == 1u && lane0(sst[a]) == 0u)
                            ok = inbox_put<Kind, CAP>(ctx, ib[(wave + a) % (uint32_t)WPG], st, bot, n, g);
                }
                if (!ok) publish_pending<Kind, CAP>(pool, g, pend);
                for (uint32_t a = 0; a < qpx && !ok; ++a) {
                    const uint32_t q = xcc * qpx + (home - xcc * qpx + a) % qpx;
                    ok = enqueue_chunk<Kind, CAP>(ctx, pool, g, q, st, bot, n, occ, pend, cfg.defer != 0);
                }
                if (!ok) break;
                ++npush;
                tl.log(kTlSpill, n);
                bot += n;
                sz = top - bot;
                if (hungry) --hungry;
                if (cfg.spills && ++nsp >= cfg.spills && sz <= cfg.spill_hi) break;
            }
            lds_sum(st, 2, __builtin_amdgcn_s_memtime() - ts);
        }
        if constexpr (GLOBAL) {
            if (hungry == 0 && (int)gidle > 0 && sz >= cfg.spill_lo) {
                uint32_t n = (sz + 1) / 2;
                if (n > pool.chunk) n = pool.chunk;
                publish_pending<Kind, CAP>(pool, g, pend);
                if (n > 0 && n < sz &&
                    global_enqueue<Kind, CAP>(ctx, gv, pool.chunk * (uint32_t)Kind::kWords, st, bot, n, &g->err)) {
                    bot += n;
                    sz = top - bot;
                    --gidle;
                }
            }
        }
        if (HX_STAMPS && cfg.stamps) t_batch = __builtin_amdgcn_s_memtime();
        if (HX_PHASES && ph_single) {
            const unsigned long long ph_e = __builtin_amdgcn_s_memtime();
            ph_sum[0] += ph_b - ph_a;
            ph_sum[1] += ph_c - ph_b;
            ph_sum[2] += ph_d - ph_c;
            ph_sum[3] += ph_e - ph_d;
            ph_sum[4] += ph_m - ph_d;
            ph_sum[5] += ph_p - ph_m;
            ++ph_n;
        }
    }
    publish_pending<Kind, CAP>(pool, g, pend);
    if constexpr (WPG > 1) {
        if (lane == 0) {
            lds_store(&ib[wave].idle, 0u);
            (void)lds_cas(&ib[wave].state, 0u, 3u);
        }
    }
    const unsigned long long t_end = __builtin_amdgcn_s_memtime();
    const unsigned long long rt_end = __builtin_amdgcn_s_memrealtime();
    lds_sum(st, busy_phase ? 0 : 1, t_end - t_mark);
    __builtin_amdgcn_s_waitcnt(0xC07F);
    const unsigned long long cyc_busy = st.cyc[0], cyc_idle = st.cyc[1], cyc_spill = st.cyc[2],
                             cyc_narrow = st.cyc[3], t_begin = st.cyc[4], rt_begin = st.cyc[5];
    unsigned long long shed_v = 0;
    if constexpr (kShed) {
        if (lane >= 32 && lane < 32 + kShedCounts) shed_v = st.shed_cnt[lane - 32];
    }
    if (active) {
        wave_goes_idle<GLOBAL>(g, gv, pool);
    }
    const bool rec = g->wave_ctr && gid < g->wave_ctr_cap;
    unsigned long long kc[8] = {0, 0, 0, 0, 0, 0, 0, 0}, km[4] = {0, 0, 0, 0};
    if constexpr (acc_has_totals<typename Kind::Acc>::value) {
        acc.totals(kc, km);
        if (!rec && lane == 0) {
            for (int i = 0; i < 8; ++i)
                if (kc[i]) add_agent(&g->counters[i], kc[i]);
            for (int i = 0; i < 4; ++i)
                if (km[i]) __hip_atomic_fetch_max(&g->maxes[i], km[i], __ATOMIC_RELAXED, HX_AGENT);
        }
    } else {
        acc.flush(g);
    }
    {
        const unsigned long long ex = wave_sum((unsigned long long)n_exec),
                                 sp = wave_sum((unsigned long long)n_spawn);
        if (g->wave_stats && gid < g->wave_stats_cap && lane < 16) {
            unsigned long long v = 0;
            switch (lane) {
            case 0: v = ex; break;
            case 1: v = sp; break;
            case 2: v = nbatch; break;
            case 3: v = npush; break;
            case 4: v = nsteal; break;
            case 5: v = items_stolen; break;
            case 6: v = xcc; break;
            case 7: v = 0; break;
            default: v = st.stolen_from[lane - 8]; break;
            }
            ((unsigned long long *)&g->wave_stats[gid])[lane] = v;
        }
    }
    const unsigned long long c_push = (HX_STAMPS && cfg.stamps) ? cyc_push - cyc_proc : 0,
                             c_form = (HX_STAMPS && cfg.stamps) ? cyc_form : 0,
                             c_proc = (HX_STAMPS && cfg.stamps) ? cyc_proc : 0;
    if (rec) {
        unsigned long long v = shed_v;
#pragma unroll
        for (int i = 0; i < 8; ++i)
            if (lane == i) v = kc[i];
#pragma unroll
        for (int i = 0; i < 4; ++i)
            if (lane == 16 + i) v = km[i];
        switch (lane) {
        case 8 + kCtrProcCycles - 8: v = c_proc; break;
        case 8 + kCtrBusyCycles - 8: v = cyc_busy; break;
        case 8 + kCtrIdleCycles - 8: v = cyc_idle; break;
        case 8 + kCtrSpillCycles - 8: v = cyc_spill; break;
        case 8 + kCtrWaves - 8: v = 1; break;
        case 8 + kCtrBatches - 8: v = nbatch; break;
        case 8 + kCtrPushed - 8: v = npush; break;
        case 8 + kCtrStolen - 8: v = nsteal; break;
        case 20: v = n_narrow_in ? (unsigned long long)n_narrow : 0; break;
        case 21: v = n_narrow_in ? cyc_narrow : 0; break;
        case 22: v = n_narrow_in; break;
        case 23: v = ph_n; break;
        case 28: v = ph_sum[0]; break;
        case 29: v = ph_sum[1]; break;
        case 30: v = ph_sum[2]; break;
        case 31: v = ph_sum[3]; break;
        case 24 + kCtrPushCycles - 4: v = HX_PHASES ? ph_sum[4] : c_push; break;
        case 24 + kCtrClockTicks - 4: v = t_end - t_begin; break;
        case 24 + kCtrRealTicks - 4: v = rt_end - rt_begin; break;
        case 24 + kCtrFormCycles - 4: v = HX_PHASES ? ph_sum[5] : c_form; break;
        default: break;
        }
        if (lane < kWaveCtrWords) g->wave_ctr[(size_t)gid * kWaveCtrWords + lane] = v;
    } else {
        if (shed_v) add_agent(&g->shed[lane - 32], shed_v);
        if (lane == 0 && n_narrow_in) {
            add_agent(&g->narrow[0], (unsigned long long)n_narrow);
            add_agent(&g->narrow[1], cyc_narrow);
            add_agent(&g->narrow[2], (unsigned long long)n_narrow_in);
        }
        if (lane == 0) {
            add_agent(&g->counters[kCtrBusyCycles], cyc_busy);
            if (HX_STAMPS && cfg.stamps) {
                add_agent(&g->counters[kCtrFormCycles], c_form);
                add_agent(&g->counters[kCtrProcCycles], c_proc);
                add_agent(&g->counters[kCtrPushCycles], c_push);
            }
            add_agent(&g->counters[kCtrIdleCycles], cyc_idle);
            add_agent(&g->counters[kCtrSpillCycles], cyc_spill);
            add_agent(&g->counters[kCtrWaves], 1ull);
            add_agent(&g->counters[kCtrBatches], (unsigned long long)nbatch);
            add_agent(&g->counters[kCtrPushed], (unsigned long long)npush);
            add_agent(&g->counters[kCtrStolen], (unsigned long long)nsteal);
            add_agent(&g->counters[kCtrClockTicks], t_end - t_begin);
            add_agent(&g->counters[kCtrRealTicks], rt_end - rt_begin);
        }
    }
    tl.log(kTlEnd, 0);
    if (HX_TIMELINE) {
        auto sat = [](uint32_t v) { return v / 16u > 0xffffu ? 0xffffu : v / 16u; };
        tl.log(kTlProbe, 0u << 16 | sat(pstat.probes));
        tl.log(kTlProbe, 1u << 16 | sat(pstat.empty));
        tl.log(kTlProbe, 2u << 16 | sat(pstat.lost));
        tl.log(kTlProbe, 3u << 16 | sat(pstat.wait_us));
    }
}

}
```

Baseline: 4.371 billion nodes/s.

## Add per-workgroup comm wave that drains outboxes into global deques for workers

Adds an extra wave per multi-wave workgroup that serves two LDS outboxes. Worker waves hand off give-away and narrow-shed blocks to these outboxes instead of publishing to global queues themselves. The comm wave either redirects a block to an idle sibling's inbox or enqueues it to the global pool. This takes global-queue latency off the worker waves' critical path, at the cost of an extra wave per block, more LDS use, and new counters.

```diff
diff --git a/hclib_amd/__init__.py b/hclib_amd/__init__.py
--- a/hclib_amd/__init__.py
+++ b/hclib_amd/__init__.py
@@ -224,7 +224,7 @@
     "hclib_hip_num_workers", "hclib_hip_uts_search", "hclib_hip_uts_num_children_host",
     "hclib_hip_uts_bucket_check", "hclib_hip_sha1_calibrate",
     "hclib_hip_fib", "hclib_hip_sw", "hclib_hip_last_sched_counters", "hclib_hip_last_narrow_counters",
-    "hclib_hip_last_phase_counters", "hclib_hip_last_shed_counters",
+    "hclib_hip_last_phase_counters", "hclib_hip_last_shed_counters", "hclib_hip_last_comm_counters",
     "hclib_hip_sw_band_begin", "hclib_hip_sw_band_rows", "hclib_hip_sw_band_end",
     "hclib_hip_sw_edges", "hclib_hip_sw_band_bottoms",
     "hclib_hip_atomic_create", "hclib_hip_atomic_destroy", "hclib_hip_atomic_view",
@@ -1259,6 +1259,13 @@
     return dict(zip(("exits", "placed", "blocks", "items", "fallbacks"), out))
 
 
+def last_comm_counters():
+    out = (C.c_uint64 * 8)()
+    lib().hclib_hip_last_comm_counters(out)
+    return dict(zip(("main_blocks", "main_items", "shed_blocks", "shed_items", "to_deque", "to_sibling", "busy",
+                     "ring_exits"), out))
+
+
 TIMELINE_EVENTS = {1: "start", 2: "busy", 3: "idle", 4: "spill", 5: "term", 6: "end"}
 
 
diff --git a/hclib_amd/csrc/hx_module.h b/hclib_amd/csrc/hx_module.h
--- a/hclib_amd/csrc/hx_module.h
+++ b/hclib_amd/csrc/hx_module.h
@@ -50,6 +50,8 @@
     unsigned long long last_counters[16] = {};
     unsigned long long last_narrow[4] = {};
     unsigned long long last_shed[8] = {};
+    unsigned long long last_comm[8] = {};
+    int comm_wpg = 0;
     unsigned long long last_phase[8] = {};
     WaveStat *wave_stats = nullptr;
     uint32_t wave_stats_cap = 0;
diff --git a/hclib_amd/csrc/hx_uts_plan.h b/hclib_amd/csrc/hx_uts_plan.h
--- a/hclib_amd/csrc/hx_uts_plan.h
+++ b/hclib_amd/csrc/hx_uts_plan.h
@@ -35,7 +35,20 @@
     int hunger = kUnset;
     int spin_limit_ms = 20000, stamps = 0, carry = 2, backoff = 16, defer = 1, spills_per_batch = 0;
     int narrow_shed = 1, narrow_shed_sibs = 3;
+    int uts_comm = 2;
 };
+
+constexpr int uts_block_waves(int wpg, bool global) { return wpg + (wpg > 1 && !global ? 1 : 0); }
+
+inline bool uts_comm_valid(int comm, std::string &err) {
+    if (comm >= 0 && comm <= 7) return true;
+    char buf[160];
+    snprintf(buf, sizeof(buf),
+             "hclib_hip_uts_search: HCLIB_HIP_UTS_COMM=%d is not a set of the outbox's users (0..7: 1 give-away, 2 "
+             "narrow shed, 4 redirect)", comm);
+    err = buf;
+    return false;
+}
 
 struct UtsPlan {
     int status = HCLIB_HIP_OK;
@@ -50,6 +63,8 @@
     uint32_t nq = 0, deque_cap = 0, chunk = 0;
     uint32_t spill_hi = 0, spill_lo = 0, spin_limit = 0, nwaves = 0, stamps = 0, hunger = 0, backoff = 0, carry = 0,
              defer = 0, dual = 0, spills = 0, hunger_init_full = 0, narrow_shed = 0;
+    uint32_t comm = 0;
+    int block = 64;
     uint32_t seed_target = 0, seed_max_levels = 0, seed_min_levels = 0, seed_solo_cap = 0;
     hclib_hip_uts_launch_t launch = {-1, 0, 0, 0, 0, 0, 0, 0, 0};
 };
@@ -72,6 +87,10 @@
     constexpr int U = UtsKnobs::kUnset;
     (void)shard;
     UtsPlan P;
+    if (!uts_comm_valid(kn.uts_comm, err)) {
+        P.status = HCLIB_HIP_EINVAL;
+        return P;
+    }
     const int trace_kind = max_levels > 0 ? kn.uts_trace : 0;
     const bool trace = trace_kind != 0;
 
@@ -233,6 +252,9 @@
         if (P.wpg != 2 && P.wpg != 4) P.wpg = 1;
         if (grid % P.wpg) P.wpg = 1;
     }
+    if (P.wpg > 1 && uts_block_waves(P.wpg, global) > P.wpg) P.comm = (uint32_t)kn.uts_comm;
+    if (kn.chunk < 64) P.comm &= ~2u;
+    P.block = 64 * (P.wpg + (P.comm ? 1 : 0));
     P.launch = hclib_hip_uts_launch_t{mode, trace ? 1 + trace_kind : P.feat, P.wpg, grid, P.ring, P.seed_target ? 1 : 0, (int)P.seed_target,
                                       (int)P.spill_lo, P.waves_per_cu};
     return P;
diff --git a/hclib_amd/csrc/module.hip b/hclib_amd/csrc/module.hip
--- a/hclib_amd/csrc/module.hip
+++ b/hclib_amd/csrc/module.hip
@@ -258,6 +258,8 @@
             if (r[16 + i] > host_copy->maxes[i]) host_copy->maxes[i] = r[16 + i];
         for (int i = 0; i < 3; ++i) host_copy->narrow[i] += r[20 + i];
         for (int i = 0; i < kShedCounts; ++i) host_copy->shed[i] += r[32 + i];
+        if (m.comm_wpg > 1 && w % (uint32_t)m.comm_wpg < 2)
+            for (int i = 0; i < 3; ++i) host_copy->comm[3 * (w % (uint32_t)m.comm_wpg) + i] += r[37 + i];
         m.last_phase[0] += r[23];
         for (int i = 0; i < 4; ++i) m.last_phase[1 + i] += r[28 + i];
         m.last_phase[5] += r[24];
@@ -266,6 +268,13 @@
     memcpy(m.last_counters, host_copy->counters, sizeof(m.last_counters));
     memcpy(m.last_narrow, host_copy->narrow, sizeof(m.last_narrow));
     memcpy(m.last_shed, host_copy->shed, sizeof(m.last_shed));
+    {
+        const unsigned long long *c = host_copy->comm;
+        const unsigned long long u[kCommCounts] = {c[0] & 0xffffffffull, c[0] >> 32, c[1] & 0xffffffffull, c[1] >> 32,
+                                                   c[2], c[3], c[4], c[5]};
+        memcpy(m.last_comm, u, sizeof(m.last_comm));
+        m.comm_wpg = 0;
+    }
     uint64_t nw = host_copy->counters[kCtrWaves];
     if (nw > nw_cap) nw = nw_cap;
     m.last_waves.resize(nw);
@@ -366,6 +375,10 @@
 
 void hclib_hip_last_shed_counters(uint64_t out[8]) {
     for (int i = 0; i < 8; ++i) out[i] = g_mod.last_shed[i];
+}
+
+void hclib_hip_last_comm_counters(uint64_t out[8]) {
+    for (int i = 0; i < 8; ++i) out[i] = g_mod.last_comm[i];
 }
 
 int hclib_hip_last_wave_stats(hclib_hip_wave_stats_t *out, int max) {
diff --git a/hclib_amd/csrc/uts.hip b/hclib_amd/csrc/uts.hip
--- a/hclib_amd/csrc/uts.hip
+++ b/hclib_amd/csrc/uts.hip
@@ -250,12 +250,16 @@
 };
 
 template <int MODE, int FEAT, int CAP = (MODE == kUtsBin ? 1024 : 512), bool GLOBAL = false, int WPG = 1>
-__global__ __launch_bounds__(64 * WPG) void k_uts_search(UtsCtx ctx, PoolView pool, SchedGlobals *g,
-                                                         SchedConfig cfg) {
+__global__ __launch_bounds__(64 * uts_block_waves(WPG, GLOBAL)) void k_uts_search(UtsCtx ctx, PoolView pool,
+                                                                                  SchedGlobals *g, SchedConfig cfg) {
     constexpr int kUtsCap = CAP;
+    constexpr bool kComm = uts_block_waves(WPG, GLOBAL) > WPG;
     using K = UtsKind<MODE, FEAT, CAP>;
     __shared__ WaveStack<K, kUtsCap> st[WPG];
-    __shared__ Inbox<K> ib[WPG];
+    __shared__ WgBoxes<K, WPG> bx;
+    static_assert(sizeof(st) + sizeof(bx) + (MODE == kUtsBin ? 0 : sizeof(s_rules) + sizeof(s_thr)) <= 160 * 1024,
+                  "a workgroup's rings, boxes and rule tables fit a CU's LDS");
+    Inbox<K> *ib = bx.ib;
     const uint32_t wave = WPG > 1 ? threadIdx.x / 64 : 0;
     const uint32_t worker = blockIdx.x * WPG + wave;
     if (WPG > 1) {
@@ -264,6 +268,14 @@
             ib[threadIdx.x].idle = 0;
         }
     }
+    if constexpr (WPG > 1) {
+        if (threadIdx.x < kOutboxes) bx.out[threadIdx.x].state = 0;
+        if (threadIdx.x < 6) bx.ctl.cnt[threadIdx.x] = 0;
+        if (threadIdx.x == 0) {
+            bx.ctl.on = kComm && blockDim.x > 64u * WPG ? (cfg.narrow_shed >> 16) & 7u : 0u;
+            bx.ctl.left = 0;
+        }
+    }
     if (MODE == kUtsGeoFixed) {
         for (int i = threadIdx.x; i < 128; i += 64 * WPG) s_thr[i] = ctx.thr[i];
         for (int i = threadIdx.x; i < kUtsBuckets / 4; i += 64 * WPG) s_thr[128 + i] = ctx.nb[i];
@@ -273,7 +285,17 @@
         for (int i = threadIdx.x; i < ctx.nthr; i += 64 * WPG) s_thr[i] = ctx.thr[i];
     }
     __syncthreads();
+    if constexpr (kComm) {
+        if (wave == (uint32_t)WPG) {
+            comm_wave<K, kUtsCap, WPG>(ctx, pool, g, cfg, bx, st[0]);
+            return;
+        }
+    }
     run_worker<K, kUtsCap, GLOBAL, WPG>(ctx, pool, g, cfg, st[wave], worker == 0, ib, wave, worker);
+    if constexpr (kComm) {
+        if (threadIdx.x % 64 == 0)
+            __hip_atomic_fetch_add((hx_lds_u32 *)&bx.ctl.left, 1u, __ATOMIC_RELAXED, __HIP_MEMORY_SCOPE_WORKGROUP);
+    }
 }
 
 static int uts_tables(const hclib_hip_uts_params_t &p, UtsTables &T) {
@@ -383,6 +405,7 @@
     k.spills_per_batch = env_int("HCLIB_HIP_SPILLS_PER_BATCH", k.spills_per_batch);
     k.narrow_shed = env_int("HCLIB_HIP_NARROW_SHED", k.narrow_shed);
     k.narrow_shed_sibs = env_int("HCLIB_HIP_NARROW_SHED_SIBS", k.narrow_shed_sibs);
+    k.uts_comm = env_int("HCLIB_HIP_UTS_COMM", k.uts_comm);
     return k;
 }
 
@@ -423,6 +446,13 @@
         set_error("hclib_hip_uts_search: invalid arguments");
         return HCLIB_HIP_EINVAL;
     }
+    {
+        std::string why;
+        if (!uts_comm_valid(knobs.uts_comm, why)) {
+            set_error("%s", why.c_str());
+            return HCLIB_HIP_EINVAL;
+        }
+    }
     HX_TRY(ensure_device());
     Module &m = mod();
     static struct {
@@ -520,15 +550,16 @@
     cfg.dual = plan.dual;
     cfg.spills = plan.spills;
     cfg.hunger_init_full = plan.hunger_init_full;
-    cfg.narrow_shed = plan.narrow_shed;
+    cfg.narrow_shed = plan.narrow_shed | plan.comm << 16;
     SeedCfg seed{plan.seed_target, plan.seed_max_levels, (uint32_t)UtsKind<kUtsBin, 0>::kWords, plan.seed_min_levels};
     seed.solo_cap = plan.seed_solo_cap;
     HX_TRY(reset_sched(pool, 1, plan.global, (uint32_t)plan.grid, seed.target ? &seed : nullptr));
     g_last_launch = plan.launch;
     SchedGlobals gl;
     float ms = 0;
-    const int rc = launch_sched((const void *)kern, plan.grid / plan.wpg, 64 * plan.wpg, who, [&] {
-        hipLaunchKernelGGL(kern, dim3(plan.grid / plan.wpg), dim3(64 * plan.wpg), 0, m.stream, ctx, pool, m.globals, cfg);
+    m.comm_wpg = plan.comm ? plan.wpg : 0;
+    const int rc = launch_sched((const void *)kern, plan.grid / plan.wpg, plan.block, who, [&] {
+        hipLaunchKernelGGL(kern, dim3(plan.grid / plan.wpg), dim3(plan.block), 0, m.stream, ctx, pool, m.globals, cfg);
     }, &gl, &ms);
     if (rc != HCLIB_HIP_OK) return rc;
     if (max_levels) {
diff --git a/include/hclib_hip.h b/include/hclib_hip.h
--- a/include/hclib_hip.h
+++ b/include/hclib_hip.h
@@ -39,6 +39,7 @@
 int hclib_hip_last_wave_stats(hclib_hip_wave_stats_t *out, int max);
 void hclib_hip_last_narrow_counters(uint64_t out[4]);
 void hclib_hip_last_shed_counters(uint64_t out[8]);
+void hclib_hip_last_comm_counters(uint64_t out[8]);
 void hclib_hip_last_phase_counters(uint64_t out[8]);
 int hclib_hip_last_timeline(uint64_t *out, uint64_t max_words, uint32_t *events_per_worker);
 
diff --git a/include/hclib_hip/hx_sched.h b/include/hclib_hip/hx_sched.h
--- a/include/hclib_hip/hx_sched.h
+++ b/include/hclib_hip/hx_sched.h
@@ -76,6 +76,7 @@
         uint32_t solo_cap;
     } seed;
     unsigned long long shed[8];
+    unsigned long long comm[8];
 };
 constexpr int kSeedMaxLevels = 24;
 constexpr int kSeedGoLines = 64;
@@ -88,6 +89,22 @@
     kShedItems = 3,
     kShedFallbacks = 4,
     kShedCounts = 5,
+};
+enum : int {
+    kCommMainBlocks = 0,
+    kCommMainItems = 1,
+    kCommShedBlocks = 2,
+    kCommShedItems = 3,
+    kCommToDeque = 4,
+    kCommToSibling = 5,
+    kCommBusy = 6,
+    kCommRing = 7,
+    kCommCounts = 8,
+};
+enum : uint32_t {
+    kCommUseMain = 1,
+    kCommUseShed = 2,
+    kCommUseRedirect = 4,
 };
 
 #ifndef HX_TIMELINE
@@ -382,16 +399,22 @@
     if constexpr (kind_has_drain<Kind>::value) Kind::drain(ctx, acc, err);
 }
 
-template <class Kind, int CAP>
+template <class Kind>
+struct Inbox;
+template <class Kind, int CAP, bool BLOCK = false, bool HELD = false>
 __device__ bool enqueue_chunk(const typename Kind::Ctx &ctx, const PoolView &pool, SchedGlobals *g, uint32_t q,
                               WaveStack<Kind, CAP> &st, uint32_t bot, uint32_t n, uint32_t &occ, PendingChunk &pc,
-                              bool defer, bool relief = false) {
+                              bool defer, bool relief = false, const Inbox<Kind> *blk = nullptr) {
     constexpr int W = Kind::kWords;
     const int lane = lane_id();
     QueueHdr *h = &pool.hdr[q];
     const bool valid = (uint32_t)lane < n;
     uint32_t w[W];
-    {
+    if constexpr (BLOCK) {
+        const hx_lds_u32 *src = (const hx_lds_u32 *)&blk->w[(valid ? (uint32_t)lane : 0u) * W];
+#pragma unroll
+        for (int i = 0; i < W; ++i) w[i] = src[i];
+    } else {
         const uint32_t p = bot + (valid ? (uint32_t)lane : 0u);
         const uint2 dd = st.d[p & (CAP - 1)];
         load_tmpl<Kind, CAP>(st, (p - (dd.y >> 24)) & (CAP - 1), w);
@@ -403,7 +426,7 @@
     const bool fast = occ < pool.cap / 4;
     if (lane == 0) {
         if (fast) {
-            add_agent(&g->outstanding, 1u);
+            if (!HELD) add_agent(&g->outstanding, 1u);
             pos = add_agent(&h->tail, 1u);
             seen = pos - ld_agent(&h->head);
             ok = 1;
@@ -411,7 +434,7 @@
             const uint32_t hd = ld_agent(&h->head), tl = ld_agent(&h->tail);
             seen = tl - hd;
             if ((int)(tl - hd) < (int)(relief ? pool.cap - 1 : pool.cap / 2) && cas_agent(&h->tail, tl, tl + 1u)) {
-                add_agent(&g->outstanding, 1u);
+                if (!HELD) add_agent(&g->outstanding, 1u);
                 pos = tl;
                 ok = 1;
             }
@@ -433,8 +456,10 @@
     }
     uint32_t *dst = pool.data + (size_t)slot * pool.chunk * W;
     {
-        kind_export<Kind>(ctx, w, valid, &g->err);
-        kind_trace_item<Kind>(ctx, w, valid, 2u, false);
+        if constexpr (!BLOCK) {
+            kind_export<Kind>(ctx, w, valid, &g->err);
+            kind_trace_item<Kind>(ctx, w, valid, 2u, false);
+        }
         if (valid) {
             if constexpr (W % 4 == 0) {
 #pragma unroll
@@ -1007,6 +1032,33 @@
     uint32_t w[64 * Kind::kWords];
 };
 
+constexpr int kOutboxes = 2;
+struct CommCtl {
+    uint32_t on;
+    uint32_t left;
+    unsigned long long cnt[6];
+};
+template <class Kind, int WPG>
+struct WgBoxes {
+    Inbox<Kind> ib[WPG];
+    Inbox<Kind> out[kOutboxes];
+    CommCtl ctl;
+};
+template <class Kind>
+struct WgBoxes<Kind, 1> {
+    Inbox<Kind> ib[1];
+};
+template <class Kind, int WPG>
+__device__ __forceinline__ WgBoxes<Kind, WPG> &wg_boxes(Inbox<Kind> *ib) {
+    using Boxes = WgBoxes<Kind, WPG>;
+    static_assert(__builtin_offsetof(Boxes, ib) == 0, "the inboxes lead the workgroup's boxes");
+    return *(WgBoxes<Kind, WPG> *)ib;
+}
+__device__ __forceinline__ void comm_count(CommCtl &c, int i, unsigned long long v) {
+    typedef __attribute__((address_space(3))) unsigned long long lds_u64;
+    if (lane_id() == 0) __hip_atomic_fetch_add((lds_u64 *)&c.cnt[i], v, __ATOMIC_RELAXED, __HIP_MEMORY_SCOPE_WORKGROUP);
+}
+
 template <class Kind>
 __device__ __forceinline__ uint32_t inbox_claim(Inbox<Kind> &ib) {
     uint32_t ok = 0;
@@ -1059,7 +1111,7 @@
     const uint32_t lane = (uint32_t)lane_id();
     to_ring = 0;
     const uint32_t cfg = lane0(lds_load(&st.shed_cfg));
-    const uint32_t rule = cfg & 0xffu, max_blocks = (cfg >> 8) & 0xffu;
+    const uint32_t rule = cfg & 0xffu, max_blocks = (cfg >> 8) & 0xffu, comm = (cfg >> 16) & 7u;
     if (rule == 0) return 0;
     const uint32_t fit = (64u * rcp16(mu)) >> 16;
     uint32_t keep = rule == 2 ? fit : (rule == 3 ? nsp / 4 : nsp / 2);
@@ -1075,6 +1127,10 @@
         sid[a] = lds_load(&ib[(wave + a) % (uint32_t)WPG].idle);
         sst[a] = lds_load(&ib[(wave + a) % (uint32_t)WPG].state);
     }
+    WgBoxes<Kind, WPG> &bx = wg_boxes<Kind, WPG>(ib);
+    uint32_t ost[kOutboxes];
+#pragma unroll
+    for (int o = 0; o < kOutboxes; ++o) ost[o] = (comm & kCommUseShed) ? lds_load(&bx.out[o].state) : 1u;
     const uint32_t nshed = nsp - keep;
     uint32_t placed = 0, blocks = 0;
 #pragma unroll
@@ -1095,7 +1151,32 @@
             }
         }
     }
-    to_ring = keep + placed;
+    uint32_t oplaced = 0;
+    if (comm & kCommUseShed) {
+        uint32_t oblocks = 0;
+#pragma unroll
+        for (int o = 0; o < kOutboxes; ++o) {
+            if (placed + oplaced < nshed && lane0(ost[o]) == 0u) {
+                Inbox<Kind> &to = bx.out[o];
+                const uint32_t left = nshed - placed - oplaced, bs = left < fit ? left : fit, n = bs * mu;
+                const bool valid = lane < n;
+                const uint32_t ok = inbox_claim<Kind>(to);
+                uint32_t w[W];
+                carry_lds_read<TW>(st.cscr, keep + placed + oplaced + (valid ? r_fix : 0u), w);
+                if (lane0(ok)) {
+                    w[W - 2] = ck_fix;
+                    w[W - 1] = ck_fix + 1u;
+                    inbox_fill<Kind>(ctx, to, w, valid, n, g);
+                    oplaced += bs;
+                    ++oblocks;
+                }
+            }
+        }
+        if (oblocks) comm_count(bx.ctl, 1, (unsigned long long)oblocks | (unsigned long long)(oplaced * mu) << 32);
+        if (placed + oplaced < nshed && oblocks < (uint32_t)kOutboxes) comm_count(bx.ctl, 4, 1ull);
+    }
+    to_ring = keep + placed + oplaced;
+    if (comm && to_ring < nsp) comm_count(bx.ctl, 5, 1ull);
     if (lane == 0) {
         st.shed_cnt[kShedExits] += 1u;
         st.shed_cnt[placed == nshed ? kShedPlaced : kShedFallbacks] += 1u;
@@ -1367,6 +1448,112 @@
     return tout;
 }
 
+template <class Kind, int CAP, int WPG>
+__device__ void comm_wave(const typename Kind::Ctx &ctx, const PoolView &pool, SchedGlobals *g, const SchedConfig &cfg,
+                          WgBoxes<Kind, WPG> &bx, WaveStack<Kind, CAP> &st_unused) {
+    constexpr int W = Kind::kWords;
+    const uint32_t lane = (uint32_t)lane_id();
+    const uint32_t on = lane0(lds_load(&bx.ctl.on));
+    const uint32_t qpx = pool.nq / 8, xcc = xcc_id() & 7u, home_off = ((blockIdx.x * (uint32_t)WPG) / 8u) % qpx;
+    uint32_t occ = 0, naps = 0;
+    PendingChunk pend;
+    pend.live = false;
+    while (true) {
+        uint32_t ost[kOutboxes], sid[WPG], sst[WPG];
+#pragma unroll
+        for (int o = 0; o < kOutboxes; ++o) ost[o] = lds_load(&bx.out[o].state);
+        const uint32_t left = lds_load(&bx.ctl.left);
+#pragma unroll
+        for (int a = 0; a < WPG; ++a) {
+            sid[a] = lds_load(&bx.ib[a].idle);
+            sst[a] = lds_load(&bx.ib[a].state);
+        }
+        bool served = false, failed = false;
+#pragma unroll
+        for (int o = 0; o < kOutboxes; ++o) {
+            if (failed || lane0(ost[o]) != 1u) continue;
+            served = true;
+            Inbox<Kind> &blk = bx.out[o];
+            const uint32_t n = lane0(lds_load(&blk.n));
+            bool done = false;
+            if (n > 64u || (n > pool.chunk && !(on & kCommUseRedirect))) {
+                if (lane == 0) dev_error(&g->err, kErrBadTask);
+                failed = true;
+                continue;
+            }
+            if (on & kCommUseRedirect) {
+#pragma unroll
+                for (int a = 0; a < WPG; ++a) {
+                    if (done || lane0(sid[a]) != 1u || lane0(sst[a]) != 0u) continue;
+                    if (!lane0(inbox_claim<Kind>(bx.ib[a]))) continue;
+                    comm_count(bx.ctl, 3, 1ull);
+                    if (lane < n) {
+                        const hx_lds_u32 *src = (const hx_lds_u32 *)&blk.w[lane * W];
+                        hx_lds_u32 *dst = (hx_lds_u32 *)&bx.ib[a].w[lane * W];
+#pragma unroll
+                        for (int i = 0; i < W; ++i) dst[i] = src[i];
+                    }
+                    asm volatile("" ::: "memory");
+                    if (lane == 0) {
+                        lds_store(&bx.ib[a].n, n);
+                        lds_store(&bx.ib[a].idle, 0u);
+                        lds_store(&bx.ib[a].state, 1u);
+                    }
+                    sst[a] = 1u;
+                    done = true;
+                }
+            }
+            if (!done && n > pool.chunk) {
+                if (lane == 0) dev_error(&g->err, kErrBadTask);
+                failed = true;
+                continue;
+            }
+            if (!done) {
+                comm_count(bx.ctl, 2, 1ull);
+                const unsigned long long t0 = __builtin_amdgcn_s_memrealtime();
+                for (uint32_t round = 0; !done; ++round) {
+                    for (uint32_t a = 0; a < qpx && !done; ++a)
+                        done = enqueue_chunk<Kind, CAP, true, true>(ctx, pool, g, xcc * qpx + (home_off + a) % qpx, st_unused,
+                                                                    0u, n, occ, pend, false, round != 0, &blk);
+                    if (done) break;
+                    uint32_t e = 0;
+                    if (lane == 0) e = ld_agent(&g->err);
+                    if (lane0(e)) break;
+                    if (__builtin_amdgcn_s_memrealtime() - t0 > 100000ull * cfg.spin_limit) {
+                        if (lane == 0) dev_error(&g->err, kErrQueueFull);
+                        break;
+                    }
+                    __builtin_amdgcn_s_sleep(8);
+                }
+            }
+            if (!done) {
+                failed = true;
+                continue;
+            }
+            if (lane == 0) lds_store(&blk.state, 0u);
+        }
+        if (failed) break;
+        if (served) {
+            naps = 0;
+            continue;
+        }
+        bool empty = true;
+#pragma unroll
+        for (int o = 0; o < kOutboxes; ++o) empty = empty && lane0(ost[o]) == 0u;
+        if (lane0(left) == (uint32_t)WPG && empty) break;
+        if ((++naps & 255u) == 0u) {
+            uint32_t e = 0;
+            if (lane == 0) e = ld_agent(&g->err);
+            if (lane0(e)) break;
+        }
+        bool all_idle = true;
+#pragma unroll
+        for (int a = 0; a < WPG; ++a) all_idle = all_idle && lane0(sid[a]) == 1u;
+        __builtin_amdgcn_s_sleep(1);
+        if (all_idle) __builtin_amdgcn_s_sleep(8);
+    }
+}
+
 template <class Kind, int CAP, bool GLOBAL = false, int WPG = 1>
 __device__ void run_worker(const typename Kind::Ctx &ctx, const PoolView &pool, SchedGlobals *g,
                            const SchedConfig &cfg, WaveStack<Kind, CAP> &st, bool seed_roots,
@@ -1411,7 +1598,7 @@
             st.shed_g = (unsigned long long)(uintptr_t)g;
             st.shed_ib = (uint32_t)(uintptr_t)(__attribute__((address_space(3))) Inbox<Kind> *)ib;
             st.shed_wave = wave;
-            st.shed_cfg = cfg.narrow_shed;
+            st.shed_cfg = (cfg.narrow_shed & 0xffffu) | lds_load(&wg_boxes<Kind, WPG>(ib).ctl.on) << 16;
         }
         if (lane < kShedCounts) st.shed_cnt[lane] = 0;
     }
@@ -1880,15 +2067,30 @@
                 bool ok = false;
                 if constexpr (WPG > 1) {
                     uint32_t sid[WPG], sst[WPG];
+                    WgBoxes<Kind, WPG> &bx = wg_boxes<Kind, WPG>(ib);
+                    uint32_t ost[kOutboxes], comm_on = 0;
 #pragma unroll
                     for (uint32_t a = 1; a < (uint32_t)WPG; ++a) {
                         sid[a] = lds_load(&ib[(wave + a) % (uint32_t)WPG].idle);
                         sst[a] = lds_load(&ib[(wave + a) % (uint32_t)WPG].state);
                     }
+                    if constexpr (!GLOBAL) {
+                        comm_on = lds_load(&bx.ctl.on);
+#pragma unroll
+                        for (int o = 0; o < kOutboxes; ++o) ost[o] = lds_load(&bx.out[o].state);
+                    }
 #pragma unroll
                     for (uint32_t a = 1; a < (uint32_t)WPG; ++a)
                         if (!ok && lane0(sid[a]) == 1u && lane0(sst[a]) == 0u)
                             ok = inbox_put<Kind, CAP>(ctx, ib[(wave + a) % (uint32_t)WPG], st, bot, n, g);
+                    if constexpr (!GLOBAL) {
+                        if (!ok && (lane0(comm_on) & kCommUseMain)) {
+#pragma unroll
+                            for (int o = 0; o < kOutboxes; ++o)
+                                if (!ok && lane0(ost[o]) == 0u) ok = inbox_put<Kind, CAP>(ctx, bx.out[o], st, bot, n, g);
+                            comm_count(bx.ctl, ok ? 0 : 4, ok ? 1ull | (unsigned long long)n << 32 : 1ull);
+                        }
+                    }
                 }
                 if (!ok) publish_pending<Kind, CAP>(pool, g, pend);
                 for (uint32_t a = 0; a < qpx && !ok; ++a) {
@@ -1946,6 +2148,9 @@
     unsigned long long shed_v = 0;
     if constexpr (kShed) {
         if (lane >= 32 && lane < 32 + kShedCounts) shed_v = st.shed_cnt[lane - 32];
+    }
+    if constexpr (WPG > 1 && !GLOBAL) {
+        if (wave < 2 && lane >= 37 && lane < 40) shed_v = wg_boxes<Kind, WPG>(ib).ctl.cnt[3 * wave + (lane - 37)];
     }
     if (active) {
         wave_goes_idle<GLOBAL>(g, gv, pool);
@@ -2018,7 +2223,8 @@
         }
         if (lane < kWaveCtrWords) g->wave_ctr[(size_t)gid * kWaveCtrWords + lane] = v;
     } else {
-        if (shed_v) add_agent(&g->shed[lane - 32], shed_v);
+        if (shed_v && lane < 32 + kShedCounts) add_agent(&g->shed[lane - 32], shed_v);
+        if (shed_v && lane >= 37) add_agent(&g->comm[3 * wave + (lane - 37)], shed_v);
         if (lane == 0 && n_narrow_in) {
             add_agent(&g->narrow[0], (unsigned long long)n_narrow);
             add_agent(&g->narrow[1], cyc_narrow);
```

New measurement: 4.496 billion nodes/s (median of 6 runs). +2.9%, better.
